# zjhellofss/KuiperLLama

Hardware: AMD Instinct MI355X
Metric: decode tokens/sec (higher is better)
Workload: dtype f32; 1 GPU; llama3.2-1b greedy decode, batch 1, prompt [1, 263], 2002 steps from pos 0 (demo/main.cpp generate); timing_backend=none, exec=hipGraph replay, 5L+2 fused HIP kernels per token, kv_cache_rows=131072

## Files before the change

include/kuiper_hip.h:

```cpp
#ifndef KUIPER_HIP_H
#define KUIPER_HIP_H
#include <stddef.h>
#include <stdint.h>

#ifdef __cplusplus
extern "C" {
#endif

#define KH_VERSION 100

enum {
  KH_OK = 0,
  KH_ERR_INVALID_ARG = -1,
  KH_ERR_UNSUPPORTED = -2,
  KH_ERR_IO = -3,
  KH_ERR_FORMAT = -4,
  KH_ERR_NO_DEVICE = -5,
  KH_ERR_RANGE = -6,
  KH_ERR_INTERNAL = -7
};
const char* kh_error_string(int code);
int kh_version(void);
int kh_device_count(void);

enum { KH_ROPE_INTERLEAVED = 0, KH_ROPE_HALF = 1 };
enum { KH_FAMILY_LLAMA = 0, KH_FAMILY_QWEN2 = 1 };


int kh_add_f32(const float* in1, const float* in2, float* out, int32_t n, void* stream);

int kh_matmul_f32(const float* x, const float* w, float* y, int32_t M, int32_t K, float scale,
                  void* stream);

int kh_matmul_q8(const float* x, const int8_t* w8, const float* scales, int32_t group_size,
                 float* y, int32_t M, int32_t K, void* stream);

int kh_embedding_f32(const int32_t* tokens, int32_t n_tokens, const float* w, float* out,
                     int32_t dim, int32_t vocab, void* stream);

int kh_embedding_f32_host(const int32_t* h_tokens, int32_t n_tokens, const float* w, float* out,
                          int32_t dim, int32_t vocab, void* stream);

int kh_swiglu_f32(const float* a, const float* b, float* out, int32_t n, void* stream);

int kh_rmsnorm_f32(const float* x, const float* w, float* out, int32_t n, float eps,
                   void* stream);

int kh_rope_f32(int32_t dim, int32_t kv_dim, int32_t head_size, float* q, float* k,
                const int32_t* d_pos, int32_t pos, const float* sin_cache,
                const float* cos_cache, int32_t mode, void* stream);

int kh_sincos_cache_f32(int32_t head_size, int32_t max_seq_len, float theta, float* sin_cache,
                        float* cos_cache, void* stream);

int kh_mha_f32(const int32_t* d_pos, int32_t pos, int32_t head_num, int32_t layer_index,
               int32_t seq_len, int32_t kv_dim, int32_t kv_mul, int32_t head_size,
               float* mha_out, const float* q, float* score, const float* kcache,
               const float* vcache, void* stream);

int kh_mha_prefill_f32(int32_t pos0, int32_t n_tokens, int32_t head_num, int32_t layer_index,
                       int32_t seq_len, int32_t kv_dim, int32_t kv_mul, int32_t head_size,
                       float* mha_out, const float* q, const float* key_cache,
                       const float* value_cache, void* stream);

int64_t kh_mha_decode_workspace_bytes(int32_t head_num, int32_t head_size, int32_t seq_len);
int kh_mha_decode_f32(const int32_t* d_pos, int32_t pos, int32_t head_num, int32_t layer_index,
                      int32_t seq_len, int32_t kv_dim, int32_t kv_mul, int32_t head_size,
                      float* mha_out, const float* q, const float* kcache, const float* vcache,
                      void* workspace, int64_t workspace_bytes, void* stream);

int kh_argmax_f32(const float* logits, int64_t n, int32_t* d_out_index, void* stream);
int kh_argmax_f32_host(const float* logits, int64_t n, int64_t* h_out_index, void* stream);

typedef struct kh_sampling {
  float temperature;
  int32_t top_k;
  float top_p;
  uint64_t seed;
} kh_sampling;
int kh_sample_f32(const float* logits, int64_t n, const kh_sampling* p, int64_t counter0, int32_t n_draws,
                  int32_t* d_out, void* stream);
int kh_sample_f32_host(const float* logits, int64_t n, const kh_sampling* p, int64_t counter, int64_t* h_out,
                       void* stream);

int kh_softmax_f32(float* x, int32_t n, void* stream);
int kh_scale_f32(float scale, float* x, int32_t n, void* stream);
int kh_scale_sum_f32(const float* value, const float* scale, float* out, int32_t pos,
                     int32_t size, int32_t stride, void* stream);

typedef struct kh_model kh_model;

typedef struct kh_model_opts {
  int32_t family;
  int32_t is_quant;
  int32_t rope_mode;
  float rope_theta;
  float rms_eps;
  int32_t max_seq_len;
  int32_t device;
  int32_t flags;
} kh_model_opts;
#define KH_FLAG_ATTN_MERGE_IN_LAUNCH 1
#define KH_FLAG_ATTN_MERGE_FENCED 2
#define KH_FLAG_PREFILL_EXACT 4

typedef struct kh_config {
  int32_t dim, hidden_dim, layer_num, head_num, kv_head_num, vocab_size, seq_len;
  int32_t kv_dim, kv_mul, head_size, is_shared_weight, is_quant, group_size;
  int32_t family, rope_mode, cache_len;
  float rope_theta, rms_eps;
  int64_t weight_bytes;
  int32_t launches_per_token;
  int32_t ring_selftest, attn_merge_selftest;
} kh_config;

int kh_model_create_from_file(const char* path, const kh_model_opts* opts, kh_model** out);
int kh_model_create_from_host_image(const void* h_image, size_t nbytes,
                                    const kh_model_opts* opts, kh_model** out);
int kh_model_create_from_device_weights(const int32_t* h_header, const void* d_weight_data,
                                        size_t weight_nbytes, const kh_model_opts* opts,
                                        kh_model** out);
void kh_model_destroy(kh_model* m);
int kh_model_get_config(const kh_model* m, kh_config* out);
void* kh_model_stream(kh_model* m);
float kh_model_get_load_ms(const kh_model* m);

enum {
  KH_EXEC_GRAPH = 0,
  KH_EXEC_FUSED = 1,
  KH_EXEC_UNFUSED = 2
};

int kh_model_predict(kh_model* m, int32_t token, int32_t pos, int32_t is_prompt, int32_t exec,
                     int32_t* h_next);
int kh_model_get_logits(kh_model* m, float* h_logits);
int kh_model_get_kv(kh_model* m, float** d_kcache, float** d_vcache);
int kh_model_kv_bytes(const kh_model* m, int64_t* reserved, int64_t* committed);
int kh_model_read_kv(kh_model* m, int32_t layer, int32_t row0, int32_t nrows, float* h_k,
                     float* h_v);
int kh_model_write_kv(kh_model* m, int32_t layer, int32_t row0, int32_t nrows, const float* h_k,
                      const float* h_v);

int kh_model_generate(kh_model* m, const int32_t* h_prompt, int32_t n_prompt,
                      int32_t total_steps, int32_t exec, int32_t* h_words, int32_t* n_words,
                      float* h_elapsed_ms);
int kh_model_generate_until(kh_model* m, const int32_t* h_prompt, int32_t n_prompt,
                            int32_t total_steps, int32_t exec, const int32_t* h_stop,
                            int32_t n_stop, int32_t* h_words, int32_t* n_words,
                            float* h_elapsed_ms);

int kh_model_prefill(kh_model* m, const int32_t* h_tokens, int32_t n, int32_t pos0);

int kh_model_prefill_gemm(kh_model* m, const int32_t* h_tokens, int32_t n, int32_t pos0);

typedef struct kh_first_sample {
  int32_t pos;
  int32_t prefill_mode;
  int32_t top1_id, top2_id;
  float top1, top2;
} kh_first_sample;
int kh_model_first_sample(kh_model* m, kh_first_sample* out);

int kh_model_set_sampling(kh_model* m, const kh_sampling* p);
int kh_model_get_sampling(const kh_model* m, kh_sampling* out);

int kh_plan_decode_shapes(int32_t dim, int32_t hidden_dim, int32_t kv_dim, int32_t vocab_size,
                          int32_t is_quant, int32_t* out20);
int kh_plan_decode_ring(int32_t dim, int32_t hidden_dim, int32_t vocab_size, int32_t is_quant, int32_t group_size,
                        int32_t* out4);
int kh_plan_attention(int32_t head_num, int32_t kv_mul, int32_t head_size, int32_t seq_len, int32_t pos,
                      int32_t* out8);
int kh_plan_prefill_shape(int32_t epi, int32_t T, int32_t rows, int32_t K, int32_t is_quant,
                          int32_t r2_ok, int32_t* out7);

int kh_debug_set(const char* key, const char* value);
const char* kh_debug_get(const char* key);
int64_t kh_debug_list(char* buf, int64_t cap);
int64_t kh_debug_launch_log(char* buf, int64_t cap);

enum { KH_PREFILL_TOKEN = 0, KH_PREFILL_GEMV = 1, KH_PREFILL_GEMM = 2 };
int kh_model_time_prefill(kh_model* m, const int32_t* h_tokens, int32_t n, int32_t pos0,
                          int32_t mode, float* h_ms);

int kh_model_profile_kernel(kh_model* m, int32_t kclass, int32_t pos, int32_t reps,
                            float* h_avg_us);

int kh_model_time_step(kh_model* m, int32_t pos, int32_t reps, float* h_us);

enum {
  KH_K_QKV = 0, KH_K_ATTN = 1, KH_K_WO = 2, KH_K_FFN13 = 3, KH_K_W2 = 4, KH_K_CLS = 5,
  KH_K_SAMPLE = 6, KH_NUM_KCLASS = 7
};
int kh_model_profile_step(kh_model* m, int32_t start_pos, int32_t n_steps, float* h_avg_us,
                          int32_t* h_count);
const char* kh_kclass_name(int kclass);

typedef struct kh_spm kh_spm;
int kh_spm_create_from_file(const char* tokenizer_model_path, kh_spm** out);
int kh_spm_create_from_memory(const void* model_proto, int64_t nbytes, kh_spm** out);
void kh_spm_destroy(kh_spm* t);
int32_t kh_spm_vocab_size(const kh_spm* t);
int32_t kh_spm_bos_id(const kh_spm* t);
int32_t kh_spm_eos_id(const kh_spm* t);
int32_t kh_spm_unk_id(const kh_spm* t);
int kh_spm_encode(const kh_spm* t, const char* utf8, int64_t len, int32_t add_bos, int32_t add_eos,
                  int32_t* out_ids, int32_t cap, int32_t* n_ids);
int kh_spm_decode(const kh_spm* t, const int32_t* ids, int32_t n, char* out_utf8, int64_t cap,
                  int64_t* out_len);

typedef struct kh_bpe kh_bpe;
enum { KH_BPE_LLAMA3 = 0, KH_BPE_QWEN2 = 1 };
enum { KH_BPE_REF_SPACES = 1 };
int kh_bpe_create_from_file(const char* tokenizer_json_path, int32_t flavor, kh_bpe** out);
int kh_bpe_create_from_memory(const void* tokenizer_json, int64_t nbytes, int32_t flavor, kh_bpe** out);
void kh_bpe_destroy(kh_bpe* t);
int32_t kh_bpe_vocab_size(const kh_bpe* t);
int32_t kh_bpe_bos_id(const kh_bpe* t);
int32_t kh_bpe_eos_id(const kh_bpe* t);
int32_t kh_bpe_stop_id(const kh_bpe* t, int32_t which);
int kh_bpe_encode(const kh_bpe* t, const char* utf8, int64_t len, int32_t add_bos, int32_t add_eos,
                  int32_t flags, int32_t* out_ids, int32_t cap, int32_t* n_ids);
int kh_bpe_decode(const kh_bpe* t, const int32_t* ids, int32_t n, int32_t flags, char* out_utf8,
                  int64_t cap, int64_t* out_len);

#ifdef __cplusplus
}
#endif
#endif
```

kuiperllama_amd/_ffi.py:

```python
from __future__ import annotations

import ctypes as C
import os
from typing import Optional

_PKG = os.path.dirname(os.path.abspath(__file__))
LIB_PATH = os.environ.get("KH_LIB") or os.path.join(_PKG, "lib", "libkuiper_hip.so")

EXPORTS = [
    "kh_error_string", "kh_version", "kh_device_count",
    "kh_add_f32", "kh_matmul_f32", "kh_matmul_q8", "kh_embedding_f32", "kh_embedding_f32_host", "kh_swiglu_f32",
    "kh_rmsnorm_f32", "kh_rope_f32", "kh_sincos_cache_f32", "kh_mha_f32", "kh_mha_decode_f32", "kh_mha_prefill_f32",
    "kh_mha_decode_workspace_bytes", "kh_argmax_f32",
    "kh_argmax_f32_host", "kh_sample_f32", "kh_sample_f32_host", "kh_softmax_f32", "kh_scale_f32", "kh_scale_sum_f32",
    "kh_model_create_from_file", "kh_model_create_from_host_image",
    "kh_model_create_from_device_weights", "kh_model_destroy", "kh_model_get_config",
    "kh_model_stream", "kh_model_get_load_ms", "kh_model_predict", "kh_model_get_logits", "kh_model_get_kv", "kh_model_kv_bytes", "kh_model_read_kv", "kh_model_write_kv",
    "kh_spm_create_from_file", "kh_spm_create_from_memory", "kh_spm_destroy", "kh_spm_vocab_size",
    "kh_spm_bos_id", "kh_spm_eos_id", "kh_spm_unk_id", "kh_spm_encode", "kh_spm_decode",
    "kh_bpe_create_from_file", "kh_bpe_create_from_memory", "kh_bpe_destroy", "kh_bpe_vocab_size",
    "kh_bpe_bos_id", "kh_bpe_eos_id", "kh_bpe_stop_id", "kh_bpe_encode", "kh_bpe_decode",
    "kh_model_generate", "kh_model_generate_until", "kh_model_first_sample", "kh_model_set_sampling", "kh_model_get_sampling", "kh_model_time_step", "kh_model_prefill", "kh_model_prefill_gemm", "kh_model_time_prefill", "kh_model_profile_kernel", "kh_model_profile_step", "kh_kclass_name",
    "kh_plan_decode_shapes", "kh_plan_decode_ring", "kh_plan_prefill_shape", "kh_plan_attention",
    "kh_debug_set", "kh_debug_get", "kh_debug_list", "kh_debug_launch_log",
]

KH_EXEC_GRAPH, KH_EXEC_FUSED, KH_EXEC_UNFUSED = 0, 1, 2
KH_NUM_KCLASS = 7
KH_ERR_RANGE = -6
KH_ERR_INTERNAL = -7
KH_FLAG_ATTN_MERGE_IN_LAUNCH = 1
KH_FLAG_ATTN_MERGE_FENCED = 2
KH_FLAG_PREFILL_EXACT = 4


class KhError(RuntimeError):
    def __init__(self, code: int, what: str):
        self.code = code
        super().__init__(f"{what}: kh error {code} ({error_string(code)})")


class ModelOpts(C.Structure):
    _fields_ = [("family", C.c_int32), ("is_quant", C.c_int32), ("rope_mode", C.c_int32),
                ("rope_theta", C.c_float), ("rms_eps", C.c_float), ("max_seq_len", C.c_int32),
                ("device", C.c_int32), ("flags", C.c_int32)]


class FirstSample(C.Structure):
    _fields_ = [("pos", C.c_int32), ("prefill_mode", C.c_int32), ("top1_id", C.c_int32), ("top2_id", C.c_int32),
                ("top1", C.c_float), ("top2", C.c_float)]


class Sampling(C.Structure):
    _fields_ = [("temperature", C.c_float), ("top_k", C.c_int32), ("top_p", C.c_float), ("seed", C.c_uint64)]

    def as_dict(self) -> dict:
        return {"temperature": float(self.temperature), "top_k": int(self.top_k), "top_p": float(self.top_p),
                "seed": int(self.seed)}


def sampling(temperature: float = 0.0, top_k: int = 0, top_p: float = 1.0, seed: int = 0) -> Sampling:
    return Sampling(float(temperature), int(top_k), float(top_p), int(seed) & 0xFFFFFFFFFFFFFFFF)


class Config(C.Structure):
    _fields_ = [(n, C.c_int32) for n in (
        "dim", "hidden_dim", "layer_num", "head_num", "kv_head_num", "vocab_size", "seq_len",
        "kv_dim", "kv_mul", "head_size", "is_shared_weight", "is_quant", "group_size", "family",
        "rope_mode", "cache_len")] + [("rope_theta", C.c_float), ("rms_eps", C.c_float),
                                      ("weight_bytes", C.c_int64), ("launches_per_token", C.c_int32),
                                      ("ring_selftest", C.c_int32), ("attn_merge_selftest", C.c_int32)]


_lib: Optional[C.CDLL] = None
_vp, _i32, _i64, _f32 = C.c_void_p, C.c_int32, C.c_int64, C.c_float


def lib() -> C.CDLL:
    global _lib
    if _lib is not None:
        return _lib
    import torch
    if not os.path.exists(LIB_PATH):
        raise ImportError(
            f"{LIB_PATH} is missing: build it with `python -m kuiperllama_amd.build` "
            "(there is no CPU fallback for the HIP path)")
    L = C.CDLL(LIB_PATH)
    L.kh_error_string.argtypes = [C.c_int]
    L.kh_error_string.restype = C.c_char_p
    L.kh_version.restype = C.c_int
    L.kh_device_count.restype = C.c_int
    L.kh_add_f32.argtypes = [_vp, _vp, _vp, _i32, _vp]
    L.kh_matmul_f32.argtypes = [_vp, _vp, _vp, _i32, _i32, _f32, _vp]
    L.kh_matmul_q8.argtypes = [_vp, _vp, _vp, _i32, _vp, _i32, _i32, _vp]
    L.kh_embedding_f32.argtypes = [_vp, _i32, _vp, _vp, _i32, _i32, _vp]
    L.kh_embedding_f32_host.argtypes = [_vp, _i32, _vp, _vp, _i32, _i32, _vp]
    L.kh_swiglu_f32.argtypes = [_vp, _vp, _vp, _i32, _vp]
    L.kh_rmsnorm_f32.argtypes = [_vp, _vp, _vp, _i32, _f32, _vp]
    L.kh_rope_f32.argtypes = [_i32, _i32, _i32, _vp, _vp, _vp, _i32, _vp, _vp, _i32, _vp]
    L.kh_sincos_cache_f32.argtypes = [_i32, _i32, _f32, _vp, _vp, _vp]
    L.kh_mha_f32.argtypes = [_vp, _i32, _i32, _i32, _i32, _i32, _i32, _i32, _vp, _vp, _vp, _vp,
                             _vp, _vp]
    L.kh_mha_decode_workspace_bytes.argtypes = [_i32, _i32, _i32]
    L.kh_mha_decode_workspace_bytes.restype = _i64
    L.kh_mha_prefill_f32.argtypes = [_i32] * 8 + [_vp, _vp, _vp, _vp, _vp]
    L.kh_mha_decode_f32.argtypes = [_vp, _i32, _i32, _i32, _i32, _i32, _i32, _i32, _vp, _vp, _vp,
                                    _vp, _vp, _i64, _vp]
    L.kh_argmax_f32.argtypes = [_vp, _i64, _vp, _vp]
    L.kh_argmax_f32_host.argtypes = [_vp, _i64, C.POINTER(_i64), _vp]
    L.kh_sample_f32.argtypes = [_vp, _i64, C.POINTER(Sampling), _i64, _i32, _vp, _vp]
    L.kh_sample_f32_host.argtypes = [_vp, _i64, C.POINTER(Sampling), _i64, C.POINTER(_i64), _vp]
    L.kh_softmax_f32.argtypes = [_vp, _i32, _vp]
    L.kh_scale_f32.argtypes = [_f32, _vp, _i32, _vp]
    L.kh_scale_sum_f32.argtypes = [_vp, _vp, _vp, _i32, _i32, _i32, _vp]
    L.kh_model_create_from_file.argtypes = [C.c_char_p, C.POINTER(ModelOpts), C.POINTER(_vp)]
    L.kh_model_create_from_host_image.argtypes = [_vp, C.c_size_t, C.POINTER(ModelOpts),
                                                  C.POINTER(_vp)]
    L.kh_model_create_from_device_weights.argtypes = [C.POINTER(_i32), _vp, C.c_size_t,
                                                      C.POINTER(ModelOpts), C.POINTER(_vp)]
    L.kh_model_destroy.argtypes = [_vp]
    L.kh_model_destroy.restype = None
    L.kh_model_get_config.argtypes = [_vp, C.POINTER(Config)]
    L.kh_model_stream.argtypes = [_vp]
    L.kh_model_stream.restype = _vp
    L.kh_model_get_load_ms.argtypes = [_vp]
    L.kh_model_get_load_ms.restype = _f32
    L.kh_model_predict.argtypes = [_vp, _i32, _i32, _i32, _i32, C.POINTER(_i32)]
    L.kh_model_get_logits.argtypes = [_vp, _vp]
    L.kh_model_get_kv.argtypes = [_vp, C.POINTER(_vp), C.POINTER(_vp)]
    L.kh_model_kv_bytes.argtypes = [_vp, C.POINTER(_i64), C.POINTER(_i64)]
    L.kh_model_read_kv.argtypes = [_vp, _i32, _i32, _i32, _vp, _vp]
    L.kh_model_write_kv.argtypes = [_vp, _i32, _i32, _i32, _vp, _vp]
    L.kh_model_generate.argtypes = [_vp, C.POINTER(_i32), _i32, _i32, _i32, C.POINTER(_i32),
                                    C.POINTER(_i32), C.POINTER(_f32)]
    L.kh_model_generate_until.argtypes = [_vp, C.POINTER(_i32), _i32, _i32, _i32, C.POINTER(_i32),
                                          _i32, C.POINTER(_i32), C.POINTER(_i32), C.POINTER(_f32)]
    L.kh_model_first_sample.argtypes = [_vp, C.POINTER(FirstSample)]
    L.kh_model_set_sampling.argtypes = [_vp, C.POINTER(Sampling)]
    L.kh_model_get_sampling.argtypes = [_vp, C.POINTER(Sampling)]
    L.kh_model_time_step.argtypes = [_vp, _i32, _i32, C.POINTER(_f32)]
    L.kh_plan_decode_shapes.argtypes = [_i32, _i32, _i32, _i32, _i32, C.POINTER(_i32)]
    L.kh_plan_decode_ring.argtypes = [_i32, _i32, _i32, _i32, _i32, C.POINTER(_i32)]
    L.kh_plan_prefill_shape.argtypes = [_i32, _i32, _i32, _i32, _i32, _i32, C.POINTER(_i32)]
    L.kh_plan_attention.argtypes = [_i32, _i32, _i32, _i32, _i32, C.POINTER(_i32)]
    L.kh_spm_create_from_file.argtypes = [C.c_char_p, C.POINTER(_vp)]
    L.kh_spm_create_from_memory.argtypes = [_vp, C.c_int64, C.POINTER(_vp)]
    L.kh_spm_destroy.argtypes = [_vp]
    L.kh_spm_destroy.restype = None
    for fn in (L.kh_spm_vocab_size, L.kh_spm_bos_id, L.kh_spm_eos_id, L.kh_spm_unk_id):
        fn.argtypes = [_vp]
        fn.restype = _i32
    L.kh_spm_encode.argtypes = [_vp, C.c_char_p, C.c_int64, _i32, _i32, C.POINTER(_i32), _i32,
                                C.POINTER(_i32)]
    L.kh_spm_decode.argtypes = [_vp, C.POINTER(_i32), _i32, C.c_char_p, C.c_int64,
                                C.POINTER(C.c_int64)]
    L.kh_bpe_create_from_file.argtypes = [C.c_char_p, _i32, C.POINTER(_vp)]
    L.kh_bpe_create_from_memory.argtypes = [_vp, C.c_int64, _i32, C.POINTER(_vp)]
    L.kh_bpe_destroy.argtypes = [_vp]
    L.kh_bpe_destroy.restype = None
    for fn in (L.kh_bpe_vocab_size, L.kh_bpe_bos_id, L.kh_bpe_eos_id):
        fn.argtypes = [_vp]
    L.kh_bpe_stop_id.argtypes = [_vp, _i32]
    L.kh_bpe_encode.argtypes = [_vp, C.c_char_p, C.c_int64, _i32, _i32, _i32, C.POINTER(_i32), _i32,
                                C.POINTER(_i32)]
    L.kh_bpe_decode.argtypes = [_vp, C.POINTER(_i32), _i32, _i32, C.c_char_p, C.c_int64,
                                C.POINTER(C.c_int64)]
    L.kh_model_prefill.argtypes = [_vp, C.POINTER(_i32), _i32, _i32]
    L.kh_model_prefill_gemm.argtypes = [_vp, C.POINTER(_i32), _i32, _i32]
    L.kh_model_time_prefill.argtypes = [_vp, C.POINTER(_i32), _i32, _i32, _i32, C.POINTER(_f32)]
    L.kh_model_profile_kernel.argtypes = [_vp, _i32, _i32, _i32, C.POINTER(_f32)]
    L.kh_model_profile_step.argtypes = [_vp, _i32, _i32, C.POINTER(_f32), C.POINTER(_i32)]
    L.kh_kclass_name.argtypes = [C.c_int]
    L.kh_kclass_name.restype = C.c_char_p
    L.kh_debug_set.argtypes = [C.c_char_p, C.c_char_p]
    L.kh_debug_get.argtypes = [C.c_char_p]
    L.kh_debug_get.restype = C.c_char_p
    L.kh_debug_list.argtypes = [C.c_char_p, _i64]
    L.kh_debug_list.restype = _i64
    L.kh_debug_launch_log.argtypes = [C.c_char_p, _i64]
    L.kh_debug_launch_log.restype = _i64
    for name in EXPORTS:
        getattr(L, name)
    _lib = L
    return L


def debug_set(key: str, value: Optional[str]) -> None:
    _ENV_MIRRORED.pop(key, None)
    check(lib().kh_debug_set(key.encode(), None if value is None else str(value).encode()), "kh_debug_set")


def debug_get(key: str) -> Optional[str]:
    v = lib().kh_debug_get(key.encode())
    return None if v is None else v.decode()


def launch_log() -> set:
    L = lib()
    n = L.kh_debug_launch_log(None, 0)
    buf = C.create_string_buffer(int(n) + 1)
    L.kh_debug_launch_log(buf, int(n) + 1)
    return {k for k in buf.value.decode().split("\n") if k}


_HOOK_PREFIXES = ("KH_SHAPE_", "KH_ATTN_", "KH_PG_", "KH_PREFILL", "KH_RING", "KH_SELFTEST", "KH_KV_")
_ENV_MIRRORED = {}
_ENV_SEEDED = False


def _seed_mirror(L) -> None:
    global _ENV_SEEDED
    _ENV_SEEDED = True
    n = L.kh_debug_list(None, 0)
    if n <= 0:
        return
    buf = C.create_string_buffer(int(n) + 1)
    L.kh_debug_list(buf, int(n) + 1)
    for k in buf.value.decode().split("\n"):
        if k and k.startswith(_HOOK_PREFIXES) and k in _ENV_AT_IMPORT:
            v = L.kh_debug_get(k.encode())
            if v is not None and v.decode() == _ENV_AT_IMPORT[k]:
                _ENV_MIRRORED.setdefault(k, _ENV_AT_IMPORT[k])


_ENV_AT_IMPORT = {k: v for k, v in os.environ.items() if k.startswith(_HOOK_PREFIXES)}


def sync_env() -> None:
    if not _ENV_SEEDED:
        _seed_mirror(lib())
    want = {k: v for k, v in os.environ.items() if k.startswith(_HOOK_PREFIXES)}
    if want == _ENV_MIRRORED:
        return
    L = lib()
    for k in set(_ENV_MIRRORED) - set(want):
        L.kh_debug_set(k.encode(), None)
        del _ENV_MIRRORED[k]
    for k, v in want.items():
        if _ENV_MIRRORED.get(k) != v:
            L.kh_debug_set(k.encode(), v.encode())
            _ENV_MIRRORED[k] = v


def error_string(code: int) -> str:
    return lib().kh_error_string(int(code)).decode()


def check(code: int, what: str) -> None:
    if code != 0:
        raise KhError(int(code), what)


def plan_decode_shapes(dim: int, hidden_dim: int, kv_dim: int, vocab_size: int, quant: bool) -> dict:
    sync_env()
    out = (_i32 * 20)()
    rc = lib().kh_plan_decode_shapes(dim, hidden_dim, kv_dim, vocab_size, int(quant), out)
    if rc != 0:
        raise KhError(rc, "kh_plan_decode_shapes")
    names = ("qkv", "wo", "ffn13", "w2", "cls")
    return {n: dict(zip(("split", "u", "grid", "wg"), out[4 * i:4 * i + 4])) for i, n in enumerate(names)}


def plan_decode_ring(dim: int, hidden_dim: int, vocab_size: int, quant: bool, group_size: int = 64) -> dict:
    sync_env()
    out = (_i32 * 4)()
    rc = lib().kh_plan_decode_ring(dim, hidden_dim, vocab_size, int(quant), group_size, out)
    if rc != 0:
        raise KhError(rc, "kh_plan_decode_ring")
    return {"ffn13": {"slots": out[0], "grid": out[1]}, "cls": {"slots": out[2], "grid": out[3]}}


def plan_attention(head_num: int, kv_mul: int, head_size: int, seq_len: int, pos: int) -> dict:
    sync_env()
    out = (_i32 * 8)()
    rc = lib().kh_plan_attention(head_num, kv_mul, head_size, seq_len, pos, out)
    if rc != 0:
        raise KhError(rc, "kh_plan_attention")
    return dict(zip(("ns", "ns_g", "stride", "t_long", "group_path", "active_splits", "split_len", "workgroups"),
                    list(out)))


def plan_prefill_shape(epi: str, T: int, rows: int, K: int, quant: bool, r2_ok: bool = True) -> dict:
    sync_env()
    out = (_i32 * 7)()
    rc = lib().kh_plan_prefill_shape({"qkv": 0, "resid": 1, "swiglu": 2}[epi], T, rows, K, int(quant),
                                     int(r2_ok), out)
    if rc != 0:
        raise KhError(rc, "kh_plan_prefill_shape")
    return dict(zip(("R", "NT", "ks", "slices", "solo", "kz", "workgroups"), out[:]))
```

kuiperllama_amd/build.py:

```python
from __future__ import annotations

import os
import shutil
import subprocess
import sys

_PKG = os.path.dirname(os.path.abspath(__file__))
CSRC = os.path.join(_PKG, "csrc")
LIB_DIR = os.path.join(_PKG, "lib")
LIB_PATH = os.path.join(LIB_DIR, "libkuiper_hip.so")
SOURCES = ["kh_ops.hip", "kh_model_load.hip", "kh_model_step.hip", "kh_model_prefill.hip", "kh_model_profile.hip", "kh_model_selftest.hip",
           "kh_tokenizer.cpp", "kh_bpe.cpp", "kh_debug.cpp"]
HEADERS = ["kh_common.h", "kh_gemv.h", "kh_attn.h", "kh_fused.h", "kh_q8ring.h", "kh_fused_ring.h", "kh_prefill.h", "kh_gemm.h", "kh_pattn.h", "kh_sample.h", "kh_unicode_tables.h",
           "kh_model_internal.h",
           "../../include/kuiper_hip.h"]
ARCH = "gfx950"


def _hipcc() -> str:
    for cand in (os.environ.get("HIPCC"), shutil.which("hipcc"), "/opt/rocm/bin/hipcc"):
        if cand and os.path.exists(cand):
            return cand
    raise RuntimeError("hipcc not found (set HIPCC=...)")


def _stale() -> bool:
    if not os.path.exists(LIB_PATH):
        return True
    t = os.path.getmtime(LIB_PATH)
    for f in SOURCES + HEADERS:
        p = os.path.normpath(os.path.join(CSRC, f))
        if os.path.exists(p) and os.path.getmtime(p) > t:
            return True
    return False


def build_lib(force: bool = False, verbose: bool = False) -> str:
    if not force and not _stale():
        return LIB_PATH
    os.makedirs(LIB_DIR, exist_ok=True)
    objs, procs = [], []
    for src in SOURCES:
        obj = os.path.join(LIB_DIR, os.path.splitext(src)[0] + ".o")
        cmd = [_hipcc(), f"--offload-arch={ARCH}", "-O3", "-std=c++17", "-fPIC", "-Wall",
               "-ffp-contract=off",
               "-Wno-unused-function", "-c", os.path.join(CSRC, src), "-o", obj]
        if verbose:
            print(" ".join(cmd), flush=True)
        procs.append((cmd, subprocess.Popen(cmd)))
        objs.append(obj)
    for cmd, pr in procs:
        if pr.wait() != 0:
            raise subprocess.CalledProcessError(pr.returncode, cmd)
    cmd = [_hipcc(), f"--offload-arch={ARCH}", "-shared", "-fPIC", "-o", LIB_PATH] + objs
    if verbose:
        print(" ".join(cmd), flush=True)
    subprocess.check_call(cmd)
    return LIB_PATH


def build_variant(name: str, defines: list[str], commit: str | None = None) -> str:
    out = os.path.join(LIB_DIR, name + ".so")
    if commit:
        import tarfile
        import tempfile
        root = os.path.normpath(os.path.join(_PKG, ".."))
        with tempfile.TemporaryDirectory() as td:
            tar = os.path.join(td, "src.tar")
            subprocess.check_call(["git", "-C", root, "archive", "-o", tar, commit, "kuiperllama_amd/csrc", "include"])
            with tarfile.open(tar) as tf:
                tf.extractall(td)
            global CSRC
            saved, CSRC = CSRC, os.path.join(td, "kuiperllama_amd", "csrc")
            try:
                return build_variant(name, defines)
            finally:
                CSRC = saved
    objs, procs = [], []
    od = os.path.join(LIB_DIR, "_" + name)
    os.makedirs(od, exist_ok=True)
    for src in SOURCES:
        if not os.path.exists(os.path.join(CSRC, src)):
            continue
        obj = os.path.join(od, os.path.splitext(src)[0] + ".o")
        cmd = [_hipcc(), f"--offload-arch={ARCH}", "-O3", "-std=c++17", "-fPIC", "-ffp-contract=off", "-w"] + \
              [f"-D{d}" for d in defines] + ["-c", os.path.join(CSRC, src), "-o", obj]
        procs.append((cmd, subprocess.Popen(cmd)))
        objs.append(obj)
    for cmd, pr in procs:
        if pr.wait() != 0:
            raise subprocess.CalledProcessError(pr.returncode, cmd)
    subprocess.check_call([_hipcc(), f"--offload-arch={ARCH}", "-shared", "-fPIC", "-o", out] + objs)
    shutil.rmtree(od, ignore_errors=True)
    return out


if __name__ == "__main__":
    if len(sys.argv) > 2 and sys.argv[1] == "--variant":
        print(build_variant(sys.argv[2], sys.argv[3:]))
    elif len(sys.argv) > 3 and sys.argv[1] == "--variant-at":
        print(build_variant(sys.argv[3], sys.argv[4:], commit=sys.argv[2]))
    else:
        print(build_lib(force="--force" in sys.argv, verbose=True))


ADAPTER_TEST_SRC = os.path.normpath(os.path.join(_PKG, "..", "tests", "cpp", "test_adapter.cpp"))
ADAPTER_TEST_BIN = os.path.join(LIB_DIR, "test_adapter")


def build_adapter_test(force: bool = False) -> str:
    build_lib()
    inc = os.path.normpath(os.path.join(_PKG, "..", "include"))
    deps = [ADAPTER_TEST_SRC, os.path.join(os.path.dirname(ADAPTER_TEST_SRC), "adapter_cases.hpp"),
            os.path.join(inc, "kuiper_hip_adapter.hpp"), os.path.join(inc, "kuiper_hip_alloc.hpp"), os.path.join(inc, "kuiper_hip.h"), LIB_PATH]
    if (not force and os.path.exists(ADAPTER_TEST_BIN)
            and all(os.path.getmtime(d) <= os.path.getmtime(ADAPTER_TEST_BIN) for d in deps)):
        return ADAPTER_TEST_BIN
    subprocess.check_call([_hipcc(), "-std=c++17", "-O2", f"-I{inc}", ADAPTER_TEST_SRC, "-o",
                           ADAPTER_TEST_BIN, f"-L{LIB_DIR}", "-lkuiper_hip",
                           "-Wl,-rpath,$ORIGIN"])
    return ADAPTER_TEST_BIN


DEMO_SRC = os.path.normpath(os.path.join(_PKG, "..", "tools", "kuiper_demo.cpp"))
DEMO_BIN = os.path.join(LIB_DIR, "kuiper_demo")


def build_demo(force: bool = False) -> str:
    build_lib()
    inc = os.path.normpath(os.path.join(_PKG, "..", "include"))
    deps = [DEMO_SRC, os.path.join(inc, "kuiper_hip.h"), LIB_PATH]
    if (not force and os.path.exists(DEMO_BIN)
            and all(os.path.getmtime(d) <= os.path.getmtime(DEMO_BIN) for d in deps)):
        return DEMO_BIN
    subprocess.check_call([_hipcc(), "-std=c++17", "-O2", f"-I{inc}", DEMO_SRC, "-o", DEMO_BIN,
                           f"-L{LIB_DIR}", "-lkuiper_hip", "-Wl,-rpath,$ORIGIN"])
    return DEMO_BIN


REF_ROOT = os.environ.get("KUIPER_REF", "/root/reference")
REF_BINDING_BIN = os.path.normpath(os.path.join(_PKG, "..", "oracle", "_ref", "test_ref_binding"))


def build_ref_binding() -> str | None:
    if not os.path.isdir(os.path.join(REF_ROOT, "kuiper", "include")):
        return REF_BINDING_BIN if os.path.exists(REF_BINDING_BIN) else None
    build_lib()
    subprocess.check_call(["make", "-s", "-C", os.path.normpath(os.path.join(_PKG, "..", "oracle")),
                           "ref", f"KUIPER_REF={REF_ROOT}", f"HIPCC={_hipcc()}"])
    return REF_BINDING_BIN


REF_LAYERS_BIN = os.path.normpath(os.path.join(_PKG, "..", "oracle", "_ref", "test_ref_layers"))


def build_ref_layers() -> str | None:
    if not os.path.isdir(os.path.join(REF_ROOT, "kuiper", "include")):
        return REF_LAYERS_BIN if os.path.exists(REF_LAYERS_BIN) else None
    build_lib()
    subprocess.check_call(["make", "-s", "-C", os.path.normpath(os.path.join(_PKG, "..", "oracle")),
                           "ref_layers", f"KUIPER_REF={REF_ROOT}", f"HIPCC={_hipcc()}"])
    return REF_LAYERS_BIN


REF_MODEL_BIN = os.path.normpath(os.path.join(_PKG, "..", "oracle", "_ref", "test_ref_model"))


def build_ref_model(qwen2: bool = False) -> str | None:
    exe = REF_MODEL_BIN + ("_qwen2" if qwen2 else "")
    if not os.path.isdir(os.path.join(REF_ROOT, "kuiper", "include")):
        return exe if os.path.exists(exe) else None
    build_lib()
    subprocess.check_call(["make", "-s", "-C", os.path.normpath(os.path.join(_PKG, "..", "oracle")),
                           "ref_model_qwen2" if qwen2 else "ref_model", f"KUIPER_REF={REF_ROOT}", f"HIPCC={_hipcc()}"])
    return exe


REF_CPU_BINS = {flavor: os.path.normpath(os.path.join(_PKG, "..", "oracle", "_ref", "ref_cpu_model" + suffix))
                for flavor, suffix in (("default", ""), ("llama3", "_llama3"), ("qwen2", "_qwen2"))}


def build_ref_cpu() -> dict | None:
    if os.path.isdir(os.path.join(REF_ROOT, "kuiper", "include")):
        build_lib()
        subprocess.check_call(["make", "-s", "-C", os.path.normpath(os.path.join(_PKG, "..", "oracle")),
                               "ref_cpu", f"KUIPER_REF={REF_ROOT}", f"HIPCC={_hipcc()}"])
    return dict(REF_CPU_BINS) if all(os.path.exists(p) for p in REF_CPU_BINS.values()) else None


def ref_cpu_flavor(spec) -> str | None:
    from . import binfmt
    if spec.quant:
        return None
    key = (spec.family, spec.rope_mode, float(spec.rope_theta), float(spec.rms_eps))
    table = {(binfmt.FAMILY_LLAMA, binfmt.ROPE_INTERLEAVED, 10000.0, 1e-5): "default",
             (binfmt.FAMILY_LLAMA, binfmt.ROPE_HALF, 500000.0, 1e-5): "llama3",
             (binfmt.FAMILY_QWEN2, binfmt.ROPE_HALF, 1000000.0, 1e-6): "qwen2"}
    return table.get(key)


def kernel_sources_sha1() -> str:
    import hashlib
    h = hashlib.sha1()
    d = os.path.join(os.path.dirname(os.path.abspath(__file__)), "csrc")
    for f in sorted(os.listdir(d)):
        if f.startswith("kh_") and f.endswith(".h") and f != "kh_model_internal.h":
            h.update(f.encode())
            h.update(open(os.path.join(d, f), "rb").read())
    return h.hexdigest()
```

kuiperllama_amd/csrc/kh_model_internal.h:

```cpp
#pragma once
#include <new>
#include <thread>
#include <stdint.h>

#include <vector>

#include "kh_attn.h"
#include "kh_common.h"

namespace khm {
template <class F>
static inline int kh_api_guard(F&& body) noexcept {
  try {
    return body();
  } catch (const std::bad_alloc&) {
    return (int)hipErrorOutOfMemory;
  } catch (...) {
    return KH_ERR_INTERNAL;
  }
}
struct KhJoinOnExit {
  std::thread& t;
  ~KhJoinOnExit() {
    if (t.joinable()) t.join();
  }
};

struct LayerW {
  KhLin wq, wk, wv, wo, w1, w2, w3;
  const float* att_norm;
  const float* ffn_norm;
};

}
using khm::LayerW;

#define KH_STEP_VARIANTS 3
struct KhSampParams;
struct kh_model {
  kh_config cfg{};
  kh_model_opts opts{};
  hipStream_t stream = nullptr;
  char* arena = nullptr;
  bool owns_arena = false;
  size_t arena_bytes = 0;
  std::vector<LayerW> layers;
  const float* tok_emb = nullptr;
  const float* final_norm = nullptr;
  KhLin cls{};
  int gshift = 0;
  float *x = nullptr, *rms = nullptr, *q = nullptr, *att = nullptr, *h1 = nullptr,
        *h3 = nullptr, *w2o = nullptr, *logits = nullptr, *score = nullptr, *kcache = nullptr,
        *vcache = nullptr, *sin_cache = nullptr, *cos_cache = nullptr;
  float* part_val = nullptr;
  int32_t* part_idx = nullptr;
  int nparts = 0;
  struct KvVmm {
    bool on = false;
    size_t chunk = 0;
    size_t reserved = 0;
    size_t mapped = 0;
    std::vector<uint8_t> have[2];
    struct Run {
      void* va;
      size_t len;
      hipMemGenericAllocationHandle_t h;
    };
    std::vector<Run> runs;
    int rows_all = 0;
  };
  KvVmm kv;
  float load_ms = 0.f;
  std::thread unmap_thread;
  void* attn_ws = nullptr;
  int attn_ns = 1;
  int attn_ns_g = 0;
  int attn_ws_stride = 1;
  int attn_t_long = 1 << 30;
  int attn_wg = KH_WG;
  int attn_ts_shift = 8;
  bool attn_fenced = false;
  bool attn_defer = false;
  int attn_defer_max = 0;
  int step_var = 0;
  int32_t *d_pos = nullptr, *d_token = nullptr, *d_next = nullptr, *d_forced = nullptr,
          *d_words = nullptr;
  int seq_cap = 0;
  float *pf_x = nullptr, *pf_q = nullptr, *pf_att = nullptr, *pf_h = nullptr;
  void* pf_ws = nullptr;
  size_t pf_ws_tok_bytes = 0;
  float *pg_x = nullptr, *pg_xn = nullptr, *pg_q = nullptr, *pg_att = nullptr, *pg_h = nullptr;
  float* pg_part = nullptr;
  void* pg_ws = nullptr;
  size_t pg_ws_tok_bytes = 0;
  bool pf_ready = false, pg_ready = false;
  bool pg_launch_failed = false;
  int32_t* h_words_pin = nullptr;
  int32_t* h_forced_pin = nullptr;
  int forced_hwm = 0;
  bool forced_in_flight = false;
  float* first_logits = nullptr;
  int first_pos = -1;
  int first_mode = 0;
  int pin_cap = 0;
  hipEvent_t ev_chunk[2] = {nullptr, nullptr};
  struct Shape {
    int u = 2, split = 1, grid = 1, wg = KH_WG;
  };
  Shape sh_qkv, sh_wo, sh_ffn, sh_w2, sh_cls;
  struct RingPlan {
    int ffn_r = 0, ffn_grid = 0, cls_r = 0, cls_grid = 0;
  };
  RingPlan ring;
  struct StepGraph {
    hipGraph_t g = nullptr;
    hipGraphExec_t e = nullptr;
  };
  StepGraph sg[2][KH_STEP_VARIANTS][4];
  kh_sampling samp{0.f, 0, 1.f, 0};
  bool samp_on = false;
  KhSampParams* d_samp = nullptr;
  hipEvent_t ev0 = nullptr, ev1 = nullptr;
};

#define KH_GRAPH_STEPS 8
#define KH_PG_MIN_TOKENS 16

namespace khm {
template <typename T>
int dalloc(T** p, size_t n) {
  hipError_t e = hipMalloc((void**)p, n * sizeof(T));
  return e == hipSuccess ? KH_OK : (int)e;
}

kh_model::Shape pick_shape(bool quant, int pairs, int M, int max_split, const char* env, int wg = KH_WG,
                           int wg_max = KH_WG, bool many_waves = false, bool u3 = false);
void plan_decode_shapes(bool quant, int dim, int hidden_dim, int kv_dim, int vocab_size, kh_model::Shape (&out)[5]);
void plan_ring(bool quant, int dim, int hidden_dim, int vocab_size, int group_size, kh_model::RingPlan* out);
int configure_step_kernels(kh_model* m);
KhAttnArgs fill_attn(kh_model* m, int l);
void launch_qkv(kh_model* m, int l);
void launch_attn(kh_model* m, int l);
void launch_wo(kh_model* m, int l);
void launch_ffn13(kh_model* m, int l);
void launch_w2(kh_model* m, int l);
void launch_cls(kh_model* m);
void launch_sample(kh_model* m, int advance, int n_forced);
int step_variant(const kh_model* m, int pos_lo, int pos_hi);
void launch_step_fused(kh_model* m, int advance, int n_forced, hipEvent_t* ev, int variant);
int launch_step_unfused(kh_model* m, int pos);
void set_state(kh_model* m, int token, int pos);
int ensure_pinned_words(kh_model* m, int n);
int ensure_seq_cap(kh_model* m, int n);
void destroy_step_graphs(kh_model* m);
int step_graph(kh_model* m, int n_forced, int variant, bool steps8, hipGraphExec_t* out);
int step_graph_n(kh_model* m, int n_forced, int variant, int nsteps, hipGraphExec_t* out);
int kv_ensure(kh_model* m, int rows, int layer = -1);
int run_selftests(kh_model* m);
bool prefill_supported(const kh_model* m);
bool pg_supported(const kh_model* m);
}
```

kuiperllama_amd/csrc/kh_model_load.hip:

```cpp
#include <fcntl.h>
#include <math.h>
#include <stdio.h>
#include <stdlib.h>
#include <string.h>
#include <sys/mman.h>
#include <sys/stat.h>
#include <unistd.h>

#include <atomic>
#include <mutex>
#include <utility>
#include <chrono>
#include <new>
#include <thread>
#include <vector>

#include "kh_model_internal.h"

using namespace khm;

namespace {

struct PhaseClock {
  std::chrono::steady_clock::time_point t = std::chrono::steady_clock::now();
  const bool on = dbg("KH_LOAD_DEBUG") != nullptr;
  void lap(const char* what) {
    if (!on) return;
    const auto n = std::chrono::steady_clock::now();
    fprintf(stderr, "[kh load] %-34s %7.2f ms\n", what, std::chrono::duration<double, std::milli>(n - t).count());
    t = n;
  }
};

int ilog2_exact(int v) {
  if (v <= 0 || (v & (v - 1))) return -1;
  int s = 0;
  while ((1 << s) < v) ++s;
  return s;
}

int upload_threads() {
  long n = sysconf(_SC_NPROCESSORS_ONLN);
  if (FILE* f = fopen("/sys/fs/cgroup/cpu.max", "r")) {
    long long quota = 0, period = 0;
    char q[32] = {0};
    if (fscanf(f, "%31s %lld", q, &period) == 2 && strcmp(q, "max") != 0 && period > 0) {
      quota = atoll(q);
      if (quota > 0 && quota / period < n) n = (long)(quota / period);
    }
    fclose(f);
  }
  n /= 2;
  return n < 1 ? 1 : (n > 8 ? 8 : (int)n);
}
hipError_t upload_chunked(char* d_dst, const char* h_src, size_t n, hipStream_t stream,
                          float* ms_out) {
  constexpr int NB = 4;
  const size_t CH = (size_t)32 << 20;
  const auto t0 = std::chrono::steady_clock::now();
  if (n <= CH) {
    hipError_t e = hipMemcpy(d_dst, h_src, n, hipMemcpyHostToDevice);
    if (ms_out)
      *ms_out = std::chrono::duration<float, std::milli>(std::chrono::steady_clock::now() - t0).count();
    return e;
  }
  char* pin[NB] = {nullptr, nullptr, nullptr, nullptr};
  hipEvent_t done[NB] = {nullptr, nullptr, nullptr, nullptr};
  hipError_t e = hipSuccess;
  PhaseClock pc;
  for (int i = 0; i < NB && e == hipSuccess; ++i) {
    e = hipHostMalloc((void**)&pin[i], CH, hipHostMallocDefault);
    if (e == hipSuccess) e = hipEventCreateWithFlags(&done[i], hipEventDisableTiming);
  }
  pc.lap("pinned staging ring");
  if (e == hipSuccess) {
    const size_t nchunks = (n + CH - 1) / CH;
    const int NT = upload_threads();
    std::vector<std::atomic<int>> filled(nchunks);
    for (auto& f : filled) f.store(0, std::memory_order_relaxed);
    std::atomic<long> released{NB};
    std::atomic<bool> abort_{false};
    auto worker = [&](int w) {
      for (size_t c = 0; c < nchunks; ++c) {
        if (abort_.load(std::memory_order_relaxed)) return;
        while ((long)c >= released.load(std::memory_order_acquire)) {
          if (abort_.load(std::memory_order_relaxed)) return;
          std::this_thread::yield();
        }
        const size_t off = c * CH, len = off + CH <= n ? CH : n - off;
        const size_t per = ((len + NT - 1) / NT + 4095) & ~(size_t)4095;
        const size_t s0 = (size_t)w * per, s1 = s0 + per < len ? s0 + per : len;
        if (s0 < len) memcpy(pin[c % NB] + s0, h_src + off + s0, s1 - s0);
        filled[c].fetch_add(1, std::memory_order_release);
      }
    };
    std::vector<std::thread> team;
    try {
      team.reserve((size_t)NT);
      for (int w = 0; w < NT; ++w) team.emplace_back(worker, w);
    } catch (...) {
      abort_.store(true);
      e = hipErrorOutOfMemory;
    }
    for (size_t c = 0; c < nchunks && e == hipSuccess; ++c) {
      while (filled[c].load(std::memory_order_acquire) < NT) std::this_thread::yield();
      const size_t off = c * CH, len = off + CH <= n ? CH : n - off;
      e = hipMemcpyAsync(d_dst + off, pin[c % NB], len, hipMemcpyHostToDevice, stream);
      if (e == hipSuccess) e = hipEventRecord(done[c % NB], stream);
      if (c + 1 >= (size_t)NB && c + 1 < nchunks && e == hipSuccess) {
        e = hipEventSynchronize(done[(c + 1) % NB]);
        released.store((long)c + 2, std::memory_order_release);
      }
    }
    if (e != hipSuccess) abort_.store(true);
    released.store((long)nchunks + NB, std::memory_order_release);
    for (auto& t : team) t.join();
    if (e == hipSuccess) e = hipStreamSynchronize(stream);
    pc.lap("staged upload");
  }
  for (int i = 0; i < NB; ++i) {
    if (done[i]) (void)hipEventDestroy(done[i]);
    if (pin[i]) (void)hipHostFree(pin[i]);
  }
  if (ms_out)
    *ms_out = std::chrono::duration<float, std::milli>(std::chrono::steady_clock::now() - t0).count();
  return e;
}

struct SinCosJob {
  std::vector<float> s, c;
  std::vector<std::thread> team;
  void start(size_t CL, int head_size, float theta) {
    const size_t n = CL * (size_t)head_size;
    s.resize(n);
    c.resize(n);
    std::vector<float> freq((size_t)head_size);
    for (int d = 0; d < head_size; ++d) freq[d] = 1.0f / powf(theta, (float)d / (float)head_size);
    const int NT = CL >= 4096 ? upload_threads() : 1;
    for (int w = 0; w < NT; ++w)
      team.emplace_back([this, CL, head_size, freq, w, NT] {
        const size_t p0 = CL * (size_t)w / NT, p1 = CL * (size_t)(w + 1) / NT;
        for (size_t p = p0; p < p1; ++p)
          for (int d = 0; d < head_size; ++d) {
            const float val = (float)p * freq[d];
            s[p * head_size + d] = sinf(val);
            c[p * head_size + d] = cosf(val);
          }
      });
  }
  void join() {
    for (auto& t : team) t.join();
    team.clear();
  }
  ~SinCosJob() { join(); }
};

int build_weight_table(kh_model* m) {
  const kh_config& c = m->cfg;
  const int L = c.layer_num, dim = c.dim, kvd = c.kv_dim, hid = c.hidden_dim, V = c.vocab_size;
  m->layers.assign((size_t)L, LayerW{});
  char* base = m->arena;
  size_t off = 0;
  if (!c.is_quant) {
    const bool bias = c.family == KH_FAMILY_QWEN2;
    auto takef = [&](size_t n) {
      const float* p = (const float*)(base + off);
      off += n * sizeof(float);
      return p;
    };
    m->tok_emb = takef((size_t)V * dim);
    for (int l = 0; l < L; ++l) m->layers[l].att_norm = takef((size_t)dim);
    for (int l = 0; l < L; ++l) {
      m->layers[l].wq.w = takef((size_t)dim * dim);
      if (bias) m->layers[l].wq.bias = takef((size_t)dim);
    }
    for (int l = 0; l < L; ++l) {
      m->layers[l].wk.w = takef((size_t)kvd * dim);
      if (bias) m->layers[l].wk.bias = takef((size_t)kvd);
    }
    for (int l = 0; l < L; ++l) {
      m->layers[l].wv.w = takef((size_t)kvd * dim);
      if (bias) m->layers[l].wv.bias = takef((size_t)kvd);
    }
    for (int l = 0; l < L; ++l) m->layers[l].wo.w = takef((size_t)dim * dim);
    for (int l = 0; l < L; ++l) m->layers[l].ffn_norm = takef((size_t)dim);
    for (int l = 0; l < L; ++l) m->layers[l].w1.w = takef((size_t)hid * dim);
    for (int l = 0; l < L; ++l) m->layers[l].w2.w = takef((size_t)dim * hid);
    for (int l = 0; l < L; ++l) m->layers[l].w3.w = takef((size_t)hid * dim);
    m->final_norm = takef((size_t)dim);
    (void)takef((size_t)c.seq_len * c.head_size);
    if (c.is_shared_weight) {
      m->cls.w = m->tok_emb;
    } else {
      m->cls.w = takef((size_t)V * dim);
    }
  } else {
    const size_t gs = (size_t)c.group_size;
    auto takeq = [&](KhLin& Lw, size_t K, size_t M) {
      const size_t n = K * M;
      Lw.w = base + off;
      Lw.scales = (const float*)(base + off + n);
      off += n + (n / gs) * sizeof(float);
    };
    for (int l = 0; l < L; ++l) takeq(m->layers[l].wq, dim, dim);
    for (int l = 0; l < L; ++l) takeq(m->layers[l].wk, kvd, dim);
    for (int l = 0; l < L; ++l) takeq(m->layers[l].wv, kvd, dim);
    for (int l = 0; l < L; ++l) takeq(m->layers[l].wo, dim, dim);
    for (int l = 0; l < L; ++l) takeq(m->layers[l].w1, hid, dim);
    for (int l = 0; l < L; ++l) takeq(m->layers[l].w2, dim, hid);
    for (int l = 0; l < L; ++l) takeq(m->layers[l].w3, hid, dim);
    takeq(m->cls, V, dim);
    const float* fp = (const float*)(base + off);
    m->tok_emb = fp;
    fp += (size_t)V * dim;
    for (int l = 0; l < L; ++l) m->layers[l].att_norm = fp + (size_t)l * dim;
    fp += (size_t)L * dim;
    for (int l = 0; l < L; ++l) m->layers[l].ffn_norm = fp + (size_t)l * dim;
    fp += (size_t)L * dim;
    m->final_norm = fp;
    fp += dim;
    off = (size_t)((const char*)fp - base);
  }
  if (off > m->arena_bytes) return KH_ERR_FORMAT;
  return KH_OK;
}

int parse_header(const int32_t* h, const kh_model_opts* o, kh_config* c) {
  memset(c, 0, sizeof(*c));
  c->dim = h[0];
  c->hidden_dim = h[1];
  c->layer_num = h[2];
  c->head_num = h[3];
  c->kv_head_num = h[4];
  c->is_shared_weight = h[5] > 0;
  c->vocab_size = h[5] < 0 ? -h[5] : h[5];
  c->seq_len = h[6];
  c->is_quant = o->is_quant ? 1 : 0;
  c->group_size = o->is_quant ? h[7] : 0;
  if (c->dim <= 0 || c->hidden_dim <= 0 || c->layer_num <= 0 || c->head_num <= 0 ||
      c->kv_head_num <= 0 || c->vocab_size <= 0 || c->seq_len <= 0)
    return KH_ERR_FORMAT;
  if (c->dim % c->head_num || c->head_num % c->kv_head_num) return KH_ERR_FORMAT;
  c->kv_dim = (c->dim * c->kv_head_num) / c->head_num;
  c->kv_mul = c->head_num / c->kv_head_num;
  c->head_size = c->dim / c->head_num;
  c->family = o->family;
  c->rope_mode = o->rope_mode;
  c->rope_theta = o->rope_theta;
  c->rms_eps = o->rms_eps;
  c->cache_len = (o->max_seq_len > 0 && o->max_seq_len < c->seq_len) ? o->max_seq_len : c->seq_len;
  if (c->is_quant) {
    if (c->group_size <= 0) return KH_ERR_FORMAT;
    if (c->is_shared_weight || c->family == KH_FAMILY_QWEN2) return KH_ERR_UNSUPPORTED;
  }
  if (o->rope_mode != KH_ROPE_HALF && o->rope_mode != KH_ROPE_INTERLEAVED) return KH_ERR_INVALID_ARG;
  if (o->family != KH_FAMILY_LLAMA && o->family != KH_FAMILY_QWEN2) return KH_ERR_INVALID_ARG;
  if (!(o->rope_theta > 0.f) || !(o->rms_eps > 0.f)) return KH_ERR_INVALID_ARG;
  const int a = c->is_quant ? 16 : 4;
  if (c->dim % a || c->hidden_dim % a || c->head_size % 4 || (c->head_size & 1) ||
      c->head_size > 256 || c->kv_dim % 4 || (c->dim & 1) || (c->kv_dim & 1))
    return KH_ERR_UNSUPPORTED;
  if (c->is_quant) {
    const int gs = ilog2_exact(c->group_size);
    if (gs < 4 || c->dim % c->group_size || c->hidden_dim % c->group_size) return KH_ERR_UNSUPPORTED;
  }
  return KH_OK;
}

size_t expected_weight_bytes(const kh_config& c) {
  const size_t L = c.layer_num, dim = c.dim, kvd = c.kv_dim, hid = c.hidden_dim, V = c.vocab_size;
  const size_t lin = L * (2 * dim * dim + 2 * kvd * dim + 3 * hid * dim);
  if (!c.is_quant) {
    size_t n = V * dim + 2 * L * dim + lin + dim + (size_t)c.seq_len * c.head_size;
    if (c.family == KH_FAMILY_QWEN2) n += L * (dim + 2 * kvd);
    if (!c.is_shared_weight) n += V * dim;
    return n * sizeof(float);
  }
  const size_t q = lin + V * dim;
  return q + (q / (size_t)c.group_size) * sizeof(float) + (V * dim + 2 * L * dim + dim) * sizeof(float);
}

static int kv_ensure_impl(kh_model* m, int row0, int rows, int layer);
static void kv_release(kh_model* m);
struct VaPool {
  std::mutex mu;
  std::vector<std::pair<void*, size_t>> ranges;
};
static VaPool& va_pool() {
  static VaPool* p = new VaPool();
  return *p;
}
static void* va_take(size_t bytes, size_t align) {
  {
    VaPool& vp = va_pool();
    std::lock_guard<std::mutex> g(vp.mu);
    for (size_t i = vp.ranges.size(); i-- > 0;)
      if (vp.ranges[i].second == bytes) {
        void* p = vp.ranges[i].first;
        vp.ranges.erase(vp.ranges.begin() + (long)i);
        return p;
      }
  }
  void* p = nullptr;
  if (hipMemAddressReserve(&p, bytes, align, nullptr, 0) != hipSuccess) {
    (void)hipGetLastError();
    return nullptr;
  }
  return p;
}
static void va_give(void* p, size_t bytes) {
  if (!p) return;
  if (dbg_off("KH_KV_VA_POOL")) {
    (void)hipMemAddressFree(p, bytes);
    return;
  }
  VaPool& vp = va_pool();
  std::lock_guard<std::mutex> g(vp.mu);
  vp.ranges.emplace_back(p, bytes);
}
static int kv_allocate(kh_model* m) {
  const kh_config& c = m->cfg;
  const size_t total = (size_t)c.layer_num * (size_t)c.cache_len * c.kv_dim * sizeof(float);
  kh_model::KvVmm& kv = m->kv;
  if (!dbg_off("KH_KV_VMM")) {
    hipMemAllocationProp prop = {};
    prop.type = hipMemAllocationTypePinned;
    prop.location.type = hipMemLocationTypeDevice;
    prop.location.id = m->opts.device;
    size_t gran = 0;
    if (hipMemGetAllocationGranularity(&gran, &prop, hipMemAllocationGranularityRecommended) == hipSuccess && gran > 0) {
      size_t chunk = (size_t)8 << 20;
      chunk = (chunk + gran - 1) / gran * gran;
      const size_t reserved = (total + chunk - 1) / chunk * chunk;
      void *pk = va_take(reserved, chunk), *pv = nullptr;
      if (pk) {
        if ((pv = va_take(reserved, chunk)) != nullptr) {
          kv.on = true;
          kv.chunk = chunk;
          kv.reserved = reserved;
          kv.have[0].assign(reserved / chunk, 0);
          kv.have[1].assign(reserved / chunk, 0);
          m->kcache = (float*)pk;
          m->vcache = (float*)pv;
          if (kv_ensure_impl(m, 0, 1, 0) == KH_OK) return KH_OK;
          kv_release(m);
          kv = kh_model::KvVmm();
        } else {
          va_give(pk, reserved);
        }
      }
    }
    (void)hipGetLastError();
  }
  int rc;
  if ((rc = dalloc(&m->kcache, total / sizeof(float))) != KH_OK) return rc;
  return dalloc(&m->vcache, total / sizeof(float));
}
static void kv_release(kh_model* m) {
  kh_model::KvVmm& kv = m->kv;
  if (!kv.on) {
    if (m->kcache) (void)hipFree(m->kcache);
    if (m->vcache) (void)hipFree(m->vcache);
  } else {
    for (const auto& r : kv.runs) {
      (void)hipMemUnmap(r.va, r.len);
      (void)hipMemRelease(r.h);
    }
    kv.runs.clear();
    if (m->kcache) va_give(m->kcache, kv.reserved);
    if (m->vcache) va_give(m->vcache, kv.reserved);
    kv.on = false;
  }
  m->kcache = m->vcache = nullptr;
}
static int kv_ensure_impl(kh_model* m, int row0, int rows, int layer) {
  kh_model::KvVmm& kv = m->kv;
  if (!kv.on || rows <= 0) return KH_OK;
  const kh_config& c = m->cfg;
  if (rows > c.cache_len) rows = c.cache_len;
  if (rows <= kv.rows_all || row0 >= rows) return KH_OK;
  if (row0 < 0) row0 = 0;
  hipMemAllocationProp prop = {};
  prop.type = hipMemAllocationTypePinned;
  prop.location.type = hipMemLocationTypeDevice;
  prop.location.id = m->opts.device;
  hipMemAccessDesc acc = {};
  acc.location = prop.location;
  acc.flags = hipMemAccessFlagsProtReadWrite;
  const size_t row_b = (size_t)c.kv_dim * sizeof(float), layer_b = (size_t)c.cache_len * row_b;
  const int l0 = layer >= 0 ? layer : 0, l1 = layer >= 0 ? layer + 1 : c.layer_num;
  for (int which = 0; which < 2; ++which) {
    char* base = (char*)(which ? m->vcache : m->kcache);
    std::vector<uint8_t>& have = kv.have[which];
    for (int l = l0; l < l1; ++l) {
      const size_t b0 = (size_t)l * layer_b + (size_t)row0 * row_b, b1 = (size_t)l * layer_b + (size_t)rows * row_b;
      size_t ch = b0 / kv.chunk;
      const size_t ch_end = (b1 + kv.chunk - 1) / kv.chunk;
      while (ch < ch_end) {
        if (have[ch]) {
          ++ch;
          continue;
        }
        size_t e = ch;
        while (e < ch_end && !have[e]) ++e;
        for (size_t k = ch; k < e; ++k) {
          kh_model::KvVmm::Run r;
          r.va = base + k * kv.chunk;
          r.len = kv.chunk;
          const char* what = "hipMemCreate";
          hipError_t err = hipMemCreate(&r.h, r.len, &prop, 0);
          if (err == hipSuccess) {
            what = "hipMemMap";
            err = hipMemMap(r.va, r.len, 0, r.h, 0);
            if (err == hipSuccess) {
              what = "hipMemSetAccess";
              err = hipMemSetAccess(r.va, r.len, &acc, 1);
              if (err != hipSuccess) (void)hipMemUnmap(r.va, r.len);
            }
            if (err != hipSuccess) (void)hipMemRelease(r.h);
          }
          if (err != hipSuccess) {
            fprintf(stderr, "[kh] KV cache: %s of %zu MiB at chunk %zu of the %s cache (layer %d) failed: %s\n", what,
                    r.len >> 20, k, which ? "V" : "K", l, hipGetErrorString(err));
            (void)hipGetLastError();
            return (int)err;
          }
          kv.runs.push_back(r);
          have[k] = 1;
          kv.mapped += r.len;
        }
        KH_CHECK_HIP(hipMemsetAsync(base + ch * kv.chunk, 0, (e - ch) * kv.chunk, m->stream));
        ch = e;
      }
    }
  }
  if (layer < 0 && row0 == 0) kv.rows_all = rows;
  return KH_OK;
}

int finish_create(kh_model* m, SinCosJob* sincos = nullptr) {
  const kh_config& c = m->cfg;
  int rc;
  PhaseClock pc;
  if ((rc = build_weight_table(m)) != KH_OK) return rc;
  m->gshift = c.is_quant ? ilog2_exact(c.group_size) : 0;
  const size_t CL = (size_t)c.cache_len;
#define KH_ALLOC(ptr, n) \
  if ((rc = dalloc(&(ptr), (n))) != KH_OK) return rc
  KH_ALLOC(m->x, (size_t)c.dim);
  KH_ALLOC(m->rms, (size_t)c.dim);
  KH_ALLOC(m->q, (size_t)c.dim);
  KH_ALLOC(m->att, (size_t)c.dim);
  KH_ALLOC(m->w2o, (size_t)c.dim);
  KH_ALLOC(m->h1, (size_t)c.hidden_dim);
  KH_ALLOC(m->h3, (size_t)c.hidden_dim);
  KH_ALLOC(m->logits, (size_t)c.vocab_size);
  KH_ALLOC(m->score, (size_t)c.head_num * CL);
  pc.lap("weight table + small buffers");
  if ((rc = kv_allocate(m)) != KH_OK) return rc;
  KH_ALLOC(m->sin_cache, CL * c.head_size);
  KH_ALLOC(m->cos_cache, CL * c.head_size);
  KH_ALLOC(m->d_pos, 1);
  KH_ALLOC(m->d_token, 1);
  KH_ALLOC(m->d_next, 1);
  {
    kh_model::Shape sh[5];
    plan_decode_shapes(c.is_quant != 0, c.dim, c.hidden_dim, c.kv_dim, c.vocab_size, sh);
    m->sh_qkv = sh[0]; m->sh_wo = sh[1]; m->sh_ffn = sh[2]; m->sh_w2 = sh[3]; m->sh_cls = sh[4];
  }
  plan_ring(c.is_quant != 0, c.dim, c.hidden_dim, c.vocab_size, c.group_size, &m->ring);
  m->nparts = m->ring.cls_r ? m->ring.cls_grid : m->sh_cls.grid;
  if (dbg("KH_SHAPE_DEBUG")) {
    if (m->ring.ffn_r || m->ring.cls_r)
      fprintf(stderr, "[kh] LDS-DMA ring: ffn13 R %d grid %d | cls R %d grid %d (256 threads)\n", m->ring.ffn_r,
              m->ring.ffn_grid, m->ring.cls_r, m->ring.cls_grid);
    const struct { const char* n; const kh_model::Shape* s; } all[] = {
        {"qkv", &m->sh_qkv}, {"wo", &m->sh_wo}, {"ffn13", &m->sh_ffn}, {"w2", &m->sh_w2}, {"cls", &m->sh_cls}};
    for (const auto& e : all)
      fprintf(stderr, "[kh] shape %-5s split %d u %d grid %d wg %d\n", e.n, e.s->split, e.s->u, e.s->grid, e.s->wg);
  }
  m->attn_wg = KH_WG_MAX;
  if (const char* e = dbg("KH_ATTN_WG"))
    if (atoi(e) == 256 || atoi(e) == 512) m->attn_wg = atoi(e);
  {
    const AttnPlan ap = attn_plan(c.head_num, c.kv_mul, c.head_size, c.cache_len, m->attn_wg, attn_tlong_hook());
    m->attn_ns = ap.ns;
    m->attn_ts_shift = ap.ts_shift;
    m->attn_ns_g = ap.ns_g;
    m->attn_ws_stride = ap.stride;
    m->attn_t_long = ap.t_long;
  }
  {
    const char* e = dbg("KH_ATTN_FENCED");
    m->attn_fenced = (m->opts.flags & KH_FLAG_ATTN_MERGE_FENCED) != 0 || (e && e[0] == '1');
  }
  m->attn_defer = m->attn_ns > 1 && !(m->opts.flags & KH_FLAG_ATTN_MERGE_IN_LAUNCH) && !dbg_off("KH_ATTN_DEFER") &&
                  comb_supported(c.dim, c.head_num, c.head_size, m->sh_wo.wg);
  {
    const int mv = c.dim <= 2 * 4 * m->sh_wo.wg ? 2 : 4;
    const bool overlap = !(m->sh_wo.u >= 8 || (c.is_quant && m->sh_wo.u >= 4 && mv >= 4));
    m->attn_defer_max = overlap ? KH_ATTN_MAX_NS : 4;
    if (const char* e = dbg("KH_ATTN_DEFER_MAX")) m->attn_defer_max = atoi(e);
  }
  if (const size_t wsb = attn_ws_bytes(c.head_num, c.head_size, m->attn_ws_stride)) {
    KH_CHECK_HIP(hipMalloc(&m->attn_ws, wsb));
    KH_CHECK_HIP(hipMemsetAsync(m->attn_ws, 0, wsb, m->stream));
  }
  KH_ALLOC(m->part_val, (size_t)m->nparts);
  KH_ALLOC(m->part_idx, (size_t)m->nparts);
#undef KH_ALLOC
  pc.lap("caches, tables, plans, workspace");
  if (!m->kv.on) {
    KH_CHECK_HIP(hipMemsetAsync(m->kcache, 0, sizeof(float) * c.layer_num * CL * c.kv_dim, m->stream));
    KH_CHECK_HIP(hipMemsetAsync(m->vcache, 0, sizeof(float) * c.layer_num * CL * c.kv_dim, m->stream));
  }
  KH_CHECK_HIP(hipMemsetAsync(m->d_pos, 0, sizeof(int32_t), m->stream));
  KH_CHECK_HIP(hipMemsetAsync(m->d_token, 0, sizeof(int32_t), m->stream));
  {
    SinCosJob local;
    SinCosJob* job = sincos;
    if (!job) {
      local.start(CL, c.head_size, c.rope_theta);
      job = &local;
    }
    job->join();
    pc.lap("wait for the RoPE table threads");
    const size_t n = CL * c.head_size;
    KH_CHECK_HIP(hipMemcpy(m->sin_cache, job->s.data(), n * sizeof(float), hipMemcpyHostToDevice));
    KH_CHECK_HIP(hipMemcpy(m->cos_cache, job->c.data(), n * sizeof(float), hipMemcpyHostToDevice));
  }
  pc.lap("RoPE table upload");
  if ((rc = configure_step_kernels(m)) != KH_OK) return rc;
  KH_CHECK_HIP(hipEventCreate(&m->ev0));
  KH_CHECK_HIP(hipEventCreate(&m->ev1));
  if ((rc = ensure_seq_cap(m, 256)) != KH_OK) return rc;
  KH_CHECK_HIP(hipStreamSynchronize(m->stream));
  pc.lap("kernel attributes, events, sync");
  return KH_OK;
}

int new_model(const int32_t* h_header, const kh_model_opts* opts, kh_model** out) {
  if (!h_header || !opts || !out) return KH_ERR_INVALID_ARG;
  *out = nullptr;
  int ndev = 0;
  if (hipGetDeviceCount(&ndev) != hipSuccess || ndev <= 0) {
    (void)hipGetLastError();
    return KH_ERR_NO_DEVICE;
  }
  if (opts->device < 0 || opts->device >= ndev) return KH_ERR_INVALID_ARG;
  kh_config cfg;
  int rc = parse_header(h_header, opts, &cfg);
  if (rc != KH_OK) return rc;
  KH_CHECK_HIP(hipSetDevice(opts->device));
  kh_model* m = new (std::nothrow) kh_model();
  if (!m) return (int)hipErrorOutOfMemory;
  m->cfg = cfg;
  m->opts = *opts;
  hipError_t e = hipStreamCreateWithFlags(&m->stream, hipStreamNonBlocking);
  if (e != hipSuccess) {
    delete m;
    return (int)e;
  }
  *out = m;
  return KH_OK;
}

}

namespace khm {
int kv_ensure(kh_model* m, int rows, int layer) { return kv_ensure_impl(m, 0, rows, layer); }
}

extern "C" void kh_model_destroy(kh_model* m) {
  if (!m) return;
  if (m->unmap_thread.joinable()) m->unmap_thread.join();
  if (m->stream) (void)hipStreamSynchronize(m->stream);
  destroy_step_graphs(m);
  if (m->ev0) (void)hipEventDestroy(m->ev0);
  if (m->ev1) (void)hipEventDestroy(m->ev1);
  for (void* q : {(void*)m->pf_x, (void*)m->pf_q, (void*)m->pf_att, (void*)m->pf_h, m->pf_ws,
                  (void*)m->pg_x, (void*)m->pg_xn, (void*)m->pg_q, (void*)m->pg_att, (void*)m->pg_h, (void*)m->pg_part,
                  m->pg_ws})
    if (q) (void)hipFree(q);
  for (auto e : m->ev_chunk)
    if (e) (void)hipEventDestroy(e);
  if (m->h_words_pin) (void)hipHostFree(m->h_words_pin);
  if (m->h_forced_pin) (void)hipHostFree(m->h_forced_pin);
  if (m->first_logits) (void)hipFree(m->first_logits);
  if (m->d_samp) (void)hipFree(m->d_samp);
  void* bufs[] = {m->x,      m->rms,    m->q,         m->att,       m->h1,       m->h3,
                  m->w2o,    m->logits, m->score,     m->sin_cache,
                  m->cos_cache, m->part_val, m->part_idx, m->d_pos, m->d_token,  m->d_next,
                  m->d_forced, m->d_words, m->attn_ws};
  for (void* b : bufs)
    if (b) (void)hipFree(b);
  kv_release(m);
  if (m->owns_arena && m->arena) (void)hipFree(m->arena);
  if (m->stream) (void)hipStreamDestroy(m->stream);
  delete m;
}

static int create_from_device_weights_impl(const int32_t* h_header, const void* d_weight_data, size_t weight_nbytes,
                                           const kh_model_opts* opts, kh_model** out) {
  kh_model* m = nullptr;
  int rc = new_model(h_header, opts, &m);
  if (rc != KH_OK) return rc;
  *out = m;
  if (weight_nbytes < expected_weight_bytes(m->cfg)) {
    kh_model_destroy(m);
    *out = nullptr;
    return KH_ERR_FORMAT;
  }
  m->arena = (char*)const_cast<void*>(d_weight_data);
  m->owns_arena = false;
  m->arena_bytes = weight_nbytes;
  m->cfg.weight_bytes = (int64_t)expected_weight_bytes(m->cfg);
  rc = finish_create(m);
  if (rc == KH_OK) rc = run_selftests(m);
  if (rc != KH_OK) {
    kh_model_destroy(m);
    m = nullptr;
  }
  *out = m;
  return rc;
}
extern "C" int kh_model_create_from_device_weights(const int32_t* h_header,
                                                   const void* d_weight_data,
                                                   size_t weight_nbytes,
                                                   const kh_model_opts* opts, kh_model** out) {
  if (!d_weight_data || !kh_aligned16(d_weight_data)) return KH_ERR_INVALID_ARG;
  if (!out) return KH_ERR_INVALID_ARG;
  *out = nullptr;
  const int rc =
      kh_api_guard([&] { return create_from_device_weights_impl(h_header, d_weight_data, weight_nbytes, opts, out); });
  if (rc != KH_OK && *out) {
    kh_model_destroy(*out);
    *out = nullptr;
  }
  return rc;
}

static int create_from_host_image_impl(const void* h_image, size_t nbytes, const kh_model_opts* opts,
                                       kh_model** out) {
  const size_t hdr = opts->is_quant ? 32 : 28;
  if (nbytes < hdr) return KH_ERR_FORMAT;
  int32_t header[8] = {0};
  memcpy(header, h_image, hdr);
  kh_model* m = nullptr;
  int rc = new_model(header, opts, &m);
  if (rc != KH_OK) return rc;
  *out = m;
  const size_t need = expected_weight_bytes(m->cfg);
  if (nbytes - hdr < need) {
    kh_model_destroy(m);
    *out = nullptr;
    return KH_ERR_FORMAT;
  }
  SinCosJob sincos;
  sincos.start((size_t)m->cfg.cache_len, m->cfg.head_size, m->cfg.rope_theta);
  PhaseClock pc;
  hipError_t e = hipMalloc((void**)&m->arena, need);
  pc.lap("arena hipMalloc");
  if (e != hipSuccess) {
    sincos.join();
    kh_model_destroy(m);
    *out = nullptr;
    return (int)e;
  }
  m->owns_arena = true;
  m->arena_bytes = need;
  m->cfg.weight_bytes = (int64_t)need;
  hipError_t eu = hipSuccess;
  const int dev = m->opts.device;
  std::thread uploader([&] {
    eu = hipSetDevice(dev);
    if (eu == hipSuccess) eu = upload_chunked(m->arena, (const char*)h_image + hdr, need, m->stream, &m->load_ms);
  });
  KhJoinOnExit join_uploader{uploader};
  rc = finish_create(m, &sincos);
  uploader.join();
  if (rc == KH_OK && eu != hipSuccess) rc = (int)eu;
  if (rc == KH_OK) {
    const hipError_t es = hipStreamSynchronize(m->stream);
    if (es != hipSuccess) rc = (int)es;
  }
  pc.lap("upload || buffers, joined");
  if (rc == KH_OK) rc = run_selftests(m);
  pc.lap("self-tests");
  if (rc != KH_OK) {
    kh_model_destroy(m);
    m = nullptr;
  }
  *out = m;
  return rc;
}
extern "C" int kh_model_create_from_host_image(const void* h_image, size_t nbytes,
                                               const kh_model_opts* opts, kh_model** out) {
  if (!h_image || !opts || !out) return KH_ERR_INVALID_ARG;
  *out = nullptr;
  const int rc = kh_api_guard([&] { return create_from_host_image_impl(h_image, nbytes, opts, out); });
  if (rc != KH_OK && *out) {
    kh_model_destroy(*out);
    *out = nullptr;
  }
  return rc;
}

extern "C" int kh_model_create_from_file(const char* path, const kh_model_opts* opts,
                                         kh_model** out) {
  if (!path || !opts || !out) return KH_ERR_INVALID_ARG;
  const int fd = open(path, O_RDONLY);
  if (fd == -1) return KH_ERR_IO;
  struct stat st;
  if (fstat(fd, &st) == -1 || st.st_size <= 0) {
    close(fd);
    return KH_ERR_IO;
  }
  PhaseClock pc;
  void* data = mmap(nullptr, (size_t)st.st_size, PROT_READ, MAP_PRIVATE, fd, 0);
  if (data == MAP_FAILED || data == nullptr) {
    close(fd);
    return KH_ERR_IO;
  }
  (void)madvise(data, (size_t)st.st_size, MADV_SEQUENTIAL);
  (void)madvise(data, (size_t)st.st_size, MADV_WILLNEED);
  pc.lap("open + mmap + madvise");
  const int rc = kh_model_create_from_host_image(data, (size_t)st.st_size, opts, out);
  pc.lap("create_from_host_image");
  const size_t len = (size_t)st.st_size;
  bool handed = false;
  if (rc == KH_OK && out && *out) {
    try {
      (*out)->unmap_thread = std::thread([data, len, fd] {
        munmap(data, len);
        close(fd);
      });
      handed = true;
    } catch (...) {
    }
  }
  if (!handed) {
    munmap(data, len);
    close(fd);
  }
  pc.lap("munmap handed to a helper thread");
  return rc;
}

extern "C" int kh_model_get_config(const kh_model* m, kh_config* out) {
  if (!m || !out) return KH_ERR_INVALID_ARG;
  *out = m->cfg;
  out->launches_per_token = 5 * m->cfg.layer_num + 2;
  return KH_OK;
}
extern "C" float kh_model_get_load_ms(const kh_model* m) { return m ? m->load_ms : -1.f; }
extern "C" void* kh_model_stream(kh_model* m) { return m ? (void*)m->stream : nullptr; }

extern "C" int kh_model_get_logits(kh_model* m, float* h_logits) {
  if (!m || !h_logits) return KH_ERR_INVALID_ARG;
  KH_CHECK_HIP(hipMemcpyAsync(h_logits, m->logits, sizeof(float) * m->cfg.vocab_size,
                              hipMemcpyDeviceToHost, m->stream));
  KH_CHECK_HIP(hipStreamSynchronize(m->stream));
  return KH_OK;
}
extern "C" int kh_model_first_sample(kh_model* m, kh_first_sample* out) {
  if (!m || !out) return KH_ERR_INVALID_ARG;
  if (m->first_pos < 0 || !m->first_logits) return KH_ERR_UNSUPPORTED;
  KH_CHECK_HIP(hipSetDevice(m->opts.device));
  const int V = m->cfg.vocab_size;
  std::vector<float> h((size_t)V);
  KH_CHECK_HIP(hipMemcpyAsync(h.data(), m->first_logits, sizeof(float) * (size_t)V, hipMemcpyDeviceToHost, m->stream));
  KH_CHECK_HIP(hipStreamSynchronize(m->stream));
  int i1 = 0, i2 = -1;
  for (int i = 1; i < V; ++i) {
    if (h[i] > h[i1]) {
      i2 = i1;
      i1 = i;
    } else if (i2 < 0 || h[i] > h[i2]) {
      i2 = i;
    }
  }
  out->pos = m->first_pos;
  out->prefill_mode = m->first_mode;
  out->top1_id = i1;
  out->top2_id = i2;
  out->top1 = h[i1];
  out->top2 = i2 >= 0 ? h[i2] : h[i1];
  return KH_OK;
}
extern "C" int kh_model_get_kv(kh_model* m, float** d_kcache, float** d_vcache) {
  if (!m || !d_kcache || !d_vcache) return KH_ERR_INVALID_ARG;
  KH_CHECK_HIP(hipSetDevice(m->opts.device));
  const int rc = kv_ensure(m, m->cfg.cache_len);
  if (rc != KH_OK) return rc;
  *d_kcache = m->kcache;
  *d_vcache = m->vcache;
  return KH_OK;
}

extern "C" int kh_model_kv_bytes(const kh_model* m, int64_t* reserved, int64_t* committed) {
  if (!m || !reserved || !committed) return KH_ERR_INVALID_ARG;
  const int64_t total = 2 * (int64_t)m->cfg.layer_num * m->cfg.cache_len * m->cfg.kv_dim * (int64_t)sizeof(float);
  *reserved = total;
  *committed = m->kv.on ? (int64_t)m->kv.mapped : total;
  return KH_OK;
}

extern "C" int kh_model_read_kv(kh_model* m, int32_t layer, int32_t row0, int32_t nrows,
                                float* h_k, float* h_v) {
  if (!m || !h_k || !h_v || layer < 0 || layer >= m->cfg.layer_num || row0 < 0 || nrows <= 0 ||
      (int64_t)row0 + nrows > m->cfg.cache_len)
    return KH_ERR_INVALID_ARG;
  KH_CHECK_HIP(hipSetDevice(m->opts.device));
  {
    const int rc = kv_ensure_impl(m, row0, row0 + nrows, layer);
    if (rc != KH_OK) return rc;
  }
  const size_t off = ((size_t)layer * m->cfg.cache_len + row0) * m->cfg.kv_dim;
  const size_t nb = (size_t)nrows * m->cfg.kv_dim * sizeof(float);
  KH_CHECK_HIP(hipMemcpyAsync(h_k, m->kcache + off, nb, hipMemcpyDeviceToHost, m->stream));
  KH_CHECK_HIP(hipMemcpyAsync(h_v, m->vcache + off, nb, hipMemcpyDeviceToHost, m->stream));
  KH_CHECK_HIP(hipStreamSynchronize(m->stream));
  return KH_OK;
}

extern "C" int kh_model_write_kv(kh_model* m, int32_t layer, int32_t row0, int32_t nrows,
                                 const float* h_k, const float* h_v) {
  if (!m || !h_k || !h_v || layer < 0 || layer >= m->cfg.layer_num || row0 < 0 || nrows <= 0 ||
      (int64_t)row0 + nrows > m->cfg.cache_len)
    return KH_ERR_INVALID_ARG;
  KH_CHECK_HIP(hipSetDevice(m->opts.device));
  {
    const int rc = kv_ensure_impl(m, row0, row0 + nrows, layer);
    if (rc != KH_OK) return rc;
  }
  const size_t off = ((size_t)layer * m->cfg.cache_len + row0) * m->cfg.kv_dim;
  const size_t nb = (size_t)nrows * m->cfg.kv_dim * sizeof(float);
  KH_CHECK_HIP(hipMemcpyAsync(m->kcache + off, h_k, nb, hipMemcpyDefault, m->stream));
  KH_CHECK_HIP(hipMemcpyAsync(m->vcache + off, h_v, nb, hipMemcpyDefault, m->stream));
  KH_CHECK_HIP(hipStreamSynchronize(m->stream));
  return KH_OK;
}
```

kuiperllama_amd/csrc/kh_model_selftest.hip:

```cpp
#include <chrono>
#include <string.h>

#include "kh_model_internal.h"

#define KH_SELFTEST_ATTN_LAUNCHES 24

namespace {

__global__ __launch_bounds__(KH_WG) void k_st_fill(float* p, size_t n, uint32_t seed, float scale) {
  for (size_t i = (size_t)blockIdx.x * KH_WG + threadIdx.x; i < n; i += (size_t)gridDim.x * KH_WG) {
    uint32_t h = (uint32_t)i * 2654435761u ^ seed;
    h ^= h >> 15;
    h *= 2246822519u;
    h ^= h >> 13;
    p[i] = scale * ((float)(h & 0xffffu) / 32768.0f - 1.0f);
  }
}
__global__ __launch_bounds__(KH_WG) void k_st_diff(const uint32_t* a, const uint32_t* b, size_t n, int32_t* flag) {
  bool d = false;
  for (size_t i = (size_t)blockIdx.x * KH_WG + threadIdx.x; i < n; i += (size_t)gridDim.x * KH_WG) d |= a[i] != b[i];
  if (d) *flag = 1;
}
inline int grid_for(size_t n) {
  const size_t g = (n + KH_WG - 1) / KH_WG;
  return (int)(g < 1 ? 1 : (g > 1024 ? 1024 : g));
}
inline bool hook_has(const char* v, const char* word) { return v && strstr(v, word) != nullptr; }

}

namespace khm {

static int ring_selftest(kh_model* m, int32_t* d_flag, bool inject, int* result) {
  const kh_config& c = m->cfg;
  *result = 0;
  if (!m->ring.ffn_r && !m->ring.cls_r) return KH_OK;
  const kh_model::RingPlan plan = m->ring;
  hipStream_t s = m->stream;
  int rc = KH_OK;
  set_state(m, 1 % c.vocab_size, 0);
  if (plan.ffn_r) {
    launch_ffn13(m, 0);
    KH_CHECK_HIP(hipMemcpyAsync(m->h3, m->h1, sizeof(float) * (size_t)c.hidden_dim, hipMemcpyDeviceToDevice, s));
    m->ring.ffn_r = 0;
    launch_ffn13(m, 0);
    m->ring = plan;
    hipLaunchKernelGGL(k_st_diff, dim3(grid_for((size_t)c.hidden_dim)), dim3(KH_WG), 0, s, (const uint32_t*)m->h1,
                       (const uint32_t*)m->h3, (size_t)c.hidden_dim, d_flag);
  }
  float* tmp_logits = nullptr;
  float* tmp_pv = nullptr;
  int32_t* tmp_pi = nullptr;
  if (plan.cls_r) {
    const size_t np = (size_t)(m->sh_cls.grid > plan.cls_grid ? m->sh_cls.grid : plan.cls_grid);
    if ((rc = dalloc(&tmp_logits, (size_t)c.vocab_size)) == KH_OK && (rc = dalloc(&tmp_pv, np)) == KH_OK &&
        (rc = dalloc(&tmp_pi, np)) == KH_OK) {
      launch_cls(m);
      float* const lg = m->logits;
      float* const pv = m->part_val;
      int32_t* const pi = m->part_idx;
      m->logits = tmp_logits;
      m->part_val = tmp_pv;
      m->part_idx = tmp_pi;
      m->ring.cls_r = 0;
      launch_cls(m);
      m->ring = plan;
      m->logits = lg;
      m->part_val = pv;
      m->part_idx = pi;
      hipLaunchKernelGGL(k_st_diff, dim3(grid_for((size_t)c.vocab_size)), dim3(KH_WG), 0, s, (const uint32_t*)lg,
                         (const uint32_t*)tmp_logits, (size_t)c.vocab_size, d_flag);
    }
  }
  int32_t flag = 0;
  hipError_t e = hipMemcpyAsync(&flag, d_flag, sizeof(flag), hipMemcpyDeviceToHost, s);
  if (e == hipSuccess) e = hipStreamSynchronize(s);
  for (void* q : {(void*)tmp_logits, (void*)tmp_pv, (void*)tmp_pi})
    if (q) (void)hipFree(q);
  if (rc != KH_OK) return rc;
  if (e != hipSuccess) return (int)e;
  if ((rc = kh_launch_status()) != KH_OK) return rc;
  *result = 1;
  if (!flag && !inject) return KH_OK;
  *result = -1;
  m->ring = kh_model::RingPlan();
  if (m->sh_cls.grid != m->nparts) {
    (void)hipFree(m->part_val);
    (void)hipFree(m->part_idx);
    m->part_val = nullptr;
    m->part_idx = nullptr;
    m->nparts = m->sh_cls.grid;
    if ((rc = dalloc(&m->part_val, (size_t)m->nparts)) != KH_OK) return rc;
    if ((rc = dalloc(&m->part_idx, (size_t)m->nparts)) != KH_OK) return rc;
  }
  return KH_OK;
}

static int attn_merge_case(kh_model* m, int pos, int variant, int32_t* d_flag) {
  const kh_config& c = m->cfg;
  hipStream_t s = m->stream;
  set_state(m, 1 % c.vocab_size, pos);
  m->step_var = variant;
  m->attn_fenced = true;
  launch_attn(m, 0);
  KH_CHECK_HIP(hipMemcpyAsync(m->rms, m->att, sizeof(float) * (size_t)c.dim, hipMemcpyDeviceToDevice, s));
  m->attn_fenced = false;
  for (int i = 0; i < KH_SELFTEST_ATTN_LAUNCHES; ++i) {
    launch_attn(m, 0);
    hipLaunchKernelGGL(k_st_diff, dim3(grid_for((size_t)c.dim)), dim3(KH_WG), 0, s, (const uint32_t*)m->att,
                       (const uint32_t*)m->rms, (size_t)c.dim, d_flag);
  }
  return kh_launch_status();
}

static int attn_selftest(kh_model* m, int32_t* d_flag, bool inject, int* result) {
  const kh_config& c = m->cfg;
  *result = 2;
  if (m->attn_fenced) return KH_OK;
  *result = 0;
  if (c.head_size <= 32 || m->attn_ns <= 1) return KH_OK;
  int pos1 = (c.cache_len < 1024 ? c.cache_len : 1024) - 1;
  if (pos1 + 1 >= m->attn_t_long) pos1 = m->attn_t_long - 2;
  const bool head_case = pos1 >= 1 && attn_active_splits(pos1, m->attn_ns, m->attn_ts_shift) >= 2;
  int pos2 = -1;
  if (m->attn_ns_g > 0 && m->attn_t_long < c.cache_len) {
    pos2 = m->attn_t_long + 255 < c.cache_len ? m->attn_t_long + 255 : c.cache_len - 1;
    if (attn_active_splits(pos2, m->attn_ns_g, KH_ATTN_TSG_SHIFT) < 2) pos2 = -1;
  }
  if (!head_case && pos2 < 0) return KH_OK;
  const size_t rows = (size_t)((head_case ? pos1 : 0) > pos2 ? (head_case ? pos1 : 0) : pos2) + 1;
  const size_t n = rows * (size_t)c.kv_dim;
  hipStream_t s = m->stream;
  int rc = kv_ensure(m, (int)rows, 0);
  if (rc != KH_OK) return rc;
  hipLaunchKernelGGL(k_st_fill, dim3(grid_for(n)), dim3(KH_WG), 0, s, m->kcache, n, 0x9e3779b9u, 1.0f);
  hipLaunchKernelGGL(k_st_fill, dim3(grid_for(n)), dim3(KH_WG), 0, s, m->vcache, n, 0x85ebca6bu, 1.0f);
  hipLaunchKernelGGL(k_st_fill, dim3(grid_for((size_t)c.dim)), dim3(KH_WG), 0, s, m->q, (size_t)c.dim, 0xc2b2ae35u, 1.0f);
  if (head_case) rc = attn_merge_case(m, pos1, m->attn_ns_g > 0 ? 2 : 0, d_flag);
  if (rc == KH_OK && pos2 >= 0) rc = attn_merge_case(m, pos2, 0, d_flag);
  m->step_var = 0;
  m->attn_fenced = false;
  int32_t flag = 0;
  hipError_t e = hipMemsetAsync(m->kcache, 0, n * sizeof(float), s);
  if (e == hipSuccess) e = hipMemsetAsync(m->vcache, 0, n * sizeof(float), s);
  if (e == hipSuccess) e = hipMemcpyAsync(&flag, d_flag, sizeof(flag), hipMemcpyDeviceToHost, s);
  if (e == hipSuccess) e = hipStreamSynchronize(s);
  if (rc != KH_OK) return rc;
  if (e != hipSuccess) return (int)e;
  *result = 1;
  if (!flag && !inject) return KH_OK;
  *result = -1;
  m->attn_fenced = true;
  return KH_OK;
}

int run_selftests(kh_model* m) {
  m->cfg.ring_selftest = 0;
  m->cfg.attn_merge_selftest = m->attn_fenced ? 2 : 0;
  if (dbg_off("KH_SELFTEST")) return KH_OK;
  const auto t0 = std::chrono::steady_clock::now();
  const char* inj = dbg("KH_SELFTEST_FAIL");
  int32_t* d_flag = nullptr;
  KH_CHECK_HIP(hipMalloc((void**)&d_flag, 2 * sizeof(int32_t)));
  int r = 0, a = 0;
  const hipError_t e = hipMemsetAsync(d_flag, 0, 2 * sizeof(int32_t), m->stream);
  int rc = e == hipSuccess ? ring_selftest(m, d_flag, hook_has(inj, "ring"), &r) : (int)e;
  if (rc == KH_OK) rc = attn_selftest(m, d_flag + 1, hook_has(inj, "attn"), &a);
  (void)hipFree(d_flag);
  if (rc != KH_OK) return rc;
  m->cfg.ring_selftest = r;
  m->cfg.attn_merge_selftest = a;
  if (dbg("KH_LOAD_DEBUG") || dbg("KH_SHAPE_DEBUG"))
    fprintf(stderr, "[kh] self-tests: ring %d, attention merge %d (%.2f ms)\n", r, a,
            std::chrono::duration<double, std::milli>(std::chrono::steady_clock::now() - t0).count());
  return KH_OK;
}

}
```

kuiperllama_amd/csrc/kh_model_step.hip:

```cpp
#include <stdio.h>
#include <stdlib.h>
#include <string.h>

#include <vector>

#include "kh_fused.h"
#include "kh_fused_ring.h"
#include "kh_sample.h"
#include "kh_model_internal.h"

namespace khm {

kh_model::Shape pick_shape(bool quant, int pairs, int M, int max_split, const char* env, int wg,
                           int wg_max, bool many_waves, bool u3) {
  kh_model::Shape sh;
  sh.wg = wg;
  if (const char* ov = env ? dbg(env) : nullptr) {
    int sp = 0, u = 0, g = 0, w = wg;
    const int nf = sscanf(ov, "%d,%d,%d,%d", &sp, &u, &g, &w);
    if (nf >= 3 && (sp == 1 || sp == 2 || sp == 4) && sp <= max_split &&
        (u == 2 || u == 4 || u == 8 || (quant && u3 && u == 3)) && !(quant && u == 8) && g >= 1 && g <= 4096 &&
        (w == 256 || (w == 512 && wg_max >= 512))) {
      sh.split = sp;
      sh.u = u;
      sh.grid = g;
      sh.wg = w;
      return sh;
    }
    fprintf(stderr, "[kh] %s=\"%s\" rejected (split <= %d, u 2/4%s%s, grid 1..4096, wg 256%s): heuristic shape\n",
            env, ov, max_split, quant ? "" : "/8", quant && u3 ? "/3" : "", wg_max >= 512 ? "/512" : "");
  }
  const int elem = quant ? 1 : 4;
  const int min_bytes = quant ? 4096 : 8192;
  const long pair_bytes = 2L * M * elem;
  const int target_waves = pair_bytes >= 16384 ? 4096 : 2048;
  while (sh.split < max_split && pairs * sh.split < target_waves &&
         pair_bytes / (sh.split * 2) >= min_bytes)
    sh.split *= 2;
  const int Mc = quant ? M / 16 : M / 4;
  const int per_lane = ((Mc + sh.split - 1) / sh.split + KH_WAVE - 1) / KH_WAVE;
  if (quant) {
    sh.u = per_lane > 4 ? 2 : (per_lane >= 3 ? 4 : 2);
    if (u3 && per_lane > 4 && per_lane <= 6) sh.u = 3;
  } else {
    sh.u = per_lane >= 8 ? 8 : (per_lane >= 3 ? 4 : 2);
  }
  const int ppw = (wg / KH_WAVE) / sh.split;
  const int need = (pairs + ppw - 1) / ppw;
  long cap = (long)(0.75 * (double)pairs * (double)pair_bytes / ((double)M * 4.0));
  const long cap_hi = 1024L * KH_WG / wg, cap_lo = 256L * KH_WG / wg;
  if (cap > cap_hi) cap = cap_hi;
  if (cap < cap_lo) cap = cap_lo;
  if (need <= cap) {
    sh.grid = need;
  } else {
    const int wpw = wg / KH_WAVE;
    const int pref_lo[4] = {8, 12, 16, 4}, pref_hi[4] = {16, 12, 8, 4};
    long best_cost = -1;
    for (int wv : (many_waves ? pref_hi : pref_lo)) {
      if (wv == 4 && best_cost >= 0) break;
      if (wv % wpw) continue;
      const long g = 256L * (wv / wpw);
      if (g > cap) continue;
      const long cost = g * ((need + g - 1) / g);
      if (best_cost < 0 || cost < best_cost) {
        best_cost = cost;
        sh.grid = (int)g;
      }
    }
    if (best_cost < 0) sh.grid = (int)cap;
  }
  return sh;
}

#define KH_L3(KERNEL, Q, UU, MV, GRID, LDS, STREAM, ARGS)                                     \
  do {                                                                                     \
    launch_log(#KERNEL "<" #Q "," #UU "," #MV ">");                                        \
    hipLaunchKernelGGL((KERNEL<Q, UU, MV>), dim3(GRID), dim3(kh_launch_wg), LDS, STREAM, ARGS); \
  } while (0)
#define KH_L4(KERNEL, Q, UU, MV, SP, GRID, LDS, STREAM, ARGS)                                     \
  do {                                                                                         \
    launch_log(#KERNEL "<" #Q "," #UU "," #MV "," #SP ">");                                    \
    hipLaunchKernelGGL((KERNEL<Q, UU, MV, SP>), dim3(GRID), dim3(kh_launch_wg), LDS, STREAM, ARGS); \
  } while (0)
#define KH_LRING(KERNEL, R, MV, GRID, LDS, STREAM, ARGS)                                   \
  do {                                                                                  \
    launch_log(#KERNEL "<" #R "," #MV ",false>");                                       \
    hipLaunchKernelGGL((KERNEL<R, MV, false>), dim3(GRID), dim3(KH_WG), LDS, STREAM, ARGS); \
  } while (0)
#define KH_SEL_MV3(KERNEL, Q, UU, MV, ...)                  \
  do {                                                      \
    if ((MV) == 4)                                          \
      KH_L3(KERNEL, Q, UU, 4, __VA_ARGS__);                 \
    else if ((MV) == 2)                                     \
      KH_L3(KERNEL, Q, UU, 2, __VA_ARGS__);                 \
    else if ((MV) == 1)                                     \
      KH_L3(KERNEL, Q, UU, 1, __VA_ARGS__);                 \
    else                                                    \
      KH_L3(KERNEL, Q, UU, 0, __VA_ARGS__);                 \
  } while (0)
#define KH_SEL_SP4(KERNEL, Q, UU, MV, SP, ...)              \
  do {                                                      \
    if ((SP) == 4)                                          \
      KH_L4(KERNEL, Q, UU, MV, 4, __VA_ARGS__);             \
    else if ((SP) == 2)                                     \
      KH_L4(KERNEL, Q, UU, MV, 2, __VA_ARGS__);             \
    else                                                    \
      KH_L4(KERNEL, Q, UU, MV, 1, __VA_ARGS__);             \
  } while (0)
#define KH_SEL_SP2(KERNEL, Q, UU, MV, SP, ...)              \
  do {                                                      \
    if ((SP) == 2)                                          \
      KH_L4(KERNEL, Q, UU, MV, 2, __VA_ARGS__);             \
    else                                                    \
      KH_L4(KERNEL, Q, UU, MV, 1, __VA_ARGS__);             \
  } while (0)
#define KH_SEL_MV4S(SELSP, KERNEL, Q, UU, MV, SP, ...)      \
  do {                                                      \
    if ((MV) == 4)                                          \
      SELSP(KERNEL, Q, UU, 4, SP, __VA_ARGS__);             \
    else if ((MV) == 2)                                     \
      SELSP(KERNEL, Q, UU, 2, SP, __VA_ARGS__);             \
    else if ((MV) == 1)                                     \
      SELSP(KERNEL, Q, UU, 1, SP, __VA_ARGS__);             \
    else                                                    \
      SELSP(KERNEL, Q, UU, 0, SP, __VA_ARGS__);             \
  } while (0)
#define KH_SEL_MV4(KERNEL, Q, UU, MV, SP, ...) KH_SEL_MV4S(KH_SEL_SP4, KERNEL, Q, UU, MV, SP, __VA_ARGS__)
#define KH_SEL_MV4Q(KERNEL, Q, UU, MV, SP, ...) KH_SEL_MV4S(KH_SEL_SP2, KERNEL, Q, UU, MV, SP, __VA_ARGS__)
#define KH_SEL_MV4X(KERNEL, Q, UU, MV, SP, ...)             \
  do {                                                      \
    if ((MV) == 6)                                          \
      KH_SEL_SP4(KERNEL, Q, UU, 6, SP, __VA_ARGS__);        \
    else                                                    \
      KH_SEL_MV4(KERNEL, Q, UU, MV, SP, __VA_ARGS__);       \
  } while (0)
#define KH_SEL_U(SEL, KERNEL, QUANT, U, ...)                \
  do {                                                      \
    if (QUANT) {                                            \
      if ((U) >= 4)                                         \
        SEL(KERNEL, true, 4, __VA_ARGS__);                  \
      else                                                  \
        SEL(KERNEL, true, 2, __VA_ARGS__);                  \
    } else {                                                \
      if ((U) >= 8)                                         \
        SEL(KERNEL, false, 8, __VA_ARGS__);                 \
      else if ((U) >= 4)                                    \
        SEL(KERNEL, false, 4, __VA_ARGS__);                 \
      else                                                  \
        SEL(KERNEL, false, 2, __VA_ARGS__);                 \
    }                                                       \
  } while (0)
#define KH_DISPATCH3(KERNEL, QUANT, U, MV, GRID, LDS, STREAM, ARGS) \
  KH_SEL_U(KH_SEL_MV3, KERNEL, QUANT, U, MV, GRID, LDS, STREAM, ARGS)
#define KH_DISPATCH4(KERNEL, QUANT, U, MV, SP, GRID, LDS, STREAM, ARGS) \
  KH_SEL_U(KH_SEL_MV4, KERNEL, QUANT, U, MV, SP, GRID, LDS, STREAM, ARGS)
#define KH_DISPATCH4X(KERNEL, QUANT, U, MV, SP, GRID, LDS, STREAM, ARGS) \
  KH_SEL_U(KH_SEL_MV4X, KERNEL, QUANT, U, MV, SP, GRID, LDS, STREAM, ARGS)
#define KH_DISPATCH4Q(KERNEL, QUANT, U, MV, SP, GRID, LDS, STREAM, ARGS) \
  KH_SEL_U(KH_SEL_MV4Q, KERNEL, QUANT, U, MV, SP, GRID, LDS, STREAM, ARGS)

KhQkvArgs fill_qkv(kh_model* m, int l) {
  const kh_config& c = m->cfg;
  const LayerW& W = m->layers[l];
  KhQkvArgs a;
  a.x = m->x;
  a.att_norm = W.att_norm;
  a.wq = W.wq;
  a.wk = W.wk;
  a.wv = W.wv;
  a.q_out = m->q;
  a.kcache_layer = m->kcache + (size_t)l * c.cache_len * c.kv_dim;
  a.vcache_layer = m->vcache + (size_t)l * c.cache_len * c.kv_dim;
  a.d_pos = m->d_pos;
  a.sin_cache = m->sin_cache;
  a.cos_cache = m->cos_cache;
  a.dim = c.dim;
  a.kv_dim = c.kv_dim;
  a.head_size = c.head_size;
  a.rope_mode = c.rope_mode;
  a.gshift = m->gshift;
  a.eps = c.rms_eps;
  return a;
}
void launch_qkv(kh_model* m, int l) {
  const kh_config& c = m->cfg;
  const KhQkvArgs a = fill_qkv(m, l);
  const bool qn = c.is_quant;
  const int kh_launch_wg = m->sh_qkv.wg;
  KH_DISPATCH4Q(k_qkv, qn, m->sh_qkv.u, kh_stage_maxv(c.dim, kh_launch_wg), m->sh_qkv.split, m->sh_qkv.grid,
               fused_lds_bytes(qn, c.dim), m->stream, a);
}
KhAttnArgs fill_attn(kh_model* m, int l) {
  const kh_config& c = m->cfg;
  KhAttnArgs a;
  a.q = m->q;
  a.kcache_layer = m->kcache + (size_t)l * c.cache_len * c.kv_dim;
  a.vcache_layer = m->vcache + (size_t)l * c.cache_len * c.kv_dim;
  a.out = m->att;
  a.d_pos = m->d_pos;
  a.kv_dim = c.kv_dim;
  a.kv_mul = c.kv_mul;
  a.head_size = c.head_size;
  a.kv_heads = c.kv_head_num;
  a.nsplit = m->attn_ns;
  a.ws = m->attn_ws;
  a.ws_stride = m->attn_ws_stride;
  a.nsplit_g = m->step_var != 0 ? 0 : m->attn_ns_g;
  a.t_long = m->attn_t_long;
  a.ts_shift = m->attn_ts_shift;
  a.defer = m->step_var == 1 ? 1 : 0;
  a.fenced = m->attn_fenced ? 1 : 0;
  a.tok_stride = 0;
  a.ws_tok_bytes = 0;
  return a;
}
int attn_group_lanes(const kh_config& c) {
  int G = 1;
  while (G < c.head_size / 4) G <<= 1;
  return G < 16 ? 16 : G;
}
void launch_attn(kh_model* m, int l) {
  const kh_config& c = m->cfg;
  const KhAttnArgs a = fill_attn(m, l);
  const int wg = m->attn_wg;
  if (c.head_size > 32)
    launch_attn_decode(a, 0, wg, m->stream);
  else
    hipLaunchKernelGGL(k_attn_generic, dim3(c.head_num), dim3(wg),
                       attn_lds_bytes(c.head_size, wg), m->stream, a);
}
KhGemvResArgs fill_wo(kh_model* m, int l) {
  const kh_config& c = m->cfg;
  KhGemvResArgs a;
  a.vec = m->att;
  a.w = m->layers[l].wo;
  a.x = m->x;
  a.M = c.dim;
  a.K = c.dim;
  a.gshift = m->gshift;
  return a;
}
#define KH_L5C(Q, UU, MV, SP, GRID, LDS, STREAM, ARGS)                                            \
  do {                                                                                          \
    launch_log("k_wo_comb<" #Q "," #UU "," #MV "," #SP ">");                                    \
    hipLaunchKernelGGL((k_wo_comb<Q, UU, MV, SP>), dim3(GRID), dim3(kh_launch_wg), LDS, STREAM, ARGS); \
  } while (0)
#define KH_SEL_SP5C(Q, UU, MV, SP, ...)                     \
  do {                                                      \
    if ((SP) == 4)                                          \
      KH_L5C(Q, UU, MV, 4, __VA_ARGS__);                    \
    else if ((SP) == 2)                                     \
      KH_L5C(Q, UU, MV, 2, __VA_ARGS__);                    \
    else                                                    \
      KH_L5C(Q, UU, MV, 1, __VA_ARGS__);                    \
  } while (0)
#define KH_SEL_MV5C(KERNEL_UNUSED, Q, UU, MV, SP, ...)      \
  do {                                                      \
    if ((MV) == 2)                                          \
      KH_SEL_SP5C(Q, UU, 2, SP, __VA_ARGS__);               \
    else                                                    \
      KH_SEL_SP5C(Q, UU, 4, SP, __VA_ARGS__);               \
  } while (0)
void launch_wo(kh_model* m, int l) {
  const kh_config& c = m->cfg;
  const bool qn = c.is_quant;
  const int kh_launch_wg = m->sh_wo.wg;
  if (m->step_var == 1) {
    KhWoCombArgs a;
    a.g = fill_wo(m, l);
    const AttnSplitWs ws = attn_ws_carve(m->attn_ws, c.head_num, c.head_size, m->attn_ws_stride);
    a.cb.ml = ws.ml;
    a.cb.o = ws.o;
    a.cb.d_pos = m->d_pos;
    a.cb.ns = m->attn_ns;
    a.cb.ts_shift = m->attn_ts_shift;
    a.cb.nsw = m->attn_ws_stride;
    a.cb.heads = c.head_num;
    a.cb.hs = c.head_size;
    const int mv = c.dim <= 2 * 4 * kh_launch_wg ? 2 : 4;
    KH_SEL_U(KH_SEL_MV5C, k_wo_comb, qn, m->sh_wo.u, mv, m->sh_wo.split, m->sh_wo.grid,
             comb_lds_bytes(qn, c.dim, c.head_num), m->stream, a);
    return;
  }
  const KhGemvResArgs a = fill_wo(m, l);
  KH_DISPATCH4(k_gemv_res, qn, m->sh_wo.u, kh_stage_maxv(c.dim, kh_launch_wg), m->sh_wo.split, m->sh_wo.grid,
               fused_lds_bytes(qn, c.dim), m->stream, a);
}
void launch_ffn13(kh_model* m, int l) {
  const kh_config& c = m->cfg;
  const LayerW& W = m->layers[l];
  KhFfn13Args a;
  a.x = m->x;
  a.ffn_norm = W.ffn_norm;
  a.w1 = W.w1;
  a.w3 = W.w3;
  a.h = m->h1;
  a.dim = c.dim;
  a.hidden = c.hidden_dim;
  a.gshift = m->gshift;
  a.eps = c.rms_eps;
  const bool qn = c.is_quant;
  if (m->ring.ffn_r == 2) {
    KH_LRING(k_ffn13_ring, 2, 4, m->ring.ffn_grid, ring_lds_bytes(c.dim, false, KH_WAVES_PER_WG, 2), m->stream, a);
    return;
  }
  const int kh_launch_wg = m->sh_ffn.wg;
  KH_DISPATCH3(k_ffn13, qn, m->sh_ffn.u, kh_stage_maxv(c.dim, kh_launch_wg), m->sh_ffn.grid,
               fused_lds_bytes(qn, c.dim), m->stream, a);
}
void launch_w2(kh_model* m, int l) {
  const kh_config& c = m->cfg;
  KhGemvResArgs a;
  a.vec = m->h1;
  a.w = m->layers[l].w2;
  a.x = m->x;
  a.M = c.hidden_dim;
  a.K = c.dim;
  a.gshift = m->gshift;
  const bool qn = c.is_quant;
  const int kh_launch_wg = m->sh_w2.wg;
  const int mv = kh_stage_maxv(c.hidden_dim, kh_launch_wg);
  if (qn && m->sh_w2.u == 3) {
    KH_SEL_MV4X(k_gemv_res, true, 3, mv, m->sh_w2.split, m->sh_w2.grid, fused_lds_bytes(qn, c.hidden_dim), m->stream, a);
    return;
  }
  KH_DISPATCH4X(k_gemv_res, qn, m->sh_w2.u, mv, m->sh_w2.split, m->sh_w2.grid,
                fused_lds_bytes(qn, c.hidden_dim), m->stream, a);
}
void launch_cls(kh_model* m) {
  const kh_config& c = m->cfg;
  KhClsArgs a;
  a.x = m->x;
  a.final_norm = m->final_norm;
  a.wcls = m->cls;
  a.logits = m->logits;
  a.part_val = m->part_val;
  a.part_idx = m->part_idx;
  a.dim = c.dim;
  a.vocab = c.vocab_size;
  a.gshift = m->gshift;
  a.eps = c.rms_eps;
  const bool qn = c.is_quant;
  if (m->ring.cls_r == 2) {
    KH_LRING(k_cls_ring, 2, 4, m->ring.cls_grid, ring_lds_bytes(c.dim, false, KH_WAVES_PER_WG, 2), m->stream, a);
    return;
  }
  const int kh_launch_wg = m->sh_cls.wg;
  KH_DISPATCH3(k_cls, qn, m->sh_cls.u, kh_stage_maxv(c.dim, kh_launch_wg), m->sh_cls.grid, cls_lds_bytes(qn, c.dim),
               m->stream, a);
}
void launch_sample(kh_model* m, int advance, int n_forced) {
  const kh_config& c = m->cfg;
  KhSampleArgs a;
  a.part_val = m->part_val;
  a.part_idx = m->part_idx;
  a.nparts = m->nparts;
  a.forced = n_forced > 0 ? m->d_forced : nullptr;
  a.n_forced = n_forced;
  a.words = m->d_words;
  a.words_cap = m->seq_cap;
  a.d_next = m->d_next;
  a.d_token = m->d_token;
  a.d_pos = m->d_pos;
  a.tok_emb = m->tok_emb;
  a.x = m->x;
  a.dim = c.dim;
  a.vocab = c.vocab_size;
  a.advance = advance;
  if (m->samp_on) {
    KhSampleTopArgs t;
    t.logits = m->logits;
    t.part_val = m->part_val;
    t.nparts = m->nparts;
    t.params = m->d_samp;
    t.forced = a.forced;
    t.n_forced = a.n_forced;
    t.words = a.words;
    t.words_cap = a.words_cap;
    t.d_next = a.d_next;
    t.d_token = a.d_token;
    t.d_pos = a.d_pos;
    t.tok_emb = a.tok_emb;
    t.x = a.x;
    t.dim = a.dim;
    t.vocab = a.vocab;
    t.advance = advance;
    launch_log("k_sample_topp");
    hipLaunchKernelGGL(k_sample_topp, dim3(1), dim3(KH_SAMP_THREADS), 0, m->stream, t);
    return;
  }
  hipLaunchKernelGGL(k_sample, dim3(1), dim3(KH_WG), 0, m->stream, a);
}

int step_variant(const kh_model* m, int pos_lo, int pos_hi) {
  (void)pos_lo;
  if (pos_hi < KH_ATTN_MIN_TS) return 0;
  if (pos_hi + 1 >= m->attn_t_long) return 0;
  if (m->attn_defer && attn_active_splits(pos_hi, m->attn_ns, m->attn_ts_shift) <= m->attn_defer_max) return 1;
  return m->attn_ns_g > 0 ? 2 : 0;
}
void launch_step_fused(kh_model* m, int advance, int n_forced, hipEvent_t* ev, int variant) {
  m->step_var = variant;
  int e = 0;
  auto mark = [&]() {
    if (ev) (void)hipEventRecord(ev[e++], m->stream);
  };
  mark();
  for (int l = 0; l < m->cfg.layer_num; ++l) {
    launch_qkv(m, l);
    mark();
    launch_attn(m, l);
    mark();
    launch_wo(m, l);
    mark();
    launch_ffn13(m, l);
    mark();
    launch_w2(m, l);
    mark();
  }
  launch_cls(m);
  mark();
  launch_sample(m, advance, n_forced);
  mark();
}

int launch_step_unfused(kh_model* m, int pos) {
  const kh_config& c = m->cfg;
  void* s = (void*)m->stream;
  int rc;
#define KH_TRY(x)          \
  if ((rc = (x)) != KH_OK) \
  return rc
  auto lin = [&](const KhLin& L, const float* in, float* out, int M, int K) -> int {
    int r = c.is_quant ? kh_matmul_q8(in, (const int8_t*)L.w, L.scales, c.group_size, out, M, K, s)
                       : kh_matmul_f32(in, (const float*)L.w, out, M, K, 1.f, s);
    if (r == KH_OK && L.bias) r = kh_add_f32(out, L.bias, out, K, s);
    return r;
  };
  for (int l = 0; l < c.layer_num; ++l) {
    const LayerW& W = m->layers[l];
    float* krow = m->kcache + ((size_t)l * c.cache_len + pos) * c.kv_dim;
    float* vrow = m->vcache + ((size_t)l * c.cache_len + pos) * c.kv_dim;
    KH_TRY(kh_rmsnorm_f32(m->x, W.att_norm, m->rms, c.dim, c.rms_eps, s));
    KH_TRY(lin(W.wq, m->rms, m->q, c.dim, c.dim));
    KH_TRY(lin(W.wk, m->rms, krow, c.dim, c.kv_dim));
    KH_TRY(lin(W.wv, m->rms, vrow, c.dim, c.kv_dim));
    KH_TRY(kh_rope_f32(c.dim, c.kv_dim, c.head_size, m->q, krow, nullptr, pos, m->sin_cache,
                       m->cos_cache, c.rope_mode, s));
    KH_TRY(kh_mha_f32(nullptr, pos, c.head_num, l, c.cache_len, c.kv_dim, c.kv_mul, c.head_size,
                      m->att, m->q, m->score, m->kcache, m->vcache, s));
    KH_TRY(lin(W.wo, m->att, m->q , c.dim,
               c.dim));
    KH_TRY(kh_add_f32(m->x, m->q, m->x, c.dim, s));
    KH_TRY(kh_rmsnorm_f32(m->x, W.ffn_norm, m->rms, c.dim, c.rms_eps, s));
    KH_TRY(lin(W.w1, m->rms, m->h1, c.dim, c.hidden_dim));
    KH_TRY(lin(W.w3, m->rms, m->h3, c.dim, c.hidden_dim));
    KH_TRY(kh_swiglu_f32(m->h1, m->h3, m->h1, c.hidden_dim, s));
    KH_TRY(lin(W.w2, m->h1, m->w2o, c.hidden_dim, c.dim));
    KH_TRY(kh_add_f32(m->x, m->w2o, m->x, c.dim, s));
  }
  KH_TRY(kh_rmsnorm_f32(m->x, m->final_norm, m->x, c.dim, c.rms_eps, s));
  KH_TRY(lin(m->cls, m->x, m->logits, c.dim, c.vocab_size));
  if (m->samp_on) {
    KH_TRY(kh_sample_f32(m->logits, c.vocab_size, &m->samp, pos, 1, m->d_next, s));
  } else {
    KH_TRY(kh_argmax_f32(m->logits, c.vocab_size, m->d_next, s));
  }
#undef KH_TRY
  return KH_OK;
}

void set_state(kh_model* m, int token, int pos) {
  hipLaunchKernelGGL(k_set_state, dim3(1), dim3(KH_WG), 0, m->stream, token, pos, m->d_token,
                     m->d_pos, m->tok_emb, m->x, m->cfg.dim);
}

int ensure_pinned_words(kh_model* m, int n) {
  for (auto& e : m->ev_chunk)
    if (!e && hipEventCreateWithFlags(&e, hipEventDisableTiming) != hipSuccess) return (int)hipErrorUnknown;
  if (n <= m->pin_cap) return KH_OK;
  if (m->h_words_pin) (void)hipHostFree(m->h_words_pin);
  m->h_words_pin = nullptr;
  m->pin_cap = 0;
  if (hipHostMalloc((void**)&m->h_words_pin, sizeof(int32_t) * (size_t)n, hipHostMallocDefault) !=
      hipSuccess)
    return (int)hipErrorUnknown;
  m->pin_cap = n;
  return KH_OK;
}

int ensure_seq_cap(kh_model* m, int n) {
  if (n <= m->seq_cap) return KH_OK;
  if (m->d_forced) (void)hipFree(m->d_forced);
  if (m->d_words) (void)hipFree(m->d_words);
  if (m->h_forced_pin) (void)hipHostFree(m->h_forced_pin);
  m->d_forced = m->d_words = nullptr;
  m->h_forced_pin = nullptr;
  m->seq_cap = 0;
  int rc;
  if (hipHostMalloc((void**)&m->h_forced_pin, sizeof(int32_t) * ((size_t)n + 1), hipHostMallocDefault) != hipSuccess)
    return (int)hipErrorUnknown;
  if ((rc = dalloc(&m->d_forced, (size_t)n + 1)) != KH_OK) return rc;
  if ((rc = dalloc(&m->d_words, (size_t)n + 1)) != KH_OK) return rc;
  KH_CHECK_HIP(hipMemsetAsync(m->d_forced, 0xFF, sizeof(int32_t) * ((size_t)n + 1), m->stream));
  m->forced_hwm = 0;
  m->forced_in_flight = false;
  m->seq_cap = n;
  destroy_step_graphs(m);
  return KH_OK;
}
void destroy_step_graphs(kh_model* m) {
  for (auto& per_sampler : m->sg)
    for (int v = 0; v < KH_STEP_VARIANTS; ++v)
      for (int k = 0; k < 4; ++k) {
        kh_model::StepGraph& sg = per_sampler[v][k];
        if (sg.e) (void)hipGraphExecDestroy(sg.e);
        if (sg.g) (void)hipGraphDestroy(sg.g);
        sg = kh_model::StepGraph{};
      }
}

int capture_steps(kh_model* m, int n_forced, int steps, int variant, hipGraph_t* g, hipGraphExec_t* ge) {
  KH_CHECK_HIP(hipStreamBeginCapture(m->stream, hipStreamCaptureModeThreadLocal));
  for (int i = 0; i < steps; ++i) launch_step_fused(m, 1, n_forced, nullptr, variant);
  hipError_t e = hipStreamEndCapture(m->stream, g);
  if (e != hipSuccess) return (int)e;
  KH_CHECK_HIP(hipGraphInstantiate(ge, *g, nullptr, nullptr, 0));
  return KH_OK;
}
int step_graph_n(kh_model* m, int n_forced, int variant, int nsteps, hipGraphExec_t* out) {
  if (variant < 0 || variant >= KH_STEP_VARIANTS) return KH_ERR_INVALID_ARG;
  const int k = nsteps == 1 ? 0 : nsteps == 2 ? 1 : nsteps == 4 ? 2 : nsteps == KH_GRAPH_STEPS ? 3 : -1;
  if (k < 0) return KH_ERR_INVALID_ARG;
  kh_model::StepGraph& sg = m->sg[m->samp_on ? 1 : 0][variant][k];
  if (!sg.e) {
    const int rc = capture_steps(m, n_forced, nsteps, variant, &sg.g, &sg.e);
    if (rc != KH_OK) return rc;
    (void)hipGraphUpload(sg.e, m->stream);
  }
  *out = sg.e;
  return KH_OK;
}
int step_graph(kh_model* m, int n_forced, int variant, bool steps8, hipGraphExec_t* out) {
  return step_graph_n(m, n_forced, variant, steps8 ? KH_GRAPH_STEPS : 1, out);
}

void plan_decode_shapes(bool quant, int dim, int hidden_dim, int kv_dim, int vocab_size,
                        kh_model::Shape (&out)[5]) {
  out[0] = pick_shape(quant, (dim + 2 * kv_dim) / 2, dim, 2, "KH_SHAPE_QKV", KH_WG, KH_WG_MAX);
  out[1] = pick_shape(quant, dim / 2, dim, 4, "KH_SHAPE_WO", KH_WG, KH_WG_MAX, true);
  out[2] = pick_shape(quant, hidden_dim, dim, 1, "KH_SHAPE_FFN", KH_WG, KH_WG_MAX);
  out[3] = pick_shape(quant, dim / 2, hidden_dim, 4, "KH_SHAPE_W2", KH_WG_MAX, KH_WG_MAX, true, true);
  out[4] = pick_shape(quant, (vocab_size + 1) / 2, dim, 1, "KH_SHAPE_CLS", quant ? KH_WG : KH_WG_MAX, KH_WG_MAX);
}

void plan_ring(bool quant, int dim, int hidden_dim, int vocab_size, int group_size, kh_model::RingPlan* out) {
  *out = kh_model::RingPlan();
  if (!quant || dbg_off("KH_RING")) return;
  if (dim % 16 != 0 || !kh_stage_fits4(dim, KH_WG)) return;
  if (group_size < 16 || (group_size & (group_size - 1)) != 0 || dim % group_size != 0) return;
  if (ring_lds_bytes(dim, false, KH_WAVES_PER_WG, 2) > 64 * 1024) return;
  auto grid_of = [](int items) {
    const int need = (items + KH_WAVES_PER_WG - 1) / KH_WAVES_PER_WG;
    return need < 512 ? need : 512;
  };
  if (!dbg("KH_SHAPE_FFN")) {
    out->ffn_r = 2;
    out->ffn_grid = grid_of(hidden_dim);
  }
  if (!dbg("KH_SHAPE_CLS")) {
    out->cls_r = 2;
    out->cls_grid = grid_of((vocab_size + 1) / 2);
  }
}
extern "C" int kh_plan_decode_ring(int32_t dim, int32_t hidden_dim, int32_t vocab_size, int32_t is_quant,
                                   int32_t group_size, int32_t* out4) {
  if (!out4 || dim <= 0 || hidden_dim <= 0 || vocab_size <= 0) return KH_ERR_INVALID_ARG;
  kh_model::RingPlan r;
  plan_ring(is_quant != 0, dim, hidden_dim, vocab_size, group_size, &r);
  out4[0] = r.ffn_r;
  out4[1] = r.ffn_grid;
  out4[2] = r.cls_r;
  out4[3] = r.cls_grid;
  return KH_OK;
}

extern "C" int kh_plan_decode_shapes(int32_t dim, int32_t hidden_dim, int32_t kv_dim, int32_t vocab_size,
                                     int32_t is_quant, int32_t* out20) {
  if (!out20 || dim <= 0 || hidden_dim <= 0 || kv_dim <= 0 || vocab_size <= 0) return KH_ERR_INVALID_ARG;
  kh_model::Shape sh[5];
  plan_decode_shapes(is_quant != 0, dim, hidden_dim, kv_dim, vocab_size, sh);
  for (int i = 0; i < 5; ++i) {
    out20[4 * i] = sh[i].split;
    out20[4 * i + 1] = sh[i].u;
    out20[4 * i + 2] = sh[i].grid;
    out20[4 * i + 3] = sh[i].wg;
  }
  return KH_OK;
}

int configure_step_kernels(kh_model* m) {
  const kh_config& c = m->cfg;
  const size_t lds_need = fused_lds_bytes(c.is_quant, c.hidden_dim);
  if (lds_need > 160 * 1024) return KH_ERR_UNSUPPORTED;
  if (lds_need > 64 * 1024) {
    const int v = (int)lds_need;
#define KH_ATTR(Q, UU, SP)                                                                     \
  (void)hipFuncSetAttribute((const void*)k_gemv_res<Q, UU, 0, SP>,                             \
                            hipFuncAttributeMaxDynamicSharedMemorySize, v);                    \
  (void)hipFuncSetAttribute((const void*)k_gemv_res<Q, UU, 6, SP>,                             \
                            hipFuncAttributeMaxDynamicSharedMemorySize, v)
    KH_ATTR(false, 8, 1); KH_ATTR(false, 8, 2); KH_ATTR(false, 8, 4);
    KH_ATTR(false, 4, 1); KH_ATTR(false, 4, 2); KH_ATTR(false, 4, 4);
    KH_ATTR(false, 2, 1); KH_ATTR(false, 2, 2); KH_ATTR(false, 2, 4);
    KH_ATTR(true, 4, 1); KH_ATTR(true, 4, 2); KH_ATTR(true, 4, 4);
    KH_ATTR(true, 3, 1); KH_ATTR(true, 3, 2); KH_ATTR(true, 3, 4);
    KH_ATTR(true, 2, 1); KH_ATTR(true, 2, 2); KH_ATTR(true, 2, 4);
#undef KH_ATTR
  }
  return KH_OK;
}

}
using namespace khm;

extern "C" int kh_model_predict(kh_model* m, int32_t token, int32_t pos, int32_t is_prompt,
                                int32_t exec, int32_t* h_next) {
  if (!m || !h_next) return KH_ERR_INVALID_ARG;
  const kh_config& c = m->cfg;
  if (token < 0 || token >= c.vocab_size || pos < 0 || pos >= c.cache_len) return KH_ERR_RANGE;
  KH_CHECK_HIP(hipSetDevice(m->opts.device));
  int rc = kv_ensure(m, pos + 1);
  if (rc != KH_OK) return rc;
  set_state(m, token, pos);
  if (exec == KH_EXEC_UNFUSED) {
    rc = launch_step_unfused(m, pos);
  } else if (exec == KH_EXEC_FUSED || exec == KH_EXEC_GRAPH) {
    launch_step_fused(m, 0, 0, nullptr, step_variant(m, pos, pos));
    rc = kh_launch_status();
  } else {
    return KH_ERR_INVALID_ARG;
  }
  if (rc != KH_OK) return rc;
  int32_t next = -1;
  KH_CHECK_HIP(hipMemcpyAsync(&next, m->d_next, sizeof(int32_t), hipMemcpyDeviceToHost, m->stream));
  KH_CHECK_HIP(hipStreamSynchronize(m->stream));
  *h_next = is_prompt ? -1 : next;
  return KH_OK;
}

extern "C" int kh_model_set_sampling(kh_model* m, const kh_sampling* p) {
  if (p && !kh_sampling_valid(p)) return KH_ERR_INVALID_ARG;
  if (!m) return KH_ERR_INVALID_ARG;
  const kh_sampling greedy{0.f, 0, 1.f, 0};
  const kh_sampling want = p ? *p : greedy;
  const bool on = !kh_sampling_greedy(&want);
  if (on) {
    KH_CHECK_HIP(hipSetDevice(m->opts.device));
    if (!m->d_samp) KH_CHECK_HIP(hipMalloc((void**)&m->d_samp, sizeof(KhSampParams)));
    const KhSampParams dp = kh_samp_params(&want);
    KH_CHECK_HIP(hipMemcpyAsync(m->d_samp, &dp, sizeof(dp), hipMemcpyHostToDevice, m->stream));
    KH_CHECK_HIP(hipStreamSynchronize(m->stream));
  }
  m->samp = want;
  m->samp_on = on;
  return KH_OK;
}
extern "C" int kh_model_get_sampling(const kh_model* m, kh_sampling* out) {
  if (!m || !out) return KH_ERR_INVALID_ARG;
  *out = m->samp;
  return KH_OK;
}

extern "C" int kh_model_generate(kh_model* m, const int32_t* h_prompt, int32_t n_prompt,
                                 int32_t total_steps, int32_t exec, int32_t* h_words,
                                 int32_t* n_words, float* h_elapsed_ms) {
  return kh_model_generate_until(m, h_prompt, n_prompt, total_steps, exec, nullptr, 0, h_words,
                                 n_words, h_elapsed_ms);
}

namespace {
inline bool is_stop(int32_t t, const int32_t* stop, int n_stop) {
  for (int i = 0; i < n_stop; ++i)
    if (stop[i] == t) return true;
  return false;
}
}

extern "C" int kh_model_generate_until(kh_model* m, const int32_t* h_prompt, int32_t n_prompt,
                                       int32_t total_steps, int32_t exec, const int32_t* h_stop,
                                       int32_t n_stop, int32_t* h_words, int32_t* n_words,
                                       float* h_elapsed_ms) {
  if (!m || !h_prompt || n_prompt <= 0 || total_steps <= 0 || !h_words || !n_words ||
      n_stop < 0 || (n_stop > 0 && !h_stop))
    return KH_ERR_INVALID_ARG;
  const kh_config& c = m->cfg;
  if (total_steps > c.cache_len) return KH_ERR_RANGE;
  for (int i = 0; i < n_prompt; ++i)
    if (h_prompt[i] < 0 || h_prompt[i] >= c.vocab_size) return KH_ERR_RANGE;
  KH_CHECK_HIP(hipSetDevice(m->opts.device));
  int rc;
  *n_words = 0;

  if (exec == KH_EXEC_UNFUSED) {
    KH_CHECK_HIP(hipEventRecord(m->ev0, m->stream));
    int pos = 0, next = -1, nw = 0;
    while (pos < total_steps) {
      const bool is_prompt = pos < n_prompt - 1;
      const int tok = pos <= n_prompt - 1 ? h_prompt[pos] : next;
      int got = -1;
      if ((rc = kh_model_predict(m, tok, pos, is_prompt, KH_EXEC_UNFUSED, &got)) != KH_OK) return rc;
      if (!is_prompt && is_stop(got, h_stop, n_stop)) break;
      next = is_prompt ? h_prompt[pos + 1] : got;
      h_words[nw++] = next;
      pos += 1;
    }
    KH_CHECK_HIP(hipEventRecord(m->ev1, m->stream));
    KH_CHECK_HIP(hipEventSynchronize(m->ev1));
    if (h_elapsed_ms) KH_CHECK_HIP(hipEventElapsedTime(h_elapsed_ms, m->ev0, m->ev1));
    *n_words = nw;
    return KH_OK;
  }
  if (exec != KH_EXEC_GRAPH && exec != KH_EXEC_FUSED) return KH_ERR_INVALID_ARG;

  if ((rc = ensure_seq_cap(m, total_steps)) != KH_OK) return rc;
  if ((rc = kv_ensure(m, total_steps < KH_GRAPH_STEPS ? KH_GRAPH_STEPS : total_steps)) != KH_OK) return rc;
  if ((rc = ensure_pinned_words(m, m->seq_cap)) != KH_OK) return rc;
  {
    if (m->forced_in_flight) KH_CHECK_HIP(hipStreamSynchronize(m->stream));
    const int nf = total_steps + 1 <= m->seq_cap + 1 ? total_steps + 1 : m->seq_cap + 1;
    for (int i = 0; i < nf; ++i) m->h_forced_pin[i] = i < n_prompt ? h_prompt[i] : -1;
    m->forced_in_flight = true;
    KH_CHECK_HIP(hipMemcpyAsync(m->d_forced, m->h_forced_pin, (size_t)nf * sizeof(int32_t), hipMemcpyHostToDevice,
                                m->stream));
    if (m->forced_hwm > nf)
      KH_CHECK_HIP(hipMemsetAsync(m->d_forced + nf, 0xFF, (size_t)(m->forced_hwm - nf) * sizeof(int32_t), m->stream));
    m->forced_hwm = nf;
  }
  const int n_forced = m->seq_cap + 1;
  if (exec == KH_EXEC_GRAPH) {
    bool fresh[4] = {false, false, false, false};
    hipGraphExec_t ge = nullptr;
    for (int n = 1, k = 0; n <= KH_GRAPH_STEPS; n *= 2, ++k) {
      fresh[k] = m->sg[m->samp_on ? 1 : 0][0][k].e == nullptr;
      if ((rc = step_graph_n(m, n_forced, 0, n, &ge)) != KH_OK) return rc;
    }
    bool dry = false;
    if (c.cache_len >= KH_GRAPH_STEPS && m->seq_cap >= KH_GRAPH_STEPS)
      for (int k = 3; k >= 0; --k)
        if (fresh[k]) {
          set_state(m, h_prompt[0], 0);
          KH_CHECK_HIP(hipGraphLaunch(m->sg[m->samp_on ? 1 : 0][0][k].e, m->stream));
          dry = true;
        }
    if (dry) KH_CHECK_HIP(hipStreamSynchronize(m->stream));
  }

  int start = 0;
  KH_CHECK_HIP(hipEventRecord(m->ev0, m->stream));
  if (n_prompt - 1 >= 2 && n_prompt - 1 < total_steps) {
    const char* e = dbg("KH_PREFILL");
    bool want_gemm = n_prompt - 1 >= KH_PG_MIN_TOKENS && !(m->opts.flags & KH_FLAG_PREFILL_EXACT), want_gemv = true;
    if (e && *e) {
      if (!strcmp(e, "0") || !strcmp(e, "token")) want_gemm = want_gemv = false;
      else if (!strcmp(e, "gemv")) want_gemm = false;
      else if (!strcmp(e, "gemm")) want_gemm = true;
      else return KH_ERR_INVALID_ARG;
    }
    if (want_gemm && pg_supported(m)) {
      if ((rc = kh_model_prefill_gemm(m, h_prompt, n_prompt - 1, 0)) != KH_OK) return rc;
      start = n_prompt - 1;
      m->first_mode = 2;
    } else if (want_gemv && prefill_supported(m)) {
      if ((rc = kh_model_prefill(m, h_prompt, n_prompt - 1, 0)) != KH_OK) return rc;
      start = n_prompt - 1;
      m->first_mode = 1;
    }
  }
  m->first_pos = -1;
  if (start > 0) {
    if (!m->first_logits) KH_CHECK_HIP(hipMalloc(&m->first_logits, sizeof(float) * (size_t)c.vocab_size));
    m->first_pos = start;
  }
  set_state(m, h_prompt[start], start);
  auto launch_chunk = [&](int s) -> int {
    if (exec == KH_EXEC_GRAPH) {
      int n = KH_GRAPH_STEPS;
      while (n > total_steps - s) n >>= 1;
      const bool keep = s == start && start > 0;
      if (keep) n = 1;
      hipGraphExec_t ge = nullptr;
      if (step_graph_n(m, n_forced, step_variant(m, s, s + n - 1), n, &ge) != KH_OK) return -1;
      if (hipGraphLaunch(ge, m->stream) != hipSuccess) return -1;
      if (keep && hipMemcpyAsync(m->first_logits, m->logits, sizeof(float) * (size_t)c.vocab_size,
                                 hipMemcpyDeviceToDevice, m->stream) != hipSuccess)
        return -1;
      return n;
    }
    launch_step_fused(m, 1, n_forced, nullptr, step_variant(m, s, s));
    if (s == start && start > 0 &&
        hipMemcpyAsync(m->first_logits, m->logits, sizeof(float) * (size_t)c.vocab_size, hipMemcpyDeviceToDevice,
                       m->stream) != hipSuccess)
      return -1;
    return 1;
  };
  int n_out = total_steps;
  if (n_stop == 0) {
    for (int s = start; s < total_steps;) {
      const int n = launch_chunk(s);
      if (n < 0) return (int)hipErrorUnknown;
      s += n;
    }
    KH_CHECK_HIP(hipEventRecord(m->ev1, m->stream));
    if ((rc = kh_launch_status()) != KH_OK) return rc;
    KH_CHECK_HIP(hipMemcpyAsync(m->h_words_pin, m->d_words, sizeof(int32_t) * total_steps,
                                hipMemcpyDeviceToHost, m->stream));
    KH_CHECK_HIP(hipStreamSynchronize(m->stream));
    memcpy(h_words, m->h_words_pin, sizeof(int32_t) * (size_t)total_steps);
    for (int i = 0; i < start; ++i) h_words[i] = h_prompt[i + 1];
  } else {
    struct Chunk { int s0, n; };
    Chunk infl[2];
    int n_infl = 0, head = 0, launched = start, stop_at = -1;
    for (int i = 0; i < start; ++i) m->h_words_pin[i] = h_prompt[i + 1];
    auto fail = [&](int code) -> int {
      (void)hipStreamSynchronize(m->stream);
      return code;
    };
#define KH_CHECK_DRAIN(expr)                          \
  do {                                                \
    hipError_t _e = (expr);                           \
    if (_e != hipSuccess) return fail((int)_e);       \
  } while (0)
    while (stop_at < 0 && (launched < total_steps || n_infl > 0)) {
      while (launched < total_steps && n_infl < 2) {
        const int n = launch_chunk(launched);
        if (n < 0) return fail((int)hipErrorUnknown);
        const int slot = (head + n_infl) & 1;
        KH_CHECK_DRAIN(hipMemcpyAsync(m->h_words_pin + launched, m->d_words + launched,
                                      sizeof(int32_t) * n, hipMemcpyDeviceToHost, m->stream));
        KH_CHECK_DRAIN(hipEventRecord(m->ev_chunk[slot], m->stream));
        infl[slot] = {launched, n};
        launched += n;
        ++n_infl;
      }
      KH_CHECK_DRAIN(hipEventSynchronize(m->ev_chunk[head]));
      const Chunk c0 = infl[head];
      for (int s = c0.s0; s < c0.s0 + c0.n; ++s)
        if (s >= n_prompt - 1 && is_stop(m->h_words_pin[s], h_stop, n_stop)) {
          stop_at = s;
          break;
        }
      if (stop_at >= 0) {
        KH_CHECK_DRAIN(hipEventRecord(m->ev1, m->stream));
      }
      head ^= 1;
      --n_infl;
    }
    if (stop_at < 0) KH_CHECK_DRAIN(hipEventRecord(m->ev1, m->stream));
    if ((rc = kh_launch_status()) != KH_OK) return fail(rc);
#undef KH_CHECK_DRAIN
    KH_CHECK_HIP(hipStreamSynchronize(m->stream));
    n_out = stop_at >= 0 ? stop_at : total_steps;
    memcpy(h_words, m->h_words_pin, sizeof(int32_t) * (size_t)n_out);
  }
  m->forced_in_flight = false;
  if (h_elapsed_ms) KH_CHECK_HIP(hipEventElapsedTime(h_elapsed_ms, m->ev0, m->ev1));
  *n_words = n_out;
  return KH_OK;
}
```

kuiperllama_amd/model.py:

```python
from __future__ import annotations

import ctypes as C
from typing import List, Optional, Sequence, Tuple

import numpy as np
import torch

from . import _ffi, binfmt
from ._ffi import KH_EXEC_FUSED, KH_EXEC_GRAPH, KH_EXEC_UNFUSED

EXEC = {"graph": KH_EXEC_GRAPH, "fused": KH_EXEC_FUSED, "unfused": KH_EXEC_UNFUSED}



def _opts(spec: binfmt.ModelSpec, max_seq_len: int, device: int, flags: int = 0) -> _ffi.ModelOpts:
    return _ffi.ModelOpts(spec.family, int(spec.quant), spec.rope_mode, spec.rope_theta,
                          spec.rms_eps, max_seq_len, device, flags)


class KuiperModel:

    def __init__(self, handle: int, spec: binfmt.ModelSpec, keepalive=None):
        self._h = C.c_void_p(handle)
        self.spec = spec
        self._keep = keepalive
        cfg = _ffi.Config()
        _ffi.check(_ffi.lib().kh_model_get_config(self._h, C.byref(cfg)), "kh_model_get_config")
        self.cfg = cfg

    @classmethod
    def from_file(cls, path: str, spec: binfmt.ModelSpec, max_seq_len: int = 0,
                  device: int = 0, flags: int = 0) -> "KuiperModel":
        _ffi.sync_env()
        h = C.c_void_p()
        o = _opts(spec, max_seq_len, device, flags)
        _ffi.check(_ffi.lib().kh_model_create_from_file(path.encode(), C.byref(o), C.byref(h)),
                   "kh_model_create_from_file")
        return cls(h.value, spec)

    @classmethod
    def from_host_image(cls, image: np.ndarray, spec: binfmt.ModelSpec, max_seq_len: int = 0,
                        device: int = 0, flags: int = 0) -> "KuiperModel":
        assert image.dtype == np.uint8 and image.flags["C_CONTIGUOUS"]
        _ffi.sync_env()
        h = C.c_void_p()
        o = _opts(spec, max_seq_len, device, flags)
        _ffi.check(_ffi.lib().kh_model_create_from_host_image(image.ctypes.data, image.size,
                                                              C.byref(o), C.byref(h)),
                   "kh_model_create_from_host_image")
        return cls(h.value, spec)

    @classmethod
    def from_device_image(cls, image: torch.Tensor, spec: binfmt.ModelSpec, max_seq_len: int = 0,
                          device: int = 0, flags: int = 0) -> "KuiperModel":
        assert image.is_cuda and image.dtype == torch.uint8
        if image.device.index != device:
            raise ValueError(f"image lives on cuda:{image.device.index} but the model is created on "
                             f"device {device}: kernels would dereference another GPU's pointers")
        hb = spec.header_bytes()
        header = np.frombuffer(image[:32].cpu().numpy().tobytes(), dtype=np.int32).copy()
        if (image.data_ptr() + hb) % 16 == 0:
            weights = image[hb:]
            keep = image
        else:
            weights = torch.empty(image.numel() - hb, dtype=torch.uint8, device=image.device)
            weights.copy_(image[hb:])
            keep = weights
        torch.cuda.synchronize()
        _ffi.sync_env()
        h = C.c_void_p()
        o = _opts(spec, max_seq_len, device, flags)
        hdr = (C.c_int32 * 8)(*header.tolist()[:8])
        _ffi.check(_ffi.lib().kh_model_create_from_device_weights(hdr, weights.data_ptr(),
                                                                  weights.numel(), C.byref(o),
                                                                  C.byref(h)),
                   "kh_model_create_from_device_weights")
        return cls(h.value, spec, keepalive=keep)

    def close(self):
        if getattr(self, "_h", None) is not None and self._h.value:
            _ffi.lib().kh_model_destroy(self._h)
            self._h = C.c_void_p()
        self._keep = None

    def __del__(self):
        try:
            self.close()
        except Exception:
            pass

    def predict(self, token: int, pos: int, is_prompt: bool = False, exec: str = "fused") -> int:
        nxt = C.c_int32(-1)
        _ffi.check(_ffi.lib().kh_model_predict(self._h, token, pos, int(is_prompt), EXEC[exec],
                                               C.byref(nxt)), "kh_model_predict")
        return int(nxt.value)

    def set_sampling(self, temperature: float = 0.0, top_k: int = 0, top_p: float = 1.0, seed: int = 0) -> None:
        _ffi.check(_ffi.lib().kh_model_set_sampling(self._h, _ffi.sampling(temperature, top_k, top_p, seed)),
                   "kh_model_set_sampling")

    @property
    def sampling(self) -> dict:
        s = _ffi.Sampling()
        _ffi.check(_ffi.lib().kh_model_get_sampling(self._h, C.byref(s)), "kh_model_get_sampling")
        return s.as_dict()

    def logits(self) -> np.ndarray:
        out = np.empty(self.cfg.vocab_size, np.float32)
        _ffi.check(_ffi.lib().kh_model_get_logits(self._h, out.ctypes.data), "kh_model_get_logits")
        return out

    def kv_bytes(self) -> Tuple[int, int]:
        r, c = C.c_int64(0), C.c_int64(0)
        _ffi.check(_ffi.lib().kh_model_kv_bytes(self._h, C.byref(r), C.byref(c)), "kh_model_kv_bytes")
        return int(r.value), int(c.value)

    def kv_cache_ptrs(self) -> Tuple[int, int]:
        k, v = C.c_void_p(), C.c_void_p()
        _ffi.check(_ffi.lib().kh_model_get_kv(self._h, C.byref(k), C.byref(v)), "kh_model_get_kv")
        return k.value, v.value

    def read_kv(self, layer: int, row0: int, nrows: int):
        k = np.empty((nrows, self.cfg.kv_dim), np.float32)
        v = np.empty((nrows, self.cfg.kv_dim), np.float32)
        _ffi.check(_ffi.lib().kh_model_read_kv(self._h, layer, row0, nrows, k.ctypes.data,
                                               v.ctypes.data), "kh_model_read_kv")
        return k, v

    def write_kv(self, layer: int, row0: int, k: np.ndarray, v: np.ndarray) -> None:
        k = np.ascontiguousarray(k, np.float32)
        v = np.ascontiguousarray(v, np.float32)
        assert k.shape == v.shape and k.ndim == 2 and k.shape[1] == self.cfg.kv_dim
        _ffi.check(_ffi.lib().kh_model_write_kv(self._h, layer, row0, k.shape[0], k.ctypes.data,
                                                v.ctypes.data), "kh_model_write_kv")

    def write_kv_device(self, layer: int, row0: int, k: torch.Tensor, v: torch.Tensor) -> None:
        assert k.is_cuda and v.is_cuda and k.dtype == v.dtype == torch.float32
        assert k.is_contiguous() and v.is_contiguous() and k.shape == v.shape
        assert k.dim() == 2 and k.shape[1] == self.cfg.kv_dim
        torch.cuda.current_stream(k.device).synchronize()
        _ffi.check(_ffi.lib().kh_model_write_kv(self._h, layer, row0, k.shape[0], k.data_ptr(),
                                                v.data_ptr()), "kh_model_write_kv")

    def generate(self, prompt: Sequence[int], total_steps: int, exec: str = "graph",
                 stop: Optional[Sequence[int]] = None) -> Tuple[List[int], float]:
        _ffi.sync_env()
        pr = (C.c_int32 * len(prompt))(*[int(t) for t in prompt])
        st = list(stop or [])
        sp = (C.c_int32 * max(len(st), 1))(*[int(t) for t in st])
        words = (C.c_int32 * total_steps)()
        n = C.c_int32(0)
        ms = C.c_float(0.0)
        _ffi.check(_ffi.lib().kh_model_generate_until(self._h, pr, len(prompt), total_steps,
                                                      EXEC[exec], sp, len(st), words,
                                                      C.byref(n), C.byref(ms)),
                   "kh_model_generate_until")
        return list(words[: n.value]), float(ms.value)

    def first_sample(self) -> Optional[dict]:
        fs = _ffi.FirstSample()
        rc = _ffi.lib().kh_model_first_sample(self._h, C.byref(fs))
        if rc == -2:
            return None
        _ffi.check(rc, "kh_model_first_sample")
        return {"pos": fs.pos, "prefill_mode": {1: "gemv", 2: "gemm"}.get(fs.prefill_mode, str(fs.prefill_mode)),
                "top1_id": fs.top1_id, "top2_id": fs.top2_id, "top1": float(fs.top1), "top2": float(fs.top2),
                "margin": float(fs.top1) - float(fs.top2)}

    def prefill(self, tokens: Sequence[int], pos0: int = 0) -> None:
        t = (C.c_int32 * len(tokens))(*[int(x) for x in tokens])
        _ffi.check(_ffi.lib().kh_model_prefill(self._h, t, len(tokens), pos0), "kh_model_prefill")
        torch.cuda.synchronize()

    def prefill_gemm(self, tokens: Sequence[int], pos0: int = 0) -> None:
        _ffi.sync_env()
        t = (C.c_int32 * len(tokens))(*[int(x) for x in tokens])
        _ffi.check(_ffi.lib().kh_model_prefill_gemm(self._h, t, len(tokens), pos0),
                   "kh_model_prefill_gemm")
        torch.cuda.synchronize()

    PREFILL_MODES = {"token": 0, "gemv": 1, "gemm": 2}

    def time_prefill(self, tokens: Sequence[int], pos0: int = 0, mode: str = "gemm") -> float:
        _ffi.sync_env()
        t = (C.c_int32 * len(tokens))(*[int(x) for x in tokens])
        ms = C.c_float(0.0)
        _ffi.check(_ffi.lib().kh_model_time_prefill(self._h, t, len(tokens), pos0,
                                                    self.PREFILL_MODES[mode], C.byref(ms)),
                   "kh_model_time_prefill")
        return float(ms.value)

    def time_step(self, pos: int, reps: int = 9) -> List[float]:
        us = (C.c_float * reps)()
        _ffi.check(_ffi.lib().kh_model_time_step(self._h, pos, reps, us), "kh_model_time_step")
        return [float(v) for v in us]

    def profile_kernels(self, pos: int, reps: int = 8):
        out = {}
        for i in range(_ffi.KH_NUM_KCLASS):
            us = C.c_float(0.0)
            _ffi.check(_ffi.lib().kh_model_profile_kernel(self._h, i, pos, reps, C.byref(us)),
                       "kh_model_profile_kernel")
            out[_ffi.lib().kh_kclass_name(i).decode()] = float(us.value)
        return out

    def profile_kernel(self, name: str, pos: int, reps: int = 8) -> float:
        names = [_ffi.lib().kh_kclass_name(i).decode() for i in range(_ffi.KH_NUM_KCLASS)]
        us = C.c_float(0.0)
        _ffi.check(_ffi.lib().kh_model_profile_kernel(self._h, names.index(name), pos, reps,
                                                      C.byref(us)), "kh_model_profile_kernel")
        return float(us.value)

    def profile_step(self, start_pos: int, n_steps: int):
        avg = (C.c_float * _ffi.KH_NUM_KCLASS)()
        cnt = (C.c_int32 * _ffi.KH_NUM_KCLASS)()
        _ffi.check(_ffi.lib().kh_model_profile_step(self._h, start_pos, n_steps, avg, cnt),
                   "kh_model_profile_step")
        names = [_ffi.lib().kh_kclass_name(i).decode() for i in range(_ffi.KH_NUM_KCLASS)]
        return {n: {"avg_us": float(avg[i]), "launches_per_step": int(cnt[i])}
                for i, n in enumerate(names)}

    @property
    def load_ms(self) -> float:
        return float(_ffi.lib().kh_model_get_load_ms(self._h))

    @property
    def stream(self) -> int:
        return int(_ffi.lib().kh_model_stream(self._h) or 0)
```

Baseline: 1033 tokens/s.

## Screen classifier with bf16 weight copy and exact rescoring of top candidates

Adds a bf16 copy of the classifier weights plus per-row error bounds, built at load time. During greedy generate, a screening kernel computes bf16 logits with rigorous lower and upper bounds, keeps the top candidates per block, and a sampler kernel rescores only those candidates in fp32. It falls back to the full classifier when the bounds cannot separate the winner. This halves classifier weight traffic in the common case, at the cost of extra memory, a load-time build and a self-test.

```diff
diff --git a/include/kuiper_hip.h b/include/kuiper_hip.h
--- a/include/kuiper_hip.h
+++ b/include/kuiper_hip.h
@@ -103,6 +103,7 @@
 #define KH_FLAG_ATTN_MERGE_IN_LAUNCH 1
 #define KH_FLAG_ATTN_MERGE_FENCED 2
 #define KH_FLAG_PREFILL_EXACT 4
+#define KH_FLAG_NO_CLS_SCREEN 8
 
 typedef struct kh_config {
   int32_t dim, hidden_dim, layer_num, head_num, kv_head_num, vocab_size, seq_len;
@@ -134,6 +135,7 @@
 int kh_model_predict(kh_model* m, int32_t token, int32_t pos, int32_t is_prompt, int32_t exec,
                      int32_t* h_next);
 int kh_model_get_logits(kh_model* m, float* h_logits);
+int kh_model_cls_screen_info(kh_model* m, int64_t* out8);
 int kh_model_get_kv(kh_model* m, float** d_kcache, float** d_vcache);
 int kh_model_kv_bytes(const kh_model* m, int64_t* reserved, int64_t* committed);
 int kh_model_read_kv(kh_model* m, int32_t layer, int32_t row0, int32_t nrows, float* h_k,
diff --git a/kuiperllama_amd/_ffi.py b/kuiperllama_amd/_ffi.py
--- a/kuiperllama_amd/_ffi.py
+++ b/kuiperllama_amd/_ffi.py
@@ -15,7 +15,7 @@
     "kh_argmax_f32_host", "kh_sample_f32", "kh_sample_f32_host", "kh_softmax_f32", "kh_scale_f32", "kh_scale_sum_f32",
     "kh_model_create_from_file", "kh_model_create_from_host_image",
     "kh_model_create_from_device_weights", "kh_model_destroy", "kh_model_get_config",
-    "kh_model_stream", "kh_model_get_load_ms", "kh_model_predict", "kh_model_get_logits", "kh_model_get_kv", "kh_model_kv_bytes", "kh_model_read_kv", "kh_model_write_kv",
+    "kh_model_stream", "kh_model_get_load_ms", "kh_model_predict", "kh_model_get_logits", "kh_model_cls_screen_info", "kh_model_get_kv", "kh_model_kv_bytes", "kh_model_read_kv", "kh_model_write_kv",
     "kh_spm_create_from_file", "kh_spm_create_from_memory", "kh_spm_destroy", "kh_spm_vocab_size",
     "kh_spm_bos_id", "kh_spm_eos_id", "kh_spm_unk_id", "kh_spm_encode", "kh_spm_decode",
     "kh_bpe_create_from_file", "kh_bpe_create_from_memory", "kh_bpe_destroy", "kh_bpe_vocab_size",
@@ -32,6 +32,7 @@
 KH_FLAG_ATTN_MERGE_IN_LAUNCH = 1
 KH_FLAG_ATTN_MERGE_FENCED = 2
 KH_FLAG_PREFILL_EXACT = 4
+KH_FLAG_NO_CLS_SCREEN = 8
 
 
 class KhError(RuntimeError):
@@ -127,6 +128,7 @@
     L.kh_model_get_load_ms.restype = _f32
     L.kh_model_predict.argtypes = [_vp, _i32, _i32, _i32, _i32, C.POINTER(_i32)]
     L.kh_model_get_logits.argtypes = [_vp, _vp]
+    L.kh_model_cls_screen_info.argtypes = [_vp, C.POINTER(_i64)]
     L.kh_model_get_kv.argtypes = [_vp, C.POINTER(_vp), C.POINTER(_vp)]
     L.kh_model_kv_bytes.argtypes = [_vp, C.POINTER(_i64), C.POINTER(_i64)]
     L.kh_model_read_kv.argtypes = [_vp, _i32, _i32, _i32, _vp, _vp]
diff --git a/kuiperllama_amd/build.py b/kuiperllama_amd/build.py
--- a/kuiperllama_amd/build.py
+++ b/kuiperllama_amd/build.py
@@ -9,9 +9,9 @@
 CSRC = os.path.join(_PKG, "csrc")
 LIB_DIR = os.path.join(_PKG, "lib")
 LIB_PATH = os.path.join(LIB_DIR, "libkuiper_hip.so")
-SOURCES = ["kh_ops.hip", "kh_model_load.hip", "kh_model_step.hip", "kh_model_prefill.hip", "kh_model_profile.hip", "kh_model_selftest.hip",
+SOURCES = ["kh_ops.hip", "kh_model_load.hip", "kh_model_step.hip", "kh_model_prefill.hip", "kh_model_profile.hip", "kh_model_selftest.hip", "kh_model_screen.hip",
            "kh_tokenizer.cpp", "kh_bpe.cpp", "kh_debug.cpp"]
-HEADERS = ["kh_common.h", "kh_gemv.h", "kh_attn.h", "kh_fused.h", "kh_q8ring.h", "kh_fused_ring.h", "kh_prefill.h", "kh_gemm.h", "kh_pattn.h", "kh_sample.h", "kh_unicode_tables.h",
+HEADERS = ["kh_common.h", "kh_gemv.h", "kh_attn.h", "kh_fused.h", "kh_q8ring.h", "kh_fused_ring.h", "kh_prefill.h", "kh_gemm.h", "kh_pattn.h", "kh_sample.h", "kh_cls_screen.h", "kh_unicode_tables.h",
            "kh_model_internal.h",
            "../../include/kuiper_hip.h"]
 ARCH = "gfx950"
diff --git a/kuiperllama_amd/csrc/kh_cls_screen.h b/kuiperllama_amd/csrc/kh_cls_screen.h
--- /dev/null
+++ b/kuiperllama_amd/csrc/kh_cls_screen.h
@@ -0,0 +1,447 @@
+#pragma once
+#include "kh_fused.h"
+
+#define KH_SCR_C 4
+#define KH_SCR_CAND 32
+#define KH_SCR_MERGE_WORDS (2 + 2 * KH_SCR_C)
+
+__device__ __forceinline__ int bf_slot(int f, int M8) { return (f & 1) * (M8 + 1) + (f >> 1); }
+static inline size_t kh_bf_lds_bytes(int M) { return (size_t)2 * (size_t)(M / 8 + 1) * 16; }
+static inline size_t cls_screen_lds_bytes(int M) {
+  return kh_bf_lds_bytes(M) + (size_t)(2 * KH_WAVES_MAX + KH_WAVES_MAX * KH_SCR_MERGE_WORDS) * sizeof(float);
+}
+
+__device__ __forceinline__ float bf_lo(int d) { return __builtin_bit_cast(float, d << 16); }
+__device__ __forceinline__ float bf_hi(int d) { return __builtin_bit_cast(float, d & (int)0xffff0000u); }
+__device__ __forceinline__ float dot8_bf16(i32x4 q, f32x4 xa, f32x4 xb, float acc) {
+  acc = __builtin_fmaf(bf_lo(q.x), xa.x, acc);
+  acc = __builtin_fmaf(bf_hi(q.x), xa.y, acc);
+  acc = __builtin_fmaf(bf_lo(q.y), xa.z, acc);
+  acc = __builtin_fmaf(bf_hi(q.y), xa.w, acc);
+  acc = __builtin_fmaf(bf_lo(q.z), xb.x, acc);
+  acc = __builtin_fmaf(bf_hi(q.z), xb.y, acc);
+  acc = __builtin_fmaf(bf_lo(q.w), xb.z, acc);
+  acc = __builtin_fmaf(bf_hi(q.w), xb.w, acc);
+  return acc;
+}
+
+template <int U>
+struct RegsBf16 {
+  i32x4 v0[U], v1[U];
+};
+struct RowsBf16 {
+  const i32x4* w0;
+  const i32x4* w1;
+};
+template <int U>
+struct GemvBf16 {
+  static constexpr int kU = U;
+  using Regs = RegsBf16<U>;
+  using Rows = RowsBf16;
+  int Mc;
+  __device__ __forceinline__ explicit GemvBf16(int M) : Mc(M >> 3) {}
+  __device__ __forceinline__ Rows rows(const uint16_t* base, int r0, int r1, int M) const {
+    return Rows{(const i32x4*)(base + (size_t)r0 * M), (const i32x4*)(base + (size_t)r1 * M)};
+  }
+  __device__ __forceinline__ void load(Regs& r, const Rows& rw, int c0, int lim, int lane) const {
+#pragma unroll
+    for (int u = 0; u < U; ++u) {
+      const int idx = c0 + u * KH_WAVE + lane;
+      const int cidx = idx < lim ? idx : 0;
+      r.v0[u] = ld_nt(rw.w0 + cidx);
+      r.v1[u] = ld_nt(rw.w1 + cidx);
+      __builtin_amdgcn_sched_barrier(0);
+    }
+  }
+  __device__ __forceinline__ void fma(const Regs& r, const f32x4* xs, int c0, int lim, int lane, float& a0,
+                                      float& a1) const {
+#pragma unroll
+    for (int u = 0; u < U; ++u) {
+      const int idx = c0 + u * KH_WAVE + lane;
+      const bool in = idx < lim;
+      const int ci = in ? idx : 0;
+      f32x4 xa = xs[ci], xb = xs[Mc + 1 + ci];
+      xa.x = in ? xa.x : 0.f;
+      xa.y = in ? xa.y : 0.f;
+      xa.z = in ? xa.z : 0.f;
+      xa.w = in ? xa.w : 0.f;
+      xb.x = in ? xb.x : 0.f;
+      xb.y = in ? xb.y : 0.f;
+      xb.z = in ? xb.z : 0.f;
+      xb.w = in ? xb.w : 0.f;
+      a0 = dot8_bf16(r.v0[u], xa, xb, a0);
+      a1 = dot8_bf16(r.v1[u], xa, xb, a1);
+    }
+  }
+};
+
+__device__ __forceinline__ uint32_t bf16_rne(float f) {
+  const uint32_t u = __builtin_bit_cast(uint32_t, f);
+  if ((u & 0x7fffffffu) > 0x7f800000u) return (u >> 16) | 0x40u;
+  return (u + 0x7fffu + ((u >> 16) & 1u)) >> 16;
+}
+__device__ __forceinline__ double wave_sum_f64(double v) {
+#pragma unroll
+  for (int off = 32; off > 0; off >>= 1) v += __shfl_xor(v, off, KH_WAVE);
+  return v;
+}
+static __global__ __launch_bounds__(KH_WG) void k_cls_bf16_build(const float* __restrict__ w, uint32_t* __restrict__ out,
+                                                                 float* __restrict__ err, int dim, int vocab,
+                                                                 double gam2) {
+  const int lane = threadIdx.x & 63, wave = threadIdx.x >> 6;
+  const int half = dim >> 1;
+  for (int row = blockIdx.x * KH_WAVES_PER_WG + wave; row < vocab; row += gridDim.x * KH_WAVES_PER_WG) {
+    const float2* src = (const float2*)(w + (size_t)row * dim);
+    uint32_t* dst = out + (size_t)row * half;
+    double d2 = 0.0, w2 = 0.0, b2 = 0.0;
+    for (int i = lane; i < half; i += KH_WAVE) {
+      const float2 v = src[i];
+      const uint32_t lo = bf16_rne(v.x), hi = bf16_rne(v.y);
+      dst[i] = lo | (hi << 16);
+      const float bx = __builtin_bit_cast(float, lo << 16), by = __builtin_bit_cast(float, hi << 16);
+      const double ex = (double)v.x - (double)bx, ey = (double)v.y - (double)by;
+      d2 += ex * ex + ey * ey;
+      w2 += (double)v.x * (double)v.x + (double)v.y * (double)v.y;
+      b2 += (double)bx * (double)bx + (double)by * (double)by;
+    }
+    d2 = wave_sum_f64(d2);
+    w2 = wave_sum_f64(w2);
+    b2 = wave_sum_f64(b2);
+    if (lane == 0) {
+      const double e = (sqrt(d2) + gam2 * (sqrt(w2) + sqrt(b2))) * (1.0 + 1e-9);
+      float f = (float)e;
+      if ((double)f < e) f = nextafterf(f, INFINITY);
+      if (!(e < (double)INFINITY)) f = INFINITY;
+      err[row] = f;
+    }
+  }
+}
+
+struct ScrTop {
+  float lb, spill;
+  float u[KH_SCR_C];
+  int i[KH_SCR_C];
+  __device__ __forceinline__ void init() {
+    lb = -INFINITY;
+    spill = -INFINITY;
+#pragma unroll
+    for (int k = 0; k < KH_SCR_C; ++k) {
+      u[k] = -INFINITY;
+      i[k] = -1;
+    }
+  }
+  __device__ __forceinline__ void insert(float ub, int idx) {
+#pragma unroll
+    for (int k = 0; k < KH_SCR_C; ++k) {
+      const bool sw = ub > u[k];
+      const float tu = sw ? u[k] : ub;
+      const int ti = sw ? i[k] : idx;
+      u[k] = sw ? ub : u[k];
+      i[k] = sw ? idx : i[k];
+      ub = tu;
+      idx = ti;
+    }
+    spill = fmaxf(spill, idx >= 0 ? ub : -INFINITY);
+  }
+};
+
+struct KhClsScreenArgs {
+  const float* x;
+  const float* final_norm;
+  const uint16_t* wbf;
+  const float* err;
+  float* x_save;
+  float* p_lb;
+  float* p_spill;
+  float* p_ub;
+  int32_t* p_idx;
+  float* dbg_lb;
+  float* dbg_ub;
+  int dim, vocab;
+  float eps;
+};
+template <int U, int MAXV>
+__global__ __launch_bounds__(KH_WG_MAX, 4) void k_cls_screen(const KhClsScreenArgs a) {
+  extern __shared__ __attribute__((aligned(16))) char smem_raw[];
+  f32x4* xs = (f32x4*)smem_raw;
+  const int dim = a.dim, vocab = a.vocab, M8 = dim >> 3;
+  float* red = (float*)(xs + 2 * (M8 + 1));
+  float* mg = red + 2 * KH_WAVES_MAX;
+  const int lane = threadIdx.x & 63, wave = threadIdx.x >> 6;
+  const uint16_t* const wbf = a.wbf;
+  const float* const err = a.err;
+  float* const dbg_lb = a.dbg_lb;
+  float* const dbg_ub = a.dbg_ub;
+  float* const x_save = a.x_save;
+  const float eps = a.eps;
+  const GemvBf16<U> g(dim);
+  Stager<true, false, MAXV> st(a.x, a.final_norm, dim);
+  ScrTop top;
+  top.init();
+  auto r1_of = [&](int p) __attribute__((always_inline)) { return 2 * p + 1 < vocab ? 2 * p + 1 : 2 * p; };
+  auto pair = [&](int p) __attribute__((always_inline)) { return g.rows(wbf, 2 * p, r1_of(p), dim); };
+  struct Aux {
+    float e0, e1;
+  };
+  auto pre = [&](int p) __attribute__((always_inline)) { return Aux{err[2 * p], err[r1_of(p)]}; };
+  float rs = 1.f, cb = 0.f;
+  auto track = [&](float s, float e, int r) __attribute__((always_inline)) {
+    const float av = s * rs;
+    const float b = __builtin_fmaf(cb, e, fabsf(av) * 0x1p-18f) + 1e-30f;
+    const bool ok = fabsf(av) < INFINITY && b < INFINITY;
+    const float lb = ok ? av - b : -INFINITY, ub = ok ? av + b : INFINITY;
+    top.lb = fmaxf(top.lb, lb);
+    top.insert(ub, r);
+    if (dbg_lb && lane == 0) {
+      dbg_lb[r] = lb;
+      dbg_ub[r] = ub;
+    }
+  };
+  auto epi = [&](int p, float s0, float s1, const Aux& x) __attribute__((always_inline)) {
+    const int r0 = 2 * p, r1 = r1_of(p);
+    track(s0, x.e0, r0);
+    if (r1 != r0) track(s1, x.e1, r1);
+  };
+  auto finish = [&]() __attribute__((always_inline)) {
+    const int M4 = dim >> 2;
+    float ss = 0.f, gg = 0.f;
+#pragma unroll
+    for (int v = 0; v < MAXV; ++v) {
+      const int i = threadIdx.x + v * kh_wg();
+      const bool in = i < M4;
+      const float t = fma4(st.xv[v], st.xv[v], 0.f);
+      ss += in ? t : 0.f;
+      f32x4 gv = st.xv[v];
+      gv.x = st.wv[v].x * gv.x;
+      gv.y = st.wv[v].y * gv.y;
+      gv.z = st.wv[v].z * gv.z;
+      gv.w = st.wv[v].w * gv.w;
+      const float t2 = fma4(gv, gv, 0.f);
+      gg += in ? t2 : 0.f;
+      if (in) {
+        xs[bf_slot(i, M8)] = gv;
+        if (blockIdx.x == 0) ((f32x4*)x_save)[i] = st.xv[v];
+      }
+    }
+    gg = wave_sum(gg);
+    if (lane == 0) red[KH_WAVES_MAX + wave] = gg;
+    rs = stage_rs(ss, dim, eps, red);
+    const int n = kh_nwaves();
+    float r = 0.f;
+#pragma unroll
+    for (int w = 0; w < KH_WAVES_MAX; ++w) r += w < n ? red[KH_WAVES_MAX + (w < n ? w : 0)] : 0.f;
+    cb = rs * sqrtf(r) * (1.f + 0x1p-17f);
+  };
+  gemv_pairs<1, false>(g, xs, (vocab + 1) >> 1, lane, nullptr, pair, pre,
+                                [&]() __attribute__((always_inline)) { st.issue(); }, finish, epi);
+  if (lane == 0) {
+    float* q = mg + wave * KH_SCR_MERGE_WORDS;
+    q[0] = top.lb;
+    q[1] = top.spill;
+#pragma unroll
+    for (int k = 0; k < KH_SCR_C; ++k) {
+      q[2 + k] = top.u[k];
+      q[2 + KH_SCR_C + k] = __builtin_bit_cast(float, top.i[k]);
+    }
+  }
+  __syncthreads();
+  if (threadIdx.x == 0) {
+    for (int w = 1, nw = kh_nwaves(); w < nw; ++w) {
+      const float* q = mg + w * KH_SCR_MERGE_WORDS;
+      top.lb = fmaxf(top.lb, q[0]);
+      top.spill = fmaxf(top.spill, q[1]);
+#pragma unroll
+      for (int k = 0; k < KH_SCR_C; ++k) top.insert(q[2 + k], __builtin_bit_cast(int, q[2 + KH_SCR_C + k]));
+    }
+    a.p_lb[blockIdx.x] = top.lb;
+    a.p_spill[blockIdx.x] = top.spill;
+#pragma unroll
+    for (int k = 0; k < KH_SCR_C; ++k) {
+      a.p_ub[blockIdx.x * KH_SCR_C + k] = top.u[k];
+      a.p_idx[blockIdx.x * KH_SCR_C + k] = top.i[k];
+    }
+  }
+}
+
+struct KhSampleScreenArgs {
+  const float* p_lb;
+  const float* p_spill;
+  const float* p_ub;
+  const int32_t* p_idx;
+  int nsp;
+  const float* x_save;
+  const float* final_norm;
+  const float* wcls;
+  float eps;
+  float* ov_val;
+  int32_t* ov_idx;
+  uint32_t* ticket;
+  int32_t* stats;
+  const int32_t* forced;
+  int n_forced;
+  int32_t* words;
+  int words_cap;
+  int32_t* d_next;
+  int32_t* d_token;
+  int32_t* d_pos;
+  const float* tok_emb;
+  float* x;
+  int dim, vocab;
+  int advance;
+};
+__device__ __forceinline__ void screen_tail(const KhSampleScreenArgs& a, int idx, int* s_next) {
+  if (threadIdx.x == 0) {
+    const int pos = *a.d_pos;
+    int feed = idx;
+    int reported = idx;
+    if (a.forced && pos + 1 < a.n_forced && a.forced[pos + 1] >= 0) {
+      feed = a.forced[pos + 1];
+      reported = -1;
+    }
+    *a.d_next = reported;
+    if (a.advance) {
+      if (a.words && pos < a.words_cap) a.words[pos] = feed;
+      *a.d_token = feed;
+      *a.d_pos = pos + 1;
+    }
+    *s_next = a.advance ? feed : -1;
+  }
+  __syncthreads();
+  const int nxt = *s_next;
+  if (nxt >= 0 && nxt < a.vocab) {
+    const f32x4* src = (const f32x4*)(a.tok_emb + (size_t)nxt * a.dim);
+    f32x4* dst = (f32x4*)a.x;
+    for (int i = threadIdx.x; i < (a.dim >> 2); i += kh_wg()) dst[i] = src[i];
+  }
+}
+template <int U, int MAXV>
+__global__ __launch_bounds__(KH_WG_MAX, 4) void k_sample_screen(const KhSampleScreenArgs a) {
+  extern __shared__ __attribute__((aligned(16))) char smem_raw[];
+  __shared__ float s_cv[KH_SCR_CAND];
+  __shared__ int s_ci[KH_SCR_CAND];
+  __shared__ int s_n, s_last, s_next;
+  f32x4* xs = (f32x4*)smem_raw;
+  const int dim = a.dim, vocab = a.vocab;
+  float* red = lds_red_ptr<false>(xs, dim);
+  const int lane = threadIdx.x & 63;
+  const int wave = __builtin_amdgcn_readfirstlane((int)(threadIdx.x >> 6));
+  const float* const wcls = a.wcls;
+  const float eps = a.eps;
+  float l = -INFINITY, sp = -INFINITY;
+  for (int i = threadIdx.x; i < a.nsp; i += kh_wg()) {
+    l = fmaxf(l, a.p_lb[i]);
+    sp = fmaxf(sp, a.p_spill[i]);
+  }
+  if (threadIdx.x == 0) s_n = 0;
+  const float L = block_max(l, red);
+  const float S = block_max(sp, red);
+  for (int i = threadIdx.x; i < a.nsp * KH_SCR_C; i += kh_wg()) {
+    const int idx = a.p_idx[i];
+    if (idx >= 0 && a.p_ub[i] >= L) {
+      const int slot = atomicAdd(&s_n, 1);
+      if (slot < KH_SCR_CAND) s_ci[slot] = idx;
+    }
+  }
+  __syncthreads();
+  const int n = s_n;
+  const bool overflow = S >= L || n > KH_SCR_CAND || n == 0;
+  const Gemv<false, U> g(dim, 0);
+  Stager<true, false, MAXV> st(a.x_save, a.final_norm, dim);
+  if (!overflow) {
+    if (blockIdx.x != 0) return;
+    typename Gemv<false, U>::Regs regs;
+    st.issue();
+    __builtin_amdgcn_sched_barrier(0);
+    const int step = KH_WAVE * U;
+    int r = s_ci[wave < n ? wave : 0];
+    typename Gemv<false, U>::Rows rw = g.rows(wcls, r, wcls, r, nullptr, nullptr, dim);
+    g.load(regs, rw, 0, g.Mc, lane);
+    const float rs = st.finish(xs, eps, red);
+    for (int j = wave; j < n; j += kh_nwaves()) {
+      if (j != wave) {
+        r = s_ci[j];
+        rw = g.rows(wcls, r, wcls, r, nullptr, nullptr, dim);
+        g.load(regs, rw, 0, g.Mc, lane);
+      }
+      float a0 = 0.f, a1 = 0.f;
+      for (int c0 = 0;;) {
+        g.fma(regs, xs, c0, g.Mc, lane, a0, a1);
+        c0 += step;
+        if (c0 >= g.Mc) break;
+        g.load(regs, rw, c0, g.Mc, lane);
+      }
+      float s0 = wave_sum(a0);
+      s0 *= rs;
+      if (lane == 0) s_cv[j] = s0;
+    }
+    __syncthreads();
+    int idx = 0x7fffffff;
+    if (threadIdx.x == 0) {
+      float v = -INFINITY;
+      for (int k = 0; k < n; ++k) amax_merge(v, idx, s_cv[k], s_ci[k]);
+      a.stats[0] += 1;
+      a.stats[1] += n;
+    }
+    screen_tail(a, idx, &s_next);
+    return;
+  }
+  float bv = -INFINITY;
+  int bi = 0x7fffffff;
+  auto r1_of = [&](int p) __attribute__((always_inline)) { return 2 * p + 1 < vocab ? 2 * p + 1 : 2 * p; };
+  auto pair = [&](int p) __attribute__((always_inline)) {
+    return g.rows(wcls, 2 * p, wcls, r1_of(p), nullptr, nullptr, dim);
+  };
+  float rs = 1.f;
+  auto epi = [&](int p, float s0, float s1, const NoAux&) __attribute__((always_inline)) {
+    if (lane != 0) return;
+    const int r0 = 2 * p, r1 = r1_of(p);
+    s0 *= rs;
+    s1 *= rs;
+    amax_merge(bv, bi, s0, r0);
+    if (r1 != r0) amax_merge(bv, bi, s1, r1);
+  };
+  gemv_pairs<1, false>(g, xs, (vocab + 1) >> 1, lane, nullptr, pair,
+                                [](int) __attribute__((always_inline)) { return NoAux{}; },
+                                [&]() __attribute__((always_inline)) { st.issue(); },
+                                [&]() __attribute__((always_inline)) { rs = st.finish(xs, eps, red); }, epi);
+  int* redi = (int*)(red + 3 * KH_WAVES_MAX);
+  __syncthreads();
+  if (lane == 0) {
+    red[wave] = bv;
+    redi[wave] = bi;
+  }
+  __syncthreads();
+  if (threadIdx.x == 0) {
+    float v = red[0];
+    int i = redi[0];
+    for (int w = 1, nw = kh_nwaves(); w < nw; ++w) amax_merge(v, i, red[w], redi[w]);
+    __hip_atomic_store(a.ov_val + blockIdx.x, v, __ATOMIC_RELAXED, __HIP_MEMORY_SCOPE_AGENT);
+    __hip_atomic_store(a.ov_idx + blockIdx.x, i, __ATOMIC_RELAXED, __HIP_MEMORY_SCOPE_AGENT);
+    const uint32_t t = __hip_atomic_fetch_add(a.ticket, 1u, __ATOMIC_ACQ_REL, __HIP_MEMORY_SCOPE_AGENT);
+    s_last = t == gridDim.x - 1 ? 1 : 0;
+  }
+  __syncthreads();
+  if (!s_last) return;
+  __builtin_amdgcn_fence(__ATOMIC_ACQUIRE, "agent");
+  float v = -INFINITY;
+  int idx = 0x7fffffff;
+  for (int i = threadIdx.x; i < (int)gridDim.x; i += kh_wg())
+    amax_merge(v, idx, __hip_atomic_load(a.ov_val + i, __ATOMIC_RELAXED, __HIP_MEMORY_SCOPE_AGENT),
+               __hip_atomic_load(a.ov_idx + i, __ATOMIC_RELAXED, __HIP_MEMORY_SCOPE_AGENT));
+  wave_amax(v, idx);
+  __syncthreads();
+  if (lane == 0) {
+    red[wave] = v;
+    redi[wave] = idx;
+  }
+  __syncthreads();
+  if (threadIdx.x == 0) {
+    v = red[0];
+    idx = redi[0];
+    for (int w = 1, nw = kh_nwaves(); w < nw; ++w) amax_merge(v, idx, red[w], redi[w]);
+    __hip_atomic_store(a.ticket, 0u, __ATOMIC_RELAXED, __HIP_MEMORY_SCOPE_AGENT);
+    a.stats[0] += 1;
+    a.stats[2] += 1;
+  }
+  screen_tail(a, idx, &s_next);
+}
diff --git a/kuiperllama_amd/csrc/kh_model_internal.h b/kuiperllama_amd/csrc/kh_model_internal.h
--- a/kuiperllama_amd/csrc/kh_model_internal.h
+++ b/kuiperllama_amd/csrc/kh_model_internal.h
@@ -116,11 +116,31 @@
     hipGraph_t g = nullptr;
     hipGraphExec_t e = nullptr;
   };
-  StepGraph sg[2][KH_STEP_VARIANTS][4];
+  StepGraph sg[3][KH_STEP_VARIANTS][4];
   kh_sampling samp{0.f, 0, 1.f, 0};
   bool samp_on = false;
   KhSampParams* d_samp = nullptr;
   hipEvent_t ev0 = nullptr, ev1 = nullptr;
+  struct ClsScreen {
+    bool on = false;
+    int selftest = 0;
+    uint16_t* wbf = nullptr;
+    float* err = nullptr;
+    float* x_save = nullptr;
+    float *p_lb = nullptr, *p_spill = nullptr, *p_ub = nullptr;
+    int32_t* p_idx = nullptr;
+    float* ov_val = nullptr;
+    int32_t* ov_idx = nullptr;
+    uint32_t* ticket = nullptr;
+    int32_t* stats = nullptr;
+    float *dbg_lb = nullptr, *dbg_ub = nullptr;
+    int u = 4, grid = 1, wg = KH_WG, sgrid = 1;
+    size_t bytes = 0;
+    float build_ms = 0.f;
+    bool now = false;
+    bool stale = false;
+  };
+  ClsScreen scr;
 };
 
 #define KH_GRAPH_STEPS 8
@@ -155,6 +175,14 @@
 void destroy_step_graphs(kh_model* m);
 int step_graph(kh_model* m, int n_forced, int variant, bool steps8, hipGraphExec_t* out);
 int step_graph_n(kh_model* m, int n_forced, int variant, int nsteps, hipGraphExec_t* out);
+static inline int sg_sampler(const kh_model* m) { return m->samp_on ? 1 : (m->scr.now ? 2 : 0); }
+int cls_screen_create(kh_model* m);
+void cls_screen_release(kh_model* m);
+bool cls_screen_wanted(const kh_model* m);
+void launch_cls_screen(kh_model* m);
+void launch_sample_screen(kh_model* m, int advance, int n_forced);
+int cls_refresh_logits(kh_model* m);
+int cls_screen_selftest(kh_model* m, int32_t* d_flag, bool inject, int* result);
 int kv_ensure(kh_model* m, int rows, int layer = -1);
 int run_selftests(kh_model* m);
 bool prefill_supported(const kh_model* m);
diff --git a/kuiperllama_amd/csrc/kh_model_load.hip b/kuiperllama_amd/csrc/kh_model_load.hip
--- a/kuiperllama_amd/csrc/kh_model_load.hip
+++ b/kuiperllama_amd/csrc/kh_model_load.hip
@@ -588,6 +588,7 @@
   if (m->h_forced_pin) (void)hipHostFree(m->h_forced_pin);
   if (m->first_logits) (void)hipFree(m->first_logits);
   if (m->d_samp) (void)hipFree(m->d_samp);
+  cls_screen_release(m);
   void* bufs[] = {m->x,      m->rms,    m->q,         m->att,       m->h1,       m->h3,
                   m->w2o,    m->logits, m->score,     m->sin_cache,
                   m->cos_cache, m->part_val, m->part_idx, m->d_pos, m->d_token,  m->d_next,
@@ -616,6 +617,7 @@
   m->arena_bytes = weight_nbytes;
   m->cfg.weight_bytes = (int64_t)expected_weight_bytes(m->cfg);
   rc = finish_create(m);
+  if (rc == KH_OK) rc = cls_screen_create(m);
   if (rc == KH_OK) rc = run_selftests(m);
   if (rc != KH_OK) {
     kh_model_destroy(m);
@@ -685,6 +687,8 @@
     if (es != hipSuccess) rc = (int)es;
   }
   pc.lap("upload || buffers, joined");
+  if (rc == KH_OK) rc = cls_screen_create(m);
+  pc.lap("bf16 classifier copy");
   if (rc == KH_OK) rc = run_selftests(m);
   pc.lap("self-tests");
   if (rc != KH_OK) {
@@ -758,6 +762,10 @@
 
 extern "C" int kh_model_get_logits(kh_model* m, float* h_logits) {
   if (!m || !h_logits) return KH_ERR_INVALID_ARG;
+  {
+    const int rc = cls_refresh_logits(m);
+    if (rc != KH_OK) return rc;
+  }
   KH_CHECK_HIP(hipMemcpyAsync(h_logits, m->logits, sizeof(float) * m->cfg.vocab_size,
                               hipMemcpyDeviceToHost, m->stream));
   KH_CHECK_HIP(hipStreamSynchronize(m->stream));
diff --git a/kuiperllama_amd/csrc/kh_model_screen.hip b/kuiperllama_amd/csrc/kh_model_screen.hip
--- /dev/null
+++ b/kuiperllama_amd/csrc/kh_model_screen.hip
@@ -0,0 +1,280 @@
+#include <stdio.h>
+#include <stdlib.h>
+
+#include "kh_cls_screen.h"
+#include "kh_model_internal.h"
+
+namespace khm {
+
+namespace {
+#define KH_LSCR(KERNEL, UU, MV, GRID, WG, LDS, STREAM, ARGS)                                \
+  do {                                                                                      \
+    launch_log(#KERNEL "<" #UU "," #MV ">");                                                \
+    hipLaunchKernelGGL((KERNEL<UU, MV>), dim3(GRID), dim3(WG), LDS, STREAM, ARGS);          \
+  } while (0)
+#define KH_LSCR_MV(KERNEL, UU, MV, ...)                    \
+  do {                                                     \
+    if ((MV) == 4)                                         \
+      KH_LSCR(KERNEL, UU, 4, __VA_ARGS__);                 \
+    else if ((MV) == 2)                                    \
+      KH_LSCR(KERNEL, UU, 2, __VA_ARGS__);                 \
+    else                                                   \
+      KH_LSCR(KERNEL, UU, 1, __VA_ARGS__);                 \
+  } while (0)
+#define KH_LSCR_U4(KERNEL, U, MV, ...)                     \
+  do {                                                     \
+    if ((U) >= 4)                                          \
+      KH_LSCR_MV(KERNEL, 4, MV, __VA_ARGS__);              \
+    else                                                   \
+      KH_LSCR_MV(KERNEL, 2, MV, __VA_ARGS__);              \
+  } while (0)
+#define KH_LSCR_U(KERNEL, U, MV, ...)                      \
+  do {                                                     \
+    if ((U) >= 8)                                          \
+      KH_LSCR_MV(KERNEL, 8, MV, __VA_ARGS__);              \
+    else if ((U) >= 4)                                     \
+      KH_LSCR_MV(KERNEL, 4, MV, __VA_ARGS__);              \
+    else                                                   \
+      KH_LSCR_MV(KERNEL, 2, MV, __VA_ARGS__);              \
+  } while (0)
+
+void plan_screen(kh_model* m) {
+  const kh_config& c = m->cfg;
+  kh_model::ClsScreen& s = m->scr;
+  const int per_lane = (c.dim / 8 + KH_WAVE - 1) / KH_WAVE;
+  s.u = per_lane >= 3 ? 4 : 2;
+  s.wg = m->sh_cls.wg;
+  const int pairs = (c.vocab_size + 1) / 2, wpw = s.wg / KH_WAVE;
+  const int need = (pairs + wpw - 1) / wpw;
+  const int cap = 1024 * KH_WG / s.wg;
+  s.grid = 2 * m->sh_cls.grid;
+  if (s.grid > cap) s.grid = cap;
+  if (s.grid > need) s.grid = need;
+  if (const char* ov = dbg("KH_SHAPE_SCREEN")) {
+    int u = 0, g = 0, w = 0;
+    if (sscanf(ov, "%d,%d,%d", &u, &g, &w) == 3 && (u == 2 || u == 4) && g >= 1 && g <= 4096 &&
+        (w == 256 || w == 512) && kh_stage_maxv(c.dim, w) >= 1 && kh_stage_maxv(c.dim, w) <= 4) {
+      s.u = u;
+      s.grid = g;
+      s.wg = w;
+    } else {
+      fprintf(stderr, "[kh] KH_SHAPE_SCREEN=\"%s\" rejected (u 2/4, grid 1..4096, wg 256/512): planned shape\n", ov);
+    }
+  }
+}
+}
+
+bool cls_screen_wanted(const kh_model* m) {
+  return m->scr.on && !m->samp_on && !dbg_off("KH_CLS_SCREEN") && !dbg("KH_SHAPE_CLS");
+}
+
+void cls_screen_release(kh_model* m) {
+  kh_model::ClsScreen& s = m->scr;
+  for (void* q : {(void*)s.wbf, (void*)s.err, (void*)s.x_save, (void*)s.p_lb, (void*)s.p_spill, (void*)s.p_ub,
+                  (void*)s.p_idx, (void*)s.ov_val, (void*)s.ov_idx, (void*)s.ticket, (void*)s.stats})
+    if (q) (void)hipFree(q);
+  s = kh_model::ClsScreen();
+}
+
+int cls_screen_create(kh_model* m) {
+  const kh_config& c = m->cfg;
+  kh_model::ClsScreen& s = m->scr;
+  s = kh_model::ClsScreen();
+  if (c.is_quant || (m->opts.flags & KH_FLAG_NO_CLS_SCREEN) || dbg_off("KH_CLS_SCREEN") || dbg("KH_SHAPE_CLS")) return KH_OK;
+  if (c.dim % 8 != 0 || c.vocab_size < 2) return KH_OK;
+  const int mv = kh_stage_maxv(c.dim, m->sh_cls.wg);
+  if (mv < 1 || mv > 4) return KH_OK;
+  plan_screen(m);
+  {
+    int cus = 0;
+    if (hipDeviceGetAttribute(&cus, hipDeviceAttributeMultiprocessorCount, m->opts.device) != hipSuccess || cus <= 0)
+      cus = 256;
+    const int wpw = m->sh_cls.wg / KH_WAVE, need = ((c.vocab_size + 1) / 2 + wpw - 1) / wpw;
+    s.sgrid = cus < need ? cus : need;
+  }
+  int rc;
+  const size_t V = (size_t)c.vocab_size;
+#define KH_ALLOC(ptr, n)                         \
+  if ((rc = dalloc(&(ptr), (n))) != KH_OK) {     \
+    cls_screen_release(m);                       \
+    return rc;                                   \
+  }
+  KH_ALLOC(s.wbf, V * (size_t)c.dim);
+  KH_ALLOC(s.err, V);
+  KH_ALLOC(s.x_save, (size_t)c.dim);
+  KH_ALLOC(s.p_lb, 4096);
+  KH_ALLOC(s.p_spill, 4096);
+  KH_ALLOC(s.p_ub, 4096 * KH_SCR_C);
+  KH_ALLOC(s.p_idx, 4096 * KH_SCR_C);
+  KH_ALLOC(s.ov_val, (size_t)s.sgrid);
+  KH_ALLOC(s.ov_idx, (size_t)s.sgrid);
+  KH_ALLOC(s.ticket, 1);
+  KH_ALLOC(s.stats, 4);
+#undef KH_ALLOC
+  s.bytes = V * (size_t)c.dim * sizeof(uint16_t) + V * sizeof(float);
+  hipStream_t st = m->stream;
+  KH_CHECK_HIP(hipMemsetAsync(s.ticket, 0, sizeof(uint32_t), st));
+  KH_CHECK_HIP(hipMemsetAsync(s.stats, 0, 4 * sizeof(int32_t), st));
+  KH_CHECK_HIP(hipMemsetAsync(s.x_save, 0, sizeof(float) * (size_t)c.dim, st));
+  const int n = (c.dim + KH_WAVE - 1) / KH_WAVE + 8;
+  const double u = 1.0 / 16777216.0;
+  const double gam2 = 2.0 * (n * u) / (1.0 - n * u);
+  KH_CHECK_HIP(hipEventRecord(m->ev0, st));
+  hipLaunchKernelGGL(k_cls_bf16_build, dim3(2048), dim3(KH_WG), 0, st, (const float*)m->cls.w, (uint32_t*)s.wbf, s.err,
+                     c.dim, c.vocab_size, gam2);
+  KH_CHECK_HIP(hipEventRecord(m->ev1, st));
+  KH_CHECK_HIP(hipEventSynchronize(m->ev1));
+  if ((rc = kh_launch_status()) != KH_OK) return rc;
+  KH_CHECK_HIP(hipEventElapsedTime(&s.build_ms, m->ev0, m->ev1));
+  s.on = true;
+  if (dbg("KH_LOAD_DEBUG") || dbg("KH_SHAPE_DEBUG"))
+    fprintf(stderr, "[kh] classifier screen: bf16 copy %.1f MB in %.2f ms; k_cls_screen u %d grid %d wg %d, "
+                    "k_sample_screen grid %d wg %d\n", (double)s.bytes / 1e6, s.build_ms, s.u, s.grid, s.wg, s.sgrid,
+            m->sh_cls.wg);
+  return KH_OK;
+}
+
+void launch_cls_screen(kh_model* m) {
+  const kh_config& c = m->cfg;
+  const kh_model::ClsScreen& s = m->scr;
+  KhClsScreenArgs a;
+  a.x = m->x;
+  a.final_norm = m->final_norm;
+  a.wbf = s.wbf;
+  a.err = s.err;
+  a.x_save = s.x_save;
+  a.p_lb = s.p_lb;
+  a.p_spill = s.p_spill;
+  a.p_ub = s.p_ub;
+  a.p_idx = s.p_idx;
+  a.dbg_lb = s.dbg_lb;
+  a.dbg_ub = s.dbg_ub;
+  a.dim = c.dim;
+  a.vocab = c.vocab_size;
+  a.eps = c.rms_eps;
+  KH_LSCR_U4(k_cls_screen, s.u, kh_stage_maxv(c.dim, s.wg), s.grid, s.wg, cls_screen_lds_bytes(c.dim), m->stream, a);
+}
+
+void launch_sample_screen(kh_model* m, int advance, int n_forced) {
+  const kh_config& c = m->cfg;
+  const kh_model::ClsScreen& s = m->scr;
+  KhSampleScreenArgs a;
+  a.p_lb = s.p_lb;
+  a.p_spill = s.p_spill;
+  a.p_ub = s.p_ub;
+  a.p_idx = s.p_idx;
+  a.nsp = s.grid;
+  a.x_save = s.x_save;
+  a.final_norm = m->final_norm;
+  a.wcls = (const float*)m->cls.w;
+  a.eps = c.rms_eps;
+  a.ov_val = s.ov_val;
+  a.ov_idx = s.ov_idx;
+  a.ticket = s.ticket;
+  a.stats = s.stats;
+  a.forced = n_forced > 0 ? m->d_forced : nullptr;
+  a.n_forced = n_forced;
+  a.words = m->d_words;
+  a.words_cap = m->seq_cap;
+  a.d_next = m->d_next;
+  a.d_token = m->d_token;
+  a.d_pos = m->d_pos;
+  a.tok_emb = m->tok_emb;
+  a.x = m->x;
+  a.dim = c.dim;
+  a.vocab = c.vocab_size;
+  a.advance = advance;
+  const int wg = m->sh_cls.wg;
+  KH_LSCR_U(k_sample_screen, m->sh_cls.u, kh_stage_maxv(c.dim, wg), s.sgrid, wg, cls_lds_bytes(false, c.dim), m->stream, a);
+}
+
+int cls_refresh_logits(kh_model* m) {
+  if (!m->scr.stale) return KH_OK;
+  KH_CHECK_HIP(hipSetDevice(m->opts.device));
+  float* const x = m->x;
+  m->x = m->scr.x_save;
+  launch_cls(m);
+  m->x = x;
+  return kh_launch_status();
+}
+
+namespace {
+__global__ __launch_bounds__(KH_WG) void k_st_interval(const float* lg, const float* lb, const float* ub, size_t n,
+                                                      int32_t* flag) {
+  bool d = false;
+  for (size_t i = (size_t)blockIdx.x * KH_WG + threadIdx.x; i < n; i += (size_t)gridDim.x * KH_WG) {
+    const float v = lg[i];
+    d |= v == v ? !(lb[i] <= v && v <= ub[i]) : !(lb[i] == -INFINITY && ub[i] == INFINITY);
+  }
+  if (d) *flag = 1;
+}
+}
+
+int cls_screen_selftest(kh_model* m, int32_t* d_flag, bool inject, int* result) {
+  const kh_config& c = m->cfg;
+  kh_model::ClsScreen& s = m->scr;
+  *result = 0;
+  if (!s.on) return KH_OK;
+  hipStream_t st = m->stream;
+  const size_t V = (size_t)c.vocab_size;
+  int rc = KH_OK;
+  int32_t tok[2] = {-1, -2};
+  if ((rc = dalloc(&s.dbg_lb, V)) == KH_OK && (rc = dalloc(&s.dbg_ub, V)) == KH_OK) {
+    set_state(m, 1 % c.vocab_size, 0);
+    s.now = true;
+    launch_cls_screen(m);
+    launch_sample(m, 0, 0);
+    s.now = false;
+    hipError_t e = hipMemcpyAsync(&tok[0], m->d_next, sizeof(int32_t), hipMemcpyDeviceToHost, st);
+    launch_cls(m);
+    launch_sample(m, 0, 0);
+    if (e == hipSuccess) e = hipMemcpyAsync(&tok[1], m->d_next, sizeof(int32_t), hipMemcpyDeviceToHost, st);
+    const size_t g = (V + KH_WG - 1) / KH_WG;
+    hipLaunchKernelGGL(k_st_interval, dim3((unsigned)(g > 1024 ? 1024 : g)), dim3(KH_WG), 0, st, m->logits, s.dbg_lb,
+                       s.dbg_ub, V, d_flag);
+    int32_t flag = 0;
+    if (e == hipSuccess) e = hipMemcpyAsync(&flag, d_flag, sizeof(flag), hipMemcpyDeviceToHost, st);
+    if (e == hipSuccess) e = hipStreamSynchronize(st);
+    if (e != hipSuccess) rc = (int)e;
+    if (rc == KH_OK) rc = kh_launch_status();
+    if (rc == KH_OK) *result = (flag || tok[0] != tok[1] || inject) ? -1 : 1;
+  }
+  if (s.dbg_lb) (void)hipFree(s.dbg_lb);
+  if (s.dbg_ub) (void)hipFree(s.dbg_ub);
+  s.dbg_lb = s.dbg_ub = nullptr;
+  if (rc != KH_OK) return rc;
+  KH_CHECK_HIP(hipMemsetAsync(s.stats, 0, 4 * sizeof(int32_t), st));
+  if (*result < 0) {
+    fprintf(stderr, "[kh] classifier screen self-test failed (tokens %d / %d): screening is off for this model\n",
+            tok[0], tok[1]);
+    cls_screen_release(m);
+    s.selftest = -1;
+  } else {
+    s.selftest = 1;
+  }
+  return KH_OK;
+}
+
+}
+using namespace khm;
+
+extern "C" int kh_model_cls_screen_info(kh_model* m, int64_t* out) {
+  if (!m || !out) return KH_ERR_INVALID_ARG;
+  const kh_model::ClsScreen& s = m->scr;
+  for (int i = 0; i < 8; ++i) out[i] = 0;
+  out[0] = s.on ? 1 : 0;
+  out[1] = s.selftest;
+  out[2] = (int64_t)s.bytes;
+  out[3] = (int64_t)(s.build_ms * 1000.f);
+  out[7] = KH_SCR_CAND;
+  if (s.on) {
+    int32_t h[4] = {0, 0, 0, 0};
+    KH_CHECK_HIP(hipSetDevice(m->opts.device));
+    KH_CHECK_HIP(hipMemcpyAsync(h, s.stats, sizeof(h), hipMemcpyDeviceToHost, m->stream));
+    KH_CHECK_HIP(hipStreamSynchronize(m->stream));
+    out[4] = h[0];
+    out[5] = h[1];
+    out[6] = h[2];
+  }
+  return KH_OK;
+}
diff --git a/kuiperllama_amd/csrc/kh_model_selftest.hip b/kuiperllama_amd/csrc/kh_model_selftest.hip
--- a/kuiperllama_amd/csrc/kh_model_selftest.hip
+++ b/kuiperllama_amd/csrc/kh_model_selftest.hip
@@ -161,17 +161,18 @@
   const auto t0 = std::chrono::steady_clock::now();
   const char* inj = dbg("KH_SELFTEST_FAIL");
   int32_t* d_flag = nullptr;
-  KH_CHECK_HIP(hipMalloc((void**)&d_flag, 2 * sizeof(int32_t)));
-  int r = 0, a = 0;
-  const hipError_t e = hipMemsetAsync(d_flag, 0, 2 * sizeof(int32_t), m->stream);
+  KH_CHECK_HIP(hipMalloc((void**)&d_flag, 3 * sizeof(int32_t)));
+  int r = 0, a = 0, sc = 0;
+  const hipError_t e = hipMemsetAsync(d_flag, 0, 3 * sizeof(int32_t), m->stream);
   int rc = e == hipSuccess ? ring_selftest(m, d_flag, hook_has(inj, "ring"), &r) : (int)e;
   if (rc == KH_OK) rc = attn_selftest(m, d_flag + 1, hook_has(inj, "attn"), &a);
+  if (rc == KH_OK) rc = cls_screen_selftest(m, d_flag + 2, hook_has(inj, "screen"), &sc);
   (void)hipFree(d_flag);
   if (rc != KH_OK) return rc;
   m->cfg.ring_selftest = r;
   m->cfg.attn_merge_selftest = a;
   if (dbg("KH_LOAD_DEBUG") || dbg("KH_SHAPE_DEBUG"))
-    fprintf(stderr, "[kh] self-tests: ring %d, attention merge %d (%.2f ms)\n", r, a,
+    fprintf(stderr, "[kh] self-tests: ring %d, attention merge %d, classifier screen %d (%.2f ms)\n", r, a, sc,
             std::chrono::duration<double, std::milli>(std::chrono::steady_clock::now() - t0).count());
   return KH_OK;
 }
diff --git a/kuiperllama_amd/csrc/kh_model_step.hip b/kuiperllama_amd/csrc/kh_model_step.hip
--- a/kuiperllama_amd/csrc/kh_model_step.hip
+++ b/kuiperllama_amd/csrc/kh_model_step.hip
@@ -330,6 +330,7 @@
 }
 void launch_cls(kh_model* m) {
   const kh_config& c = m->cfg;
+  m->scr.stale = false;
   KhClsArgs a;
   a.x = m->x;
   a.final_norm = m->final_norm;
@@ -352,6 +353,10 @@
 }
 void launch_sample(kh_model* m, int advance, int n_forced) {
   const kh_config& c = m->cfg;
+  if (m->scr.now && !m->samp_on) {
+    launch_sample_screen(m, advance, n_forced);
+    return;
+  }
   KhSampleArgs a;
   a.part_val = m->part_val;
   a.part_idx = m->part_idx;
@@ -419,7 +424,10 @@
     launch_w2(m, l);
     mark();
   }
-  launch_cls(m);
+  if (m->scr.now && !m->samp_on)
+    launch_cls_screen(m);
+  else
+    launch_cls(m);
   mark();
   launch_sample(m, advance, n_forced);
   mark();
@@ -533,12 +541,13 @@
   if (variant < 0 || variant >= KH_STEP_VARIANTS) return KH_ERR_INVALID_ARG;
   const int k = nsteps == 1 ? 0 : nsteps == 2 ? 1 : nsteps == 4 ? 2 : nsteps == KH_GRAPH_STEPS ? 3 : -1;
   if (k < 0) return KH_ERR_INVALID_ARG;
-  kh_model::StepGraph& sg = m->sg[m->samp_on ? 1 : 0][variant][k];
+  kh_model::StepGraph& sg = m->sg[sg_sampler(m)][variant][k];
   if (!sg.e) {
     const int rc = capture_steps(m, n_forced, nsteps, variant, &sg.g, &sg.e);
     if (rc != KH_OK) return rc;
     (void)hipGraphUpload(sg.e, m->stream);
   }
+  m->scr.stale = m->scr.now;
   *out = sg.e;
   return KH_OK;
 }
@@ -634,6 +643,7 @@
   int rc = kv_ensure(m, pos + 1);
   if (rc != KH_OK) return rc;
   set_state(m, token, pos);
+  m->scr.stale = false;
   if (exec == KH_EXEC_UNFUSED) {
     rc = launch_step_unfused(m, pos);
   } else if (exec == KH_EXEC_FUSED || exec == KH_EXEC_GRAPH) {
@@ -724,6 +734,12 @@
   }
   if (exec != KH_EXEC_GRAPH && exec != KH_EXEC_FUSED) return KH_ERR_INVALID_ARG;
 
+  const bool screen = cls_screen_wanted(m);
+  struct ScreenOff {
+    kh_model* m;
+    ~ScreenOff() { m->scr.now = false; }
+  } screen_off{m};
+  m->scr.now = screen;
   if ((rc = ensure_seq_cap(m, total_steps)) != KH_OK) return rc;
   if ((rc = kv_ensure(m, total_steps < KH_GRAPH_STEPS ? KH_GRAPH_STEPS : total_steps)) != KH_OK) return rc;
   if ((rc = ensure_pinned_words(m, m->seq_cap)) != KH_OK) return rc;
@@ -743,7 +759,7 @@
     bool fresh[4] = {false, false, false, false};
     hipGraphExec_t ge = nullptr;
     for (int n = 1, k = 0; n <= KH_GRAPH_STEPS; n *= 2, ++k) {
-      fresh[k] = m->sg[m->samp_on ? 1 : 0][0][k].e == nullptr;
+      fresh[k] = m->sg[sg_sampler(m)][0][k].e == nullptr;
       if ((rc = step_graph_n(m, n_forced, 0, n, &ge)) != KH_OK) return rc;
     }
     bool dry = false;
@@ -751,11 +767,12 @@
       for (int k = 3; k >= 0; --k)
         if (fresh[k]) {
           set_state(m, h_prompt[0], 0);
-          KH_CHECK_HIP(hipGraphLaunch(m->sg[m->samp_on ? 1 : 0][0][k].e, m->stream));
+          KH_CHECK_HIP(hipGraphLaunch(m->sg[sg_sampler(m)][0][k].e, m->stream));
           dry = true;
         }
     if (dry) KH_CHECK_HIP(hipStreamSynchronize(m->stream));
   }
+  m->scr.now = false;
 
   int start = 0;
   KH_CHECK_HIP(hipEventRecord(m->ev0, m->stream));
@@ -790,6 +807,8 @@
       while (n > total_steps - s) n >>= 1;
       const bool keep = s == start && start > 0;
       if (keep) n = 1;
+      m->scr.now = screen && !keep;
+      m->scr.stale = m->scr.now;
       hipGraphExec_t ge = nullptr;
       if (step_graph_n(m, n_forced, step_variant(m, s, s + n - 1), n, &ge) != KH_OK) return -1;
       if (hipGraphLaunch(ge, m->stream) != hipSuccess) return -1;
@@ -798,7 +817,9 @@
         return -1;
       return n;
     }
+    m->scr.now = screen && !(s == start && start > 0);
     launch_step_fused(m, 1, n_forced, nullptr, step_variant(m, s, s));
+    m->scr.stale = m->scr.now;
     if (s == start && start > 0 &&
         hipMemcpyAsync(m->first_logits, m->logits, sizeof(float) * (size_t)c.vocab_size, hipMemcpyDeviceToDevice,
                        m->stream) != hipSuccess)
diff --git a/kuiperllama_amd/model.py b/kuiperllama_amd/model.py
--- a/kuiperllama_amd/model.py
+++ b/kuiperllama_amd/model.py
@@ -110,6 +110,12 @@
         _ffi.check(_ffi.lib().kh_model_get_logits(self._h, out.ctypes.data), "kh_model_get_logits")
         return out
 
+    def cls_screen_info(self) -> dict:
+        out = (C.c_int64 * 8)()
+        _ffi.check(_ffi.lib().kh_model_cls_screen_info(self._h, out), "kh_model_cls_screen_info")
+        keys = ("on", "selftest", "bytes", "build_us", "steps", "candidates", "overflow_steps", "capacity")
+        return dict(zip(keys, (int(v) for v in out)))
+
     def kv_bytes(self) -> Tuple[int, int]:
         r, c = C.c_int64(0), C.c_int64(0)
         _ffi.check(_ffi.lib().kh_model_kv_bytes(self._h, C.byref(r), C.byref(c)), "kh_model_kv_bytes")
```

New measurement: 1109 tokens/s, median of 6. 1.07x the previous value.
